# martinruenz/co-fusion

Measured on AMD Instinct MI355X. Metric: frames/sec at 640x480 (N active models) + ICP-reduce achieved HBM GB/s vs peak, higher is better.
Workload: dtype f32

## Files before the change

### co_fusion_amd/csrc/cabi.hip

```cpp
#include <stdlib.h>
#include <string.h>

#include <string>

#include "cf_host.h"

using namespace cf;

void cf_ctx::set_error(const std::string& m)
{
    std::lock_guard<std::mutex> lk(error_mutex);
    last_error = m;
}

static int lane_ready(cf_ctx* ctx, int lane)
{
    if (!ctx->lanes[lane]) {
        HIPCHK(ctx, hipStreamCreateWithFlags(&ctx->lanes[lane], hipStreamNonBlocking));
        HIPCHK(ctx, hipEventCreateWithFlags(&ctx->lane_done[lane], hipEventDisableTiming));
    }
    return CF_OK;
}
static void leave_lane(cf_ctx* ctx)
{
    if (ctx->forked) { ctx->stream = ctx->forked_from; ctx->forked = false; }
}
static int join_lane(cf_ctx* ctx, int lane)
{
    HIPCHK(ctx, hipEventRecord(ctx->lane_done[lane], ctx->lanes[lane]));
    HIPCHK(ctx, hipStreamWaitEvent(ctx->stream, ctx->lane_done[lane], 0));
    return CF_OK;
}

extern "C" {

int cf_create(const cf_config* cfg, cf_ctx** out)
{
    if (!cfg || !out || cfg->width <= 0 || cfg->height <= 0 || (cfg->width % 16) || (cfg->height % 4)) return CF_EINVAL;
    int ndev = 0;
    if (hipGetDeviceCount(&ndev) != hipSuccess || ndev <= 0) return CF_EHIP;
    cf_ctx* ctx = new cf_ctx();
    ctx->cfg = *cfg;
    if (ctx->cfg.max_models <= 0) ctx->cfg.max_models = 1;
    *out = ctx;
    HIPCHK(ctx, hipSetDevice(cfg->device));
    HIPCHK(ctx, hipStreamCreateWithFlags(&ctx->own_stream, hipStreamNonBlocking));
    ctx->stream = ctx->own_stream;
    ctx->icp_launch = IcpLaunch{256, 0, 0};
    if (int r = dmalloc(ctx, &ctx->d_acc_a, (size_t)kGroups * 32)) return r;
    if (int r = dmalloc(ctx, &ctx->d_acc_b, (size_t)kGroups * 32)) return r;
    if (int r = dmalloc(ctx, &ctx->d_out, 64)) return r;
    if (int r = dmalloc(ctx, &ctx->d_scratch_state, 1)) return r;
    if (int r = dmalloc(ctx, &ctx->d_state_pool, (size_t)cf_ctx::kStateSlots)) return r;
    HIPCHK(ctx, hipHostMalloc(reinterpret_cast<void**>(&ctx->h_state_pool), sizeof(OdomDev) * cf_ctx::kStateSlots, hipHostMallocCoherent));
    memset(ctx->h_state_pool, 0, sizeof(OdomDev) * cf_ctx::kStateSlots);
    if (int r = dmalloc(ctx, &ctx->d_so3_sync, (size_t)ctx->cfg.max_models + 1)) return r;
    if (const char* e = getenv("CF_ICP_ARITH")) {
        if (cf_set_icp_arith(ctx, (!strcmp(e, "gram") || !strcmp(e, "1")) ? CF_ICP_ARITH_GRAM : (!strcmp(e, "reference") || !strcmp(e, "2")) ? CF_ICP_ARITH_REFERENCE
                                  : (!strcmp(e, "product") || !strcmp(e, "0")) ? CF_ICP_ARITH_PRODUCT : -1) != CF_OK) {
            ctx->set_error("CF_ICP_ARITH: product | gram | reference"); return CF_EINVAL;
        }
    }
    if (int r = dmalloc(ctx, &ctx->d_cand_scratch, (size_t)cfg->width * cfg->height)) return r;
    HIPCHK(ctx, hipHostMalloc(reinterpret_cast<void**>(&ctx->h_scratch_state), sizeof(OdomDev)));
    HIPCHK(ctx, hipHostMalloc(reinterpret_cast<void**>(&ctx->h_out), sizeof(unsigned long long) * 64));
    ctx->prof.capacity = 8192;
    ctx->prof.events = new hipEvent_t[ctx->prof.capacity];
    for (int i = 0; i < ctx->prof.capacity; i++) HIPCHK(ctx, hipEventCreate(&ctx->prof.events[i]));
    ctx->prof.used = 0; ctx->prof.enabled = 0; ctx->prof.bytes = 0; ctx->prof.launches = 0;
    HIPCHK(ctx, hipStreamSynchronize(ctx->stream));
    return CF_OK;
}

void cf_destroy(cf_ctx* ctx)
{
    if (ctx && ctx->batch_event) (void)hipEventDestroy(ctx->batch_event);
    if (ctx) for (int i = 0; i < cf_ctx::kSurfEvents; i++) if (ctx->surf_events[i]) (void)hipEventDestroy(ctx->surf_events[i]);
    if (!ctx) return;
    (void)hipStreamSynchronize(ctx->stream);
    (void)cf_rccl_destroy(ctx);
    (void)hipFree(ctx->d_acc_a); (void)hipFree(ctx->d_acc_b); (void)hipFree(ctx->d_out);
    (void)hipFree(ctx->d_scratch_state); (void)hipFree(ctx->d_so3_sync); (void)hipFree(ctx->d_cand_scratch);
    (void)hipFree(ctx->d_state_pool); (void)hipHostFree(ctx->h_state_pool);
    (void)hipHostFree(ctx->h_scratch_state); (void)hipHostFree(ctx->h_out);
    if (ctx->d_ref) (void)hipFree(ctx->d_ref);
    if (ctx->h_ref) (void)hipHostFree(ctx->h_ref);
    if (ctx->d_redetect_bits) (void)hipFree(ctx->d_redetect_bits);
    if (ctx->d_redetect_counts) (void)hipFree(ctx->d_redetect_counts);
    if (ctx->h_redetect_counts) (void)hipHostFree(ctx->h_redetect_counts);
    if (ctx->d_search) (void)hipFree(ctx->d_search);
    if (ctx->h_search) (void)hipHostFree(ctx->h_search);
    for (hipEvent_t e : ctx->redetect_ev) if (e) (void)hipEventDestroy(e);
    if (ctx->prof.events) {
        for (int i = 0; i < ctx->prof.capacity; i++) (void)hipEventDestroy(ctx->prof.events[i]);
        delete[] ctx->prof.events;
    }
    for (int i = 0; i < cf_ctx::kLanes; i++) {
        if (ctx->lanes[i]) (void)hipStreamDestroy(ctx->lanes[i]);
        if (ctx->lane_done[i]) (void)hipEventDestroy(ctx->lane_done[i]);
    }
    if (ctx->fork_point) (void)hipEventDestroy(ctx->fork_point);
    for (int i = 0; i < cf_ctx::kMarks; i++) if (ctx->marks[i]) (void)hipEventDestroy(ctx->marks[i]);
    if (ctx->own_stream) (void)hipStreamDestroy(ctx->own_stream);
    delete ctx;
}

const char* cf_last_error(const cf_ctx* ctx)
{
    if (!ctx) return "null ctx";
    static thread_local std::string copy;
    {
        std::lock_guard<std::mutex> lk(const_cast<cf_ctx*>(ctx)->error_mutex);
        copy = ctx->last_error;
    }
    return copy.c_str();
}
int cf_set_stream(cf_ctx* ctx, void* s)
{
    if (!ctx || ctx->forked) return CF_EINVAL;
    if (ctx->stream != (hipStream_t)s) HIPCHK(ctx, hipStreamSynchronize(ctx->stream));
    ctx->stream = (hipStream_t)s;
    return CF_OK;
}
int cf_use_own_stream(cf_ctx* ctx)
{
    if (!ctx || ctx->forked) return CF_EINVAL;
    if (ctx->stream != ctx->own_stream) HIPCHK(ctx, hipStreamSynchronize(ctx->stream));
    ctx->stream = ctx->own_stream;
    return CF_OK;
}

extern "C++" { thread_local cf_thread_binding cf_tls_binding; }

int cf_fork(cf_ctx* ctx, int lane)
{
    if (!ctx || lane < 0) return CF_EINVAL;
    lane %= cf_ctx::kLanes;
    if (int r = lane_ready(ctx, lane)) return r;
    if (!ctx->fork_point) HIPCHK(ctx, hipEventCreateWithFlags(&ctx->fork_point, hipEventDisableTiming));
    if (!ctx->forked) {
        ctx->forked_from = ctx->stream;
        HIPCHK(ctx, hipEventRecord(ctx->fork_point, ctx->forked_from));
        ctx->forked = true;
    }
    HIPCHK(ctx, hipStreamWaitEvent(ctx->lanes[lane], ctx->fork_point, 0));
    ctx->lanes_used |= 1u << lane;
    ctx->stream = ctx->lanes[lane];
    return CF_OK;
}
int cf_mark(cf_ctx* ctx, int slot)
{
    if (!ctx || slot < 0 || slot >= cf_ctx::kMarks) return CF_EINVAL;
    if (!ctx->marks[slot]) HIPCHK(ctx, hipEventCreateWithFlags(&ctx->marks[slot], hipEventDisableTiming));
    HIPCHK(ctx, hipEventRecord(ctx->marks[slot], ctx->stream));
    ctx->mark_set[slot] = true;
    return CF_OK;
}
int cf_event_wait_host(cf_ctx* ctx, int slot)
{
    if (!ctx || slot < 0 || slot >= cf_ctx::kMarks) return CF_EINVAL;
    if (ctx->mark_set[slot]) HIPCHK(ctx, hipEventSynchronize(ctx->marks[slot]));
    return CF_OK;
}
int cf_fork_after(cf_ctx* ctx, int lane, int slot)
{
    if (!ctx || lane < 0 || slot >= cf_ctx::kMarks || ctx->forked) return CF_EINVAL;
    lane %= cf_ctx::kLanes;
    if (int r = lane_ready(ctx, lane)) return r;
    if (slot >= 0 && ctx->mark_set[slot]) HIPCHK(ctx, hipStreamWaitEvent(ctx->lanes[lane], ctx->marks[slot], 0));
    ctx->forked_from = ctx->stream;
    ctx->forked = true;
    ctx->lanes_used |= 1u << lane;
    ctx->stream = ctx->lanes[lane];
    return CF_OK;
}
int cf_main(cf_ctx* ctx)
{
    if (!ctx) return CF_EINVAL;
    leave_lane(ctx);
    return CF_OK;
}
int cf_join(cf_ctx* ctx)
{
    if (!ctx) return CF_EINVAL;
    leave_lane(ctx);
    for (int lane = 0; lane < cf_ctx::kLanes; lane++)
        if (ctx->lanes_used & (1u << lane))
            if (int r = join_lane(ctx, lane)) return r;
    ctx->lanes_used = 0;
    return CF_OK;
}
int cf_join_lane(cf_ctx* ctx, int lane)
{
    if (!ctx || lane < 0) return CF_EINVAL;
    lane %= cf_ctx::kLanes;
    leave_lane(ctx);
    if (ctx->lanes_used & (1u << lane)) {
        if (int r = join_lane(ctx, lane)) return r;
        ctx->lanes_used &= ~(1u << lane);
    }
    return CF_OK;
}
int cf_thread_lane(cf_ctx* ctx, int lane)
{
    if (!ctx) return CF_EINVAL;
    if (lane < 0) { cf_tls_binding = cf_thread_binding{}; return CF_OK; }
    lane %= cf_ctx::kLanes;
    if (!ctx->lanes[lane] || !(ctx->lanes_used & (1u << lane))) { ctx->set_error("cf_thread_lane: lane was not forked"); return CF_ESTATE; }
    HIPCHK(ctx, hipSetDevice(ctx->cfg.device));
    cf_tls_binding.ctx = ctx;
    cf_tls_binding.stream = ctx->lanes[lane];
    return CF_OK;
}
void* cf_get_stream(cf_ctx* ctx) { return ctx ? (void*)ctx->stream : nullptr; }
int cf_synchronize(cf_ctx* ctx) { if (!ctx) return CF_EINVAL; HIPCHK(ctx, hipStreamSynchronize(ctx->stream)); return CF_OK; }
int cf_malloc(cf_ctx* ctx, uint64_t bytes, void** dptr)
{
    if (!ctx || !dptr) return CF_EINVAL;
    HIPCHK(ctx, hipMalloc(dptr, bytes));
    HIPCHK(ctx, hipMemsetAsync(*dptr, 0, bytes, ctx->stream));
    return CF_OK;
}
int cf_free(cf_ctx* ctx, void* dptr) { if (!ctx) return CF_EINVAL; HIPCHK(ctx, hipStreamSynchronize(ctx->stream)); HIPCHK(ctx, hipFree(dptr)); return CF_OK; }
int cf_memcpy_h2d(cf_ctx* ctx, void* dst, const void* src, uint64_t bytes)
{
    if (!ctx) return CF_EINVAL;
    HIPCHK(ctx, hipMemcpyAsync(dst, src, bytes, hipMemcpyHostToDevice, ctx->stream));
    HIPCHK(ctx, hipStreamSynchronize(ctx->stream));
    return CF_OK;
}
int cf_memcpy_d2h(cf_ctx* ctx, void* dst, const void* src, uint64_t bytes)
{
    if (!ctx) return CF_EINVAL;
    HIPCHK(ctx, hipMemcpyAsync(dst, src, bytes, hipMemcpyDeviceToHost, ctx->stream));
    HIPCHK(ctx, hipStreamSynchronize(ctx->stream));
    return CF_OK;
}

int cf_malloc_host(cf_ctx* ctx, uint64_t bytes, void** hptr)
{
    if (!ctx || !hptr) return CF_EINVAL;
    HIPCHK(ctx, hipHostMalloc(hptr, bytes));
    return CF_OK;
}
int cf_free_host(cf_ctx* ctx, void* hptr) { if (!ctx) return CF_EINVAL; HIPCHK(ctx, hipHostFree(hptr)); return CF_OK; }
int cf_memcpy_h2d_async(cf_ctx* ctx, void* dst, const void* src_pinned, uint64_t bytes)
{
    if (!ctx) return CF_EINVAL;
    HIPCHK(ctx, hipMemcpyAsync(dst, src_pinned, bytes, hipMemcpyHostToDevice, ctx->stream));
    return CF_OK;
}
int cf_memcpy_d2h_async(cf_ctx* ctx, void* dst_pinned, const void* src, uint64_t bytes)
{
    if (!ctx) return CF_EINVAL;
    HIPCHK(ctx, hipMemcpyAsync(dst_pinned, src, bytes, hipMemcpyDeviceToHost, ctx->stream));
    return CF_OK;
}
int cf_memcpy_d2d_async(cf_ctx* ctx, void* dst, const void* src, uint64_t bytes)
{
    if (!ctx) return CF_EINVAL;
    HIPCHK(ctx, hipMemcpyAsync(dst, src, bytes, hipMemcpyDeviceToDevice, ctx->stream));
    return CF_OK;
}
int cf_rgb_to_rgba(cf_ctx* ctx, const uint8_t* rgb_dev, int cols, int rows, uint8_t* rgba_dev)
{
    if (!ctx || !rgb_dev || !rgba_dev || cols <= 0 || rows <= 0) return CF_EINVAL;
    launch_rgb_expand(ctx->stream, rgb_dev, cols * rows, rgba_dev);
    LAUNCHCHK(ctx);
    return CF_OK;
}

int cf_set_icp_launch(cf_ctx* ctx, int threads, int ppt)
{
    if (!ctx || (threads != 64 && threads != 128 && threads != 256 && threads != 512 && threads != 1024) ||
        (ppt != 0 && ppt != 1 && ppt != 2 && ppt != 4))
        return CF_EINVAL;
    ctx->icp_launch = IcpLaunch{threads, ppt, ctx->icp_launch.gram};
    return CF_OK;
}

int cf_set_icp_arith(cf_ctx* ctx, int mode)
{
    if (!ctx || (mode != CF_ICP_ARITH_PRODUCT && mode != CF_ICP_ARITH_GRAM && mode != CF_ICP_ARITH_REFERENCE)) return CF_EINVAL;
    ctx->icp_arith = mode;
    ctx->icp_launch.gram = mode == CF_ICP_ARITH_GRAM ? 1 : 0;
    return CF_OK;
}
int cf_get_icp_arith(cf_ctx* ctx) { return ctx ? ctx->icp_arith : CF_EINVAL; }

int cf_profile_enable(cf_ctx* ctx, int on) { if (!ctx || on < 0) return CF_EINVAL; ctx->prof.enabled = on; ctx->prof_calls = 0; return CF_OK; }
int cf_profile_read(cf_ctx* ctx, cf_profile* out, int reset)
{
    if (!ctx || !out) return CF_EINVAL;
    HIPCHK(ctx, hipStreamSynchronize(ctx->stream));
    double ms = ctx->prof_ms_accum;
    for (int i = 0; i + 1 < ctx->prof.used; i += 2) {
        float t = 0;
        HIPCHK(ctx, hipEventElapsedTime(&t, ctx->prof.events[i], ctx->prof.events[i + 1]));
        ms += t;
    }
    ctx->prof_ms_accum = ms;
    ctx->prof.used = 0;
    out->icp_ms_total = ms; out->icp_launches = ctx->prof.launches; out->icp_bytes = ctx->prof.bytes;
    for (int i = 0; i + 1 < ctx->surf_used; i += 2) {
        float t = 0;
        HIPCHK(ctx, hipEventElapsedTime(&t, ctx->surf_events[i], ctx->surf_events[i + 1]));
        ctx->surf_ms_accum += t;
    }
    ctx->surf_used = 0;
    out->surfel_ms_total = ctx->surf_ms_accum; out->surfel_calls = ctx->surf_calls; out->surfel_bytes = ctx->surf_bytes;
    if (reset) { ctx->prof_ms_accum = 0; ctx->prof.launches = 0; ctx->prof.bytes = 0; ctx->surf_ms_accum = 0; ctx->surf_calls = 0; ctx->surf_bytes = 0; }
    return CF_OK;
}

}
```

### co_fusion_amd/csrc/cabi_model.hip

```cpp
#include <math.h>
#include <string.h>

#include <string>
#include <vector>

#include "cf_host.h"

using namespace cf;

struct cf_model {
    cf_ctx* ctx = nullptr;
    uint32_t max_surfels = 0;
    uint32_t count_host = 0;
    bool count_pending = false;
    hipEvent_t count_event = nullptr;
    hipEvent_t count_wait = nullptr;
    bool ratio_valid = false;
    hipEvent_t ratio_event = nullptr;
    float* buf[2] = {nullptr, nullptr};
    int target = 0;
    float* staged = nullptr;
    unsigned* flags = nullptr;
    unsigned* block_sums = nullptr;
    unsigned* d_count = nullptr;
// ... 240 lines not shown
}

int cf_model_initialise(cf_model* m, const uint8_t* rgba, const float* depth_raw, const float* depth_filt, int time, float maxDepth)
{
    if (!m || !rgba || !depth_raw || !depth_filt) return CF_EINVAL;
    m->drop_preindex();
    m->extents_unknown();
    cf_ctx* ctx = m->ctx; hipStream_t s = ctx->cur();
    const int W = ctx->cfg.width, H = ctx->cfg.height; const long long N = (long long)W * H;
    if ((uint32_t)N > m->max_surfels) return CF_ENOMEM;
    const cf_cam cam = ctx_cam(ctx);
    launch_feedback(s, rgba, depth_raw, W, H, cam, m->inv_fx, m->inv_fy, m->tcx, m->tcy, time, maxDepth, m->fb_rec, m->new_flags);
    HIPCHK(ctx, hipMemsetAsync(m->fb_raw, 0, sizeof(float) * 12 * N, s));
    const ScanPassArgs raw{m->fb_rec, m->new_flags, N, m->block_sums, m->d_count, 0, m->fb_raw, nullptr};
    launch_scan_scatter_batch(s, &raw, 1);
    launch_feedback(s, rgba, depth_filt, W, H, cam, m->inv_fx, m->inv_fy, m->tcx, m->tcy, time, maxDepth, m->fb_rec, m->new_flags);
    HIPCHK(ctx, hipMemsetAsync(m->fb_filt, 0, sizeof(float) * 12 * N, s));
    const ScanPassArgs filt{m->fb_rec, m->new_flags, N, m->block_sums, m->d_tmp2, 0, m->fb_filt, nullptr};
    launch_scan_scatter_batch(s, &filt, 1);
    m->new_flags_clean = false;
    launch_init(s, m->fb_raw, m->fb_filt, m->d_count, N, m->buf[m->target]);
    LAUNCHCHK(ctx);
    return sync_count(m);
}

int cf_model_count(cf_model* m, uint32_t* count) { if (!m || !count) return CF_EINVAL; return exact_count(m, count); }

int cf_model_predict_indices(cf_model* m, const float pose[16], int time, float maxDepth, int timeDelta)
{
    if (!m || !pose) return CF_EINVAL;
    m->drop_preindex();
    m->extents_unknown();
    cf_ctx* ctx = m->ctx;
    uint32_t nb = 0;
    if (int r = count_bound(m, &nb)) return r;
    const IndexPassArgs a = index_pass_args(m, pose, nullptr, nb, maxDepth, time, timeDelta);
    launch_index_keys_batch(ctx->cur(), &a, 1, ctx_cam(ctx), ctx->cfg.width, ctx->cfg.height);
    launch_index_resolve_batch(ctx->cur(), &a, 1, ctx_cam(ctx), ctx->cfg.width, ctx->cfg.height);
    LAUNCHCHK(ctx);
    return CF_OK;
}

int cf_model_index_keys(cf_model* m, const float pose[16], int time, float maxDepth, int timeDelta, uint32_t surfel_begin, uint32_t surfel_end,
                        uint64_t* keys_dev)
{
    if (!m || !pose || !keys_dev || surfel_begin > surfel_end) return CF_EINVAL;
    m->drop_preindex();
    m->extents_unknown();
    cf_ctx* ctx = m->ctx;
    const int W = ctx->cfg.width, H = ctx->cfg.height;
    uint32_t nb = 0;
    if (int r = count_bound(m, &nb)) return r;
    HIPCHK(ctx, hipMemsetAsync(keys_dev, 0xFF, sizeof(uint64_t) * (size_t)W * H, ctx->cur()));
    IndexPassArgs a = index_pass_args(m, pose, nullptr, surfel_end < nb ? surfel_end : nb, maxDepth, time, timeDelta);
    a.id_begin = surfel_begin; a.keys = reinterpret_cast<unsigned long long*>(keys_dev);
    launch_index_keys_batch(ctx->cur(), &a, 1, ctx_cam(ctx), W, H);
    LAUNCHCHK(ctx);
    return CF_OK;
}
int cf_model_index_resolve(cf_model* m, const float pose[16], uint64_t* keys_dev)
{
    if (!m || !pose || !keys_dev) return CF_EINVAL;
    m->drop_preindex();
    m->extents_unknown();
    cf_ctx* ctx = m->ctx;
    IndexPassArgs a = index_pass_args(m, pose, nullptr, 0, 0.f, 0, 0);
    a.keys = reinterpret_cast<unsigned long long*>(keys_dev);
    launch_index_resolve_batch(ctx->cur(), &a, 1, ctx_cam(ctx), ctx->cfg.width, ctx->cfg.height);
    LAUNCHCHK(ctx);
    return CF_OK;
}

int cf_model_predict_indices_sharded(cf_model* m, const float pose[16], int time, float maxDepth, int timeDelta, int shard, int nshards)
{
    if (!m || !pose || nshards < 1 || shard < 0 || shard >= nshards) return CF_EINVAL;
    m->drop_preindex();
    cf_ctx* ctx = m->ctx;
    if (!ctx->collective) { ctx->set_error("cf_model_predict_indices_sharded: no collective registered (cf_set_collective)"); return CF_ESTATE; }
    uint32_t n = 0;
    if (int r = exact_count(m, &n)) return r;
    const uint32_t b = (uint32_t)(((uint64_t)n * (uint64_t)shard) / (uint64_t)nshards), e = (uint32_t)(((uint64_t)n * (uint64_t)(shard + 1)) / (uint64_t)nshards);
    if (int r = cf_model_index_keys(m, pose, time, maxDepth, timeDelta, b, e, reinterpret_cast<uint64_t*>(m->keys))) return r;
    if (ctx->collective(ctx->collective_user, 1, m->keys, (uint64_t)ctx->cfg.width * ctx->cfg.height, (void*)ctx->cur()) != 0) {
        ctx->set_error("cf_model_predict_indices_sharded: the collective failed");
        return CF_ESTATE;
    }
    return cf_model_index_resolve(m, pose, reinterpret_cast<uint64_t*>(m->keys));
}

int cf_model_combined_predict(cf_model* m, const float pose[16], float maxDepth, float confThreshold, int time, int maxTime, int timeDelta)
{
    if (!m || !pose) return CF_EINVAL;
    cf_ctx* ctx = m->ctx;
    uint32_t nb = 0;
    if (int r = count_bound(m, &nb)) return r;
    const SplatPassArgs a = splat_args(m, pose, nb, maxDepth, confThreshold, time, maxTime, timeDelta);
    launch_combined_predict_batch(ctx->cur(), &a, 1, ctx_cam(ctx), ctx->cfg.width, ctx->cfg.height);
    LAUNCHCHK(ctx);
    m->ratio_valid = false;
    return CF_OK;
}

int cf_model_predict_inactive(cf_model* m, const float pose[16], float maxDepth, float confThreshold, int maxTime, int timeDelta)
{
    if (!m || !pose) return CF_EINVAL;
    cf_ctx* ctx = m->ctx;
    const size_t N = (size_t)ctx->cfg.width * ctx->cfg.height;
    if (!m->old_covered) {
        if (!m->old_image) if (int r = dmalloc(ctx, &m->old_image, N * 4)) return r;
        if (!m->old_vertex) if (int r = dmalloc(ctx, &m->old_vertex, N * 4)) return r;
        if (!m->old_normal) if (int r = dmalloc(ctx, &m->old_normal, N * 4)) return r;
        if (!m->old_time) if (int r = dmalloc(ctx, &m->old_time, N)) return r;
        if (int r = dmalloc(ctx, &m->old_covered, 1)) return r;
    }
    uint32_t nb = 0;
    if (int r = count_bound(m, &nb)) return r;
    SplatPassArgs a = splat_args(m, pose, nb, maxDepth, confThreshold, 0, maxTime, timeDelta);
    a.image = m->old_image; a.vertexConf = m->old_vertex; a.normalRad = m->old_normal; a.time16 = m->old_time;
    a.fill.out2 = m->old_covered;
    HIPCHK(ctx, hipMemsetAsync(m->old_covered, 0, sizeof(unsigned), ctx->cur()));
    launch_combined_predict_batch(ctx->cur(), &a, 1, ctx_cam(ctx), ctx->cfg.width, ctx->cfg.height, kSplatCount);
    LAUNCHCHK(ctx);
    return CF_OK;
}

int cf_model_synthesize_depth(cf_model* m, const float pose[16], float maxDepth, float confThreshold, int time, int maxTime, int timeDelta,
                              float* depth_out_dev)
{
    if (!m || !pose || !depth_out_dev) return CF_EINVAL;
    cf_ctx* ctx = m->ctx;
    uint32_t nb = 0;
    if (int r = count_bound(m, &nb)) return r;
    SplatPassArgs a = splat_args(m, pose, nb, maxDepth, confThreshold, time, maxTime, timeDelta);
    a.image = nullptr; a.vertexConf = depth_out_dev; a.normalRad = nullptr; a.time16 = nullptr;
    launch_combined_predict_batch(ctx->cur(), &a, 1, ctx_cam(ctx), ctx->cfg.width, ctx->cfg.height, kSplatDepth);
    LAUNCHCHK(ctx);
    return CF_OK;
}

int cf_model_prefetch_fill_ratio(cf_model* m)
{
    if (!m) return CF_EINVAL;
    cf_ctx* ctx = m->ctx;
    launch_fill_ratio(ctx->cur(), m->splat_image, ctx->cfg.width, ctx->cfg.height, m->d_tmp2 + 2, m->h_counts + 2);
    LAUNCHCHK(ctx);
    HIPCHK(ctx, hipEventRecord(m->ratio_event, ctx->cur()));
    m->ratio_valid = true;
    return CF_OK;
}

int cf_model_perform_fill_in(cf_model* m, const uint8_t* rgba, const float* depth_filt, int passthrough_geom, int passthrough_rgb)
{
    if (!m || !rgba || !depth_filt) return CF_EINVAL;
    cf_ctx* ctx = m->ctx;
    launch_fill_in(ctx->cur(), m->splat_vertex, m->splat_normal, m->splat_image, depth_filt, rgba, ctx->cfg.width, ctx->cfg.height, ctx_cam(ctx),
                   m->inv_fx, m->inv_fy, passthrough_geom, passthrough_rgb, m->fill_vertex, m->fill_normal, m->fill_image);
    LAUNCHCHK(ctx);
    return CF_OK;
}

int cf_model_requires_fill_in(cf_model* m, float ratio, int* out)
{
    if (!m || !out) return CF_EINVAL;
    cf_ctx* ctx = m->ctx;
    if (m->ratio_valid) {
        HIPCHK(ctx, hipEventSynchronize(m->ratio_event));
    } else {
        launch_fill_ratio(ctx->cur(), m->splat_image, ctx->cfg.width, ctx->cfg.height, m->d_tmp2 + 2, m->h_counts + 2);
        LAUNCHCHK(ctx);
        HIPCHK(ctx, hipStreamSynchronize(ctx->cur()));
    }
    *out = ((float)m->h_counts[2] / (float)m->h_counts[3] < ratio) ? 1 : 0;
    return CF_OK;
}

int cf_model_fill_ratio_device(cf_model* m, const uint32_t** counts_dev)
{
    if (!m || !counts_dev) return CF_EINVAL;
    *counts_dev = m->ratio_valid ? m->d_tmp2 + 2 : nullptr;
    return CF_OK;
}

int cf_model_fuse(cf_model* m, const float pose[16], int time, const uint8_t* rgba, const uint8_t* mask, const float* depth_raw,
                  const float* depth_filt, float maxDepth, float weighting, int maskID)
{
    if (!m || !pose || !rgba || !mask || !depth_raw || !depth_filt) return CF_EINVAL;
    m->drop_preindex();
    m->extents_unknown();
    cf_ctx* ctx = m->ctx; hipStream_t s = ctx->cur();
    cf_model_pass it{};
    it.model = m; it.pose = pose; it.rgba = rgba; it.mask = mask; it.depth_raw = depth_raw; it.depth_filtered = depth_filt; it.time = time;
    it.fuse_max_depth = maxDepth; it.weighting = weighting; it.mask_id = maskID;
    const SurfelFuseArgs a = fuse_args(it);
    launch_associate_batch(s, &a, 1);
    const ScanPassArgs sp = fresh_compaction_args(m);
    launch_scan_scatter_batch(s, &sp, 1);
    m->new_flags_clean = true;
    uint32_t nb = 0;
    if (int r = count_bound(m, &nb)) return r;
    const UpdatePassArgs ua = update_pass_args(m, nb, time);
    launch_update_batch(s, &ua, 1);
    m->target = 1 - m->target;
    LAUNCHCHK(ctx);
    return CF_OK;
}

int cf_model_clean(cf_model* m, const float pose[16], int time, float confThreshold, float outlierCoeff, int timeDelta, const float* depth_filt,
                   const uint8_t* mask, int maskID, uint32_t* count_out)
{
    if (!m || !pose || !depth_filt || !mask) return CF_EINVAL;
    m->drop_preindex();
    m->extents_unknown();
    cf_ctx* ctx = m->ctx; hipStream_t s = ctx->cur();
    uint32_t nb = 0;
    if (int r = count_bound(m, &nb)) return r;
    unsigned bound = 0;
    if (int r = clean_staging_bound(m, nb, "cf_model_clean", &bound)) return r;
    cf_model_pass it{};
    it.model = m; it.pose = pose; it.mask = mask; it.depth_filtered = depth_filt; it.time = time; it.mask_id = maskID; it.conf_threshold = confThreshold;
    const CleanPassArgs a = clean_pass_args(it, outlierCoeff, timeDelta, bound, false);
    launch_clean_batch(s, &a, 1);
    const ScanPassArgs sp = kept_compaction_args(m, bound);
    launch_scan_scatter_batch(s, &sp, 1);
    m->target = 1 - m->target;
    LAUNCHCHK(ctx);
    const uint32_t upper = bound < m->max_surfels ? bound : m->max_surfels;
    if (int r = post_count(m, upper)) return r;
    if (count_out) return exact_count(m, count_out);
    return CF_OK;
}

int cf_models_preindex(cf_ctx* ctx, const cf_model_preindex* items, int n, float depth_cutoff, int time_delta)
{
    if (!ctx || !items || n <= 0) return CF_EINVAL;
    hipStream_t s = ctx->cur();
    const int W = ctx->cfg.width, H = ctx->cfg.height;
    std::vector<IndexPassArgs> a((size_t)n);
    for (int k = 0; k < n; k++)
        if (!items[k].model || !items[k].odom || items[k].model->ctx != ctx || items[k].odom->ctx != ctx) return CF_EINVAL;
    ExtentGuard guard;
    for (int k = 0; k < n; k++) guard.models.push_back(items[k].model);
    const bool cull = extent_culling_on(ctx);
    for (int k = 0; k < n; k++) {
        cf_model* m = items[k].model; const cf_odom* od = items[k].odom;
        uint32_t nb = 0;
        if (int r = count_bound(m, &nb)) return r;
        const float* pinv = reinterpret_cast<const float*>(reinterpret_cast<const char*>(od->d_state) + offsetof(cf::OdomDev, pose_inv));
        a[k] = index_pass_args(m, nullptr, pinv, nb, depth_cutoff, items[k].time, time_delta);
        if (int r = next_extent(m, cull, nb, s, &a[k].ext, &a[k].ext_slot)) return r;
    }
    launch_index_keys_batch(s, a.data(), n, ctx_cam(ctx), W, H);
    launch_index_resolve_batch(s, a.data(), n, ctx_cam(ctx), W, H);
    LAUNCHCHK(ctx);
    for (int k = 0; k < n; k++) {
        cf_model* m = items[k].model;
        m->preindex_od = items[k].odom; m->preindex_time = items[k].time; m->preindex_cutoff = depth_cutoff; m->preindex_delta = time_delta; m->preindex_nb = a[k].id_end;
    }
    guard.done = true;
    return CF_OK;
}
static bool preindexed_with(const cf_model* m, const float pose[16], int time, float depth_cutoff, int time_delta, uint32_t nb)
{
    if (!m->preindex_od || m->preindex_time != time) return false;
    if (m->preindex_cutoff != depth_cutoff || m->preindex_delta != time_delta || m->preindex_nb != nb) return false;
    const cf::OdomDev* h = m->preindex_od->h_state;
    for (int r = 0; r < 3; r++) {
        if (memcmp(&pose[r * 4], &h->Rcurr[r * 3], 12) != 0 || memcmp(&pose[r * 4 + 3], &h->tcurr[r], 4) != 0) return false;
    }
    return pose[12] == 0 && pose[13] == 0 && pose[14] == 0 && pose[15] == 1;
}

int cf_models_frame_passes(cf_ctx* ctx, const cf_model_pass* items, int n, float depth_cutoff, float outlier_coeff, int time_delta)
{
    if (!ctx || !items || n <= 0) return CF_EINVAL;
    hipStream_t s = ctx->cur();
    const int W = ctx->cfg.width, H = ctx->cfg.height;
    const cf_cam cam = ctx_cam(ctx);
    std::vector<int> fusing;
    for (int k = 0; k < n; k++) {
        const cf_model_pass& it = items[k];
        if (!it.model || it.model->ctx != ctx || !it.pose || !it.rgba || !it.depth_filtered) return CF_EINVAL;
        if (it.do_fuse) { if (!it.mask || !it.depth_raw) return CF_EINVAL; fusing.push_back(k); }
    }
    for (int k : fusing) {
        cf_model* m = items[k].model;
        uint32_t nb = 0; unsigned bound = 0;
        if (int r = count_bound(m, &nb)) return r;
        if (int r = clean_staging_bound(m, nb, "cf_models_frame_passes", &bound)) return r;
    }
    for (int k = 0; k < n; k++) { uint32_t nb = 0; if (int r = count_bound(items[k].model, &nb)) return r; }
    ExtentGuard guard;
    for (int k = 0; k < n; k++) guard.models.push_back(items[k].model);
    const bool cull = extent_culling_on(ctx);
    int surf_ev = -1;
    if (ctx->prof.enabled > 0 && (ctx->surf_calls_seen++ % (unsigned)ctx->prof.enabled) == 0 && ctx->surf_used + 2 <= cf_ctx::kSurfEvents) {
        for (int e = ctx->surf_used; e < ctx->surf_used + 2; e++)
            if (!ctx->surf_events[e]) HIPCHK(ctx, hipEventCreate(&ctx->surf_events[e]));
        surf_ev = ctx->surf_used; ctx->surf_used += 2;
        HIPCHK(ctx, hipEventRecord(ctx->surf_events[surf_ev], s));
        for (int k = 0; k < n; k++) ctx->surf_bytes += (uint64_t)items[k].model->count_host * 48u * (items[k].do_fuse ? 8u : 2u);
        ctx->surf_calls++;
    }
    static const bool clean_rec_on = getenv("CF_NO_CLEAN_REC") == nullptr;
    auto index_args_of = [&](const std::vector<int>& which, bool feeds_clean, std::vector<IndexPassArgs>& a) -> int {
        a.assign(which.size(), IndexPassArgs{});
        for (size_t q = 0; q < which.size(); q++) {
            const cf_model_pass& it = items[which[q]]; cf_model* m = it.model;
            uint32_t nb = 0;
            if (int r = count_bound(m, &nb)) return r;
            a[q] = index_pass_args(m, it.pose, nullptr, nb, depth_cutoff, it.time, time_delta, feeds_clean && clean_rec_on ? it.depth_filtered : nullptr);
            if (int r = next_extent(m, cull, nb, s, &a[q].ext, &a[q].ext_slot)) return r;
        }
        return CF_OK;
    };
    if (!fusing.empty()) {
        const int nf = (int)fusing.size();
        {
            std::vector<int> todo;
            for (int k : fusing) {
                uint32_t nb = 0;
                if (int r = count_bound(items[k].model, &nb)) return r;
                if (!preindexed_with(items[k].model, items[k].pose, items[k].time, depth_cutoff, time_delta, nb)) todo.push_back(k);
            }
            std::vector<IndexPassArgs> a;
            if (int r = index_args_of(todo, false, a)) return r;
            launch_index_keys_batch(s, a.data(), (int)a.size(), cam, W, H);
            launch_index_resolve_batch(s, a.data(), (int)a.size(), cam, W, H);
        }
        std::vector<SurfelFuseArgs> fa(nf);
        std::vector<ScanPassArgs> sa(nf);
        std::vector<UpdatePassArgs> ua(nf);
        for (int q = 0; q < nf; q++) {
            const cf_model_pass& it = items[fusing[q]]; cf_model* m = it.model;
            fa[q] = fuse_args(it);
            sa[q] = fresh_compaction_args(m);
            m->new_flags_clean = true;
            uint32_t nb = 0;
            if (int r = count_bound(m, &nb)) return r;
            ua[q] = update_pass_args(m, nb, it.time);
        }
        launch_associate_batch(s, fa.data(), nf);
        for (int q = 0; q < nf; q++) items[fusing[q]].model->target = 1 - items[fusing[q]].model->target;
        {
            std::vector<IndexPassArgs> ia;
            if (int r = index_args_of(fusing, true, ia)) return r;
            static const bool side_by_side = getenv("CF_NO_SIDE_BY_SIDE") == nullptr;
            if (!(side_by_side && launch_update_compaction_index_keys(s, ua.data(), sa.data(), ia.data(), nf, cam, W, H))) {
                launch_scan_scatter_batch(s, sa.data(), nf);
                launch_update_batch(s, ua.data(), nf);
                launch_index_keys_batch(s, ia.data(), nf, cam, W, H);
            }
            launch_index_resolve_batch(s, ia.data(), nf, cam, W, H);
        }
        std::vector<CleanPassArgs> ca(nf);
        for (int q = 0; q < nf; q++) {
            const cf_model_pass& it = items[fusing[q]]; cf_model* m = it.model;
            uint32_t nb = 0; unsigned bound = 0;
            if (int r = count_bound(m, &nb)) return r;
            if (int r = clean_staging_bound(m, nb, "cf_models_frame_passes", &bound)) return r;
            ca[q] = clean_pass_args(it, outlier_coeff, time_delta, bound, clean_rec_on);
            sa[q] = kept_compaction_args(m, bound);
        }
        launch_clean_batch(s, ca.data(), nf);
        launch_scan_scatter_batch(s, sa.data(), nf);
        if (!ctx->batch_event) HIPCHK(ctx, hipEventCreateWithFlags(&ctx->batch_event, hipEventDisableTiming));
        for (int q = 0; q < nf; q++) {
            cf_model* m = items[fusing[q]].model;
            m->target = 1 - m->target;
            m->count_host = ca[q].total_bound < m->max_surfels ? ca[q].total_bound : m->max_surfels; m->count_pending = true; m->count_wait = nullptr;
        }
    }
    std::vector<SplatPassArgs> pa(n);
    for (int k = 0; k < n; k++) {
        const cf_model_pass& it = items[k]; cf_model* m = it.model;
        uint32_t nb = m->count_host;
        if (!(m->count_pending && !m->count_wait)) { if (int r = count_bound(m, &nb)) return r; }
        SplatPassArgs& p = pa[k];
        p = splat_args(m, it.pose, nb, depth_cutoff, it.conf_threshold, it.time, it.time, time_delta);
        m->ratio_valid = false;
        if (it.fill_in)
            p.fill = SplatFillArgs{it.depth_filtered, it.rgba, m->inv_fx, m->inv_fy, it.passthrough_geom ? 1 : 0, it.passthrough_rgb ? 1 : 0,
                                   m->fill_vertex, m->fill_normal, m->fill_image, reinterpret_cast<unsigned long long*>(m->d_tmp2 + 4),
                                   m->d_tmp2 + 2, m->h_counts + 2, m->ratio_blocks};
    }
    launch_combined_predict_batch(s, pa.data(), n, cam, W, H);
    LAUNCHCHK(ctx);
    for (int k = 0; k < n; k++)
        if (items[k].fill_in) {
            HIPCHK(ctx, hipEventRecord(items[k].model->ratio_event, s));
            items[k].model->ratio_valid = true;
        }
    if (surf_ev >= 0) HIPCHK(ctx, hipEventRecord(ctx->surf_events[surf_ev + 1], s));
    if (!fusing.empty()) {
        HIPCHK(ctx, hipEventRecord(ctx->batch_event, s));
        for (int k : fusing) items[k].model->count_wait = ctx->batch_event;
    }
    for (int k = 0; k < n; k++) items[k].model->drop_preindex();
    guard.done = true;
    return CF_OK;
}

int cf_model_download_map(cf_model* m, float* host_surfels, uint32_t capacity, uint32_t* count)
{
    if (!m || !count) return CF_EINVAL;
    cf_ctx* ctx = m->ctx;
    if (int r = exact_count(m, count)) return r;
    if (host_surfels) {
        const uint32_t n = m->count_host < capacity ? m->count_host : capacity;
        HIPCHK(ctx, hipMemcpyAsync(host_surfels, m->buf[m->target], (size_t)n * 48, hipMemcpyDeviceToHost, ctx->cur()));
        HIPCHK(ctx, hipStreamSynchronize(ctx->cur()));
    }
    return CF_OK;
}

int cf_model_upload_map(cf_model* m, const float* host_surfels, uint32_t count)
{
    if (!m || (!host_surfels && count) || count > m->max_surfels) return CF_EINVAL;
    m->drop_preindex();
    m->extents_unknown();
    cf_ctx* ctx = m->ctx;
    if (count) HIPCHK(ctx, hipMemcpyAsync(m->buf[m->target], host_surfels, (size_t)count * 48, hipMemcpyHostToDevice, ctx->cur()));
    launch_set_count(ctx->cur(), m->d_count, count);
    HIPCHK(ctx, hipStreamSynchronize(ctx->cur()));
    m->count_host = count; m->count_pending = false;
    return CF_OK;
}

int cf_model_buffer(cf_model* m, int which, void** dptr, uint64_t* bytes)
{
    if (!m || !dptr) return CF_EINVAL;
    const size_t N = (size_t)m->ctx->cfg.width * m->ctx->cfg.height;
    void* p = nullptr; size_t b = 0;
    switch (which) {
        case 0: p = m->index; b = N * 4; break;
        case 1: p = m->vertConf; b = N * 16; break;
        case 2: p = m->colorTime; b = N * 16; break;
        case 3: p = m->normRad; b = N * 16; break;
        case 4: p = m->splat_image; b = N * 4; break;
        case 5: p = m->splat_vertex; b = N * 16; break;
        case 6: p = m->splat_normal; b = N * 16; break;
        case 7: p = m->splat_time; b = N * 2; break;
        case 8: p = m->fill_vertex; b = N * 16; break;
        case 9: p = m->fill_normal; b = N * 16; break;
        case 10: p = m->fill_image; b = N * 4; break;
        case 11: { uint32_t c = 0; if (int r = exact_count(m, &c)) return r; p = m->buf[m->target]; b = (size_t)c * 48; break; }
        case 12: {
            unsigned nf = 0;
            HIPCHK(m->ctx, hipMemcpyAsync(&nf, m->d_nfresh, sizeof(unsigned), hipMemcpyDeviceToHost, m->ctx->cur()));
            HIPCHK(m->ctx, hipStreamSynchronize(m->ctx->cur()));
            if (nf > N / 4 + 64) { m->ctx->set_error("cf_model_buffer: the new-surfel count exceeds its buffer"); return CF_ESTATE; }
            p = m->fresh; b = (size_t)nf * 48; break;
        }
        case 13: p = m->clean_rec; b = N * 32; break;
        case 14: p = m->keys; b = N * 8; break;
        case 15: case 16: case 17: case 18: case 19:
            if (!m->old_covered) { m->ctx->set_error("cf_model_buffer: no inactive prediction yet (cf_model_predict_inactive)"); return CF_ESTATE; }
            if (which == 15) { p = m->old_image; b = N * 4; }
            else if (which == 16) { p = m->old_vertex; b = N * 16; }
            else if (which == 17) { p = m->old_normal; b = N * 16; }
            else if (which == 18) { p = m->old_time; b = N * 2; }
            else { p = m->old_covered; b = 4; }
            break;
        default: return CF_EINVAL;
    }
    *dptr = p; if (bytes) *bytes = b;
    return CF_OK;
}

int cf_set_extent_culling(cf_ctx* ctx, int on)
{
    if (!ctx) return CF_EINVAL;
    ctx->extent_cull = on != 0;
    return CF_OK;
}
int cf_model_extents_unknown(cf_model* m)
{
    if (!m) return CF_EINVAL;
    m->extents_unknown();
    return CF_OK;
}

int cf_redetect_score(cf_ctx* ctx, const cf_redetect_candidate* cands, int n, const cf_redetect_frame* f, cf_redetect_counts* counts, uint32_t* label_pixels)
{
    if (!ctx || !cands || !f || !counts || n <= 0 || n > kRedetectBatch) return CF_EINVAL;
    if (!f->depth || !f->label || f->cols <= 0 || f->rows <= 0 || (long long)f->cols * f->rows > 0x7fffffffLL) return CF_EINVAL;
    hipStream_t s = ctx->cur();
    const unsigned words = (unsigned)(((long long)f->cols * f->rows + 31) / 32);
    const size_t n_counts = (size_t)kRedetectBatch * kRedetectWords + 1;
    if (!ctx->d_redetect_counts) {
        if (int r = dmalloc(ctx, &ctx->d_redetect_counts, n_counts)) return r;
        HIPCHK(ctx, hipHostMalloc(reinterpret_cast<void**>(&ctx->h_redetect_counts), n_counts * sizeof(unsigned)));
    }
    if (words > ctx->redetect_words) {
        HIPCHK(ctx, hipStreamSynchronize(s));
        if (ctx->d_redetect_bits) (void)hipFree(ctx->d_redetect_bits);
        ctx->d_redetect_bits = nullptr; ctx->redetect_words = 0;
        if (int r = dmalloc(ctx, &ctx->d_redetect_bits, (size_t)kRedetectBatch * words)) return r;
        ctx->redetect_words = words;
    }
    RedetectCand rc[kRedetectBatch];
    for (int k = 0; k < n; k++) {
        cf_model* m = cands[k].model;
        if (!m || m->ctx != ctx) return CF_EINVAL;
        uint32_t nb = 0;
        if (int r = count_bound(m, &nb)) return r;
        rc[k].surfels = m->buf[m->target]; rc[k].count = m->d_count; rc[k].count_bound = nb; rc[k].theta = cands[k].conf_threshold;
        inv44f(cands[k].pose, rc[k].t_inv);
    }
    RedetectFrame rf{f->depth, f->label, f->cols, f->rows, f->cam, f->new_label, f->depth_cutoff, f->depth_tol};
    if (ctx->redetect_timing) HIPCHK(ctx, hipEventRecord(ctx->redetect_ev[0], s));
    HIPCHK(ctx, hipMemsetAsync(ctx->d_redetect_counts, 0, n_counts * sizeof(unsigned), s));
    launch_redetect_score(s, rc, n, rf, ctx->d_redetect_bits, words, ctx->d_redetect_counts);
    LAUNCHCHK(ctx);
    if (ctx->redetect_timing) HIPCHK(ctx, hipEventRecord(ctx->redetect_ev[1], s));
    HIPCHK(ctx, hipMemcpyAsync(ctx->h_redetect_counts, ctx->d_redetect_counts, n_counts * sizeof(unsigned), hipMemcpyDeviceToHost, s));
    HIPCHK(ctx, hipStreamSynchronize(s));
    if (ctx->redetect_timing) HIPCHK(ctx, hipEventElapsedTime(&ctx->redetect_last_ms, ctx->redetect_ev[0], ctx->redetect_ev[1]));
    for (int k = 0; k < n; k++) {
        const unsigned* w = ctx->h_redetect_counts + (size_t)k * kRedetectWords;
        counts[k] = cf_redetect_counts{w[0], w[1], w[2], w[3], w[4], w[5]};
    }
    if (label_pixels) *label_pixels = ctx->h_redetect_counts[(size_t)kRedetectBatch * kRedetectWords];
    return CF_OK;
}

int cf_redetect_timing(cf_ctx* ctx, int on, float* last_ms)
{
    if (!ctx) return CF_EINVAL;
    if (on) for (hipEvent_t& e : ctx->redetect_ev) if (!e) HIPCHK(ctx, hipEventCreate(&e));
    ctx->redetect_timing = on != 0;
    if (last_ms) *last_ms = ctx->redetect_last_ms;
    return CF_OK;
}

int cf_relabel(cf_ctx* ctx, uint8_t* label_dev, uint64_t n, int from, int to)
{
    if (!ctx || !label_dev || from < 0 || from > 255 || to < 0 || to > 255 || (reinterpret_cast<uintptr_t>(label_dev) & 15u)) return CF_EINVAL;
    if (from == to || n == 0) return CF_OK;
    launch_relabel(ctx->cur(), label_dev, n, (unsigned)from, (unsigned)to);
    LAUNCHCHK(ctx);
    return CF_OK;
}

static int search_buffers(cf_ctx* ctx)
{
    if (ctx->d_search) return CF_OK;
    HIPCHK(ctx, hipMalloc(reinterpret_cast<void**>(&ctx->d_search), cf_ctx::kSearchBytes));
    HIPCHK(ctx, hipHostMalloc(reinterpret_cast<void**>(&ctx->h_search), cf_ctx::kSearchBytes));
    return CF_OK;
}
static bool search_frame_ok(const cf_redetect_frame* f)
{
    return f && f->depth && f->label && f->cols > 0 && f->rows > 0 && (long long)f->cols * f->rows <= 0x7fffffffLL;
}
static int search_fetch(cf_ctx* ctx, hipStream_t s, size_t offset, size_t bytes)
{
    LAUNCHCHK(ctx);
    if (ctx->redetect_timing) HIPCHK(ctx, hipEventRecord(ctx->redetect_ev[1], s));
    HIPCHK(ctx, hipMemcpyAsync(reinterpret_cast<char*>(ctx->h_search) + offset, reinterpret_cast<char*>(ctx->d_search) + offset, bytes, hipMemcpyDeviceToHost, s));
    HIPCHK(ctx, hipStreamSynchronize(s));
    if (ctx->redetect_timing) HIPCHK(ctx, hipEventElapsedTime(&ctx->redetect_last_ms, ctx->redetect_ev[0], ctx->redetect_ev[1]));
    return CF_OK;
}
static unsigned* search_hist(unsigned long long* base) { return reinterpret_cast<unsigned*>(base + cf_ctx::kSearchWords); }
static constexpr size_t kSearchStepWord = (size_t)kRedetectBatch * kMomentWords;

int cf_redetect_frame_moments(cf_ctx* ctx, const cf_redetect_frame* f, const uint8_t* rgba_dev, int64_t moments[4], uint32_t hist[CF_REDETECT_BINS])
{
    if (!ctx || !search_frame_ok(f) || !rgba_dev || !moments || !hist) return CF_EINVAL;
    if (int r = search_buffers(ctx)) return r;
    hipStream_t s = ctx->cur();
    RedetectFrame rf{f->depth, f->label, f->cols, f->rows, f->cam, f->new_label, f->depth_cutoff, f->depth_tol};
    if (ctx->redetect_timing) HIPCHK(ctx, hipEventRecord(ctx->redetect_ev[0], s));
    HIPCHK(ctx, hipMemsetAsync(ctx->d_search, 0, kMomentWords * 8, s));
    HIPCHK(ctx, hipMemsetAsync(search_hist(ctx->d_search), 0, kRedetectBins * 4, s));
    launch_redetect_frame_moments(s, rf, rgba_dev, ctx->d_search, search_hist(ctx->d_search));
    if (int r = search_fetch(ctx, s, 0, cf_ctx::kSearchWords * 8 + kRedetectBins * 4)) return r;
    for (int k = 0; k < kMomentWords; k++) moments[k] = (int64_t)ctx->h_search[k];
    memcpy(hist, search_hist(ctx->h_search), kRedetectBins * 4);
    return CF_OK;
}

static int search_cand(cf_ctx* ctx, cf_model* m, float theta, RedetectCand* rc)
{
    if (!m || m->ctx != ctx) return CF_EINVAL;
    uint32_t nb = 0;
    if (int r = count_bound(m, &nb)) return r;
    rc->surfels = m->buf[m->target]; rc->count = m->d_count; rc->count_bound = nb; rc->theta = theta;
    return CF_OK;
}

int cf_redetect_model_moments(cf_ctx* ctx, const cf_redetect_candidate* cands, int n, const float dhat[3], int64_t* moments, uint32_t* hist)
{
    if (!ctx || !cands || !dhat || !moments || !hist || n <= 0 || n > kRedetectBatch) return CF_EINVAL;
    if (int r = search_buffers(ctx)) return r;
    RedetectCand rc[kRedetectBatch];
    for (int k = 0; k < n; k++) {
        if (int r = search_cand(ctx, cands[k].model, cands[k].conf_threshold, &rc[k])) return r;
        inv44f(cands[k].pose, rc[k].t_inv);
    }
    hipStream_t s = ctx->cur();
    if (ctx->redetect_timing) HIPCHK(ctx, hipEventRecord(ctx->redetect_ev[0], s));
    HIPCHK(ctx, hipMemsetAsync(ctx->d_search, 0, (size_t)n * kMomentWords * 8, s));
    HIPCHK(ctx, hipMemsetAsync(search_hist(ctx->d_search), 0, (size_t)n * kRedetectBins * 4, s));
    launch_redetect_model_moments(s, rc, n, dhat, ctx->d_search, search_hist(ctx->d_search));
    if (int r = search_fetch(ctx, s, 0, cf_ctx::kSearchWords * 8 + (size_t)n * kRedetectBins * 4)) return r;
    for (int k = 0; k < n * kMomentWords; k++) moments[k] = (int64_t)ctx->h_search[k];
    memcpy(hist, search_hist(ctx->h_search), (size_t)n * kRedetectBins * 4);
    return CF_OK;
}

static int register_step(cf_ctx* ctx, RedetectCand& rc, const float T[16], const RedetectFrame& rf, const float centre[3])
{
    hipStream_t s = ctx->cur();
    memcpy(rc.t_inv, T, sizeof(rc.t_inv));
    if (ctx->redetect_timing) HIPCHK(ctx, hipEventRecord(ctx->redetect_ev[0], s));
    HIPCHK(ctx, hipMemsetAsync(ctx->d_search + kSearchStepWord, 0, 32 * 8, s));
    launch_redetect_register_step(s, rc, rf, centre, ctx->d_search + kSearchStepWord);
    return search_fetch(ctx, s, kSearchStepWord * 8, 32 * 8);
}

int cf_redetect_register_step(cf_ctx* ctx, cf_model* model, float conf_threshold, const float cam_from_model[16], const cf_redetect_frame* f,
                              const float centre[3], int64_t sums[32])
{
    if (!ctx || !cam_from_model || !search_frame_ok(f) || !centre || !sums) return CF_EINVAL;
    if (int r = search_buffers(ctx)) return r;
    RedetectCand rc{};
    if (int r = search_cand(ctx, model, conf_threshold, &rc)) return r;
    RedetectFrame rf{f->depth, f->label, f->cols, f->rows, f->cam, f->new_label, f->depth_cutoff, f->depth_tol};
    if (int r = register_step(ctx, rc, cam_from_model, rf, centre)) return r;
    for (int k = 0; k < 32; k++) sums[k] = (int64_t)ctx->h_search[kSearchStepWord + k];
    return CF_OK;
}

int cf_redetect_register(cf_ctx* ctx, cf_model* model, float conf_threshold, const float seed[16], const cf_redetect_frame* f, const float centre[3],
                         int max_iterations, cf_redetect_registration* out)
{
    if (!ctx || !seed || !search_frame_ok(f) || !centre || !out || max_iterations < 1) return CF_EINVAL;
    if (int r = search_buffers(ctx)) return r;
    RedetectCand rc{};
    if (int r = search_cand(ctx, model, conf_threshold, &rc)) return r;
    RedetectFrame rf{f->depth, f->label, f->cols, f->rows, f->cam, f->new_label, f->depth_cutoff, f->depth_tol};
    double R[9], t[3];
    for (int i = 0; i < 3; i++) { R[3 * i] = seed[4 * i]; R[3 * i + 1] = seed[4 * i + 1]; R[3 * i + 2] = seed[4 * i + 2]; t[i] = seed[4 * i + 3]; }
    const double c[3] = {centre[0], centre[1], centre[2]};
    cf_redetect_registration res{};
    res.ok = 1;
    for (int it = 0; it < max_iterations; it++) {
        float T[16] = {(float)R[0], (float)R[1], (float)R[2], (float)t[0], (float)R[3], (float)R[4], (float)R[5], (float)t[1],
                       (float)R[6], (float)R[7], (float)R[8], (float)t[2], 0.f, 0.f, 0.f, 1.f};
        if (int r = register_step(ctx, rc, T, rf, centre)) return r;
        const long long* sums = reinterpret_cast<const long long*>(ctx->h_search + kSearchStepWord);
        const long long n = sums[28];
        if (it == 0) res.first_inliers = (uint32_t)n;
        res.last_inliers = (uint32_t)n;
        res.rms = n > 0 ? (float)sqrt(ldexp((double)sums[27], -32) / (double)n) : 0.f;
        if (n < 6 || 2 * n < (long long)res.first_inliers) { res.ok = 0; break; }
        double tn, on;
        if (!redetect_register_solve(sums, 1e-3, c, R, t, &tn, &on)) { res.ok = 0; break; }
        res.iterations = it + 1;
        if (tn < 1e-5 && on < 1e-5) break;
    }
    const float T[16] = {(float)R[0], (float)R[1], (float)R[2], (float)t[0], (float)R[3], (float)R[4], (float)R[5], (float)t[1],
                         (float)R[6], (float)R[7], (float)R[8], (float)t[2], 0.f, 0.f, 0.f, 1.f};
    memcpy(res.cam_from_model, T, sizeof(T));
    *out = res;
    return CF_OK;
}

float cf_fusion_weight(const float pose[16], const float lastPose[16], float weightMultiplier)
{
    float pinv[16], diff[16];
    inv44f(pose, pinv);
    for (int i = 0; i < 4; i++)
        for (int j = 0; j < 4; j++) {
            float s = 0;
            for (int k = 0; k < 4; k++) s += pinv[i * 4 + k] * lastPose[k * 4 + j];
            diff[i * 4 + j] = s;
        }
    const float tn = sqrtf(diff[3] * diff[3] + diff[7] * diff[7] + diff[11] * diff[11]);
    const float* R = diff;
    double rx = R[2 * 4 + 1] - R[1 * 4 + 2], ry = R[0 * 4 + 2] - R[2 * 4 + 0], rz = R[1 * 4 + 0] - R[0 * 4 + 1];
    const double s = sqrt((rx * rx + ry * ry + rz * rz) * 0.25);
    double c = (double)((R[0] + R[5] + R[10]) - 1.0f) * 0.5;
    c = c > 1. ? 1. : c < -1. ? -1. : c;
    double theta = acos(c);
    if (s < 1e-5) {
        double t;
        if (c > 0) rx = ry = rz = 0;
        else {
            t = (R[0] + 1) * 0.5; rx = sqrt(t > 0.0 ? t : 0.0);
            t = (R[5] + 1) * 0.5; ry = sqrt(t > 0.0 ? t : 0.0) * (R[0 * 4 + 1] < 0 ? -1.0 : 1.0);
            t = (R[10] + 1) * 0.5; rz = sqrt(t > 0.0 ? t : 0.0) * (R[0 * 4 + 2] < 0 ? -1.0 : 1.0);
            if (fabs(rx) < fabs(ry) && fabs(rx) < fabs(rz) && (R[1 * 4 + 2] > 0) != (ry * rz > 0)) rz = -rz;
            theta /= sqrt(rx * rx + ry * ry + rz * rz);
            rx *= theta; ry *= theta; rz *= theta;
        }
    } else {
        double vth = 1 / (2 * s);
        vth *= theta;
        rx *= vth; ry *= vth; rz *= vth;
    }
    const float rv[3] = {(float)rx, (float)ry, (float)rz};
    const float rn = sqrtf(rv[0] * rv[0] + rv[1] * rv[1] + rv[2] * rv[2]);
    float weighting = tn > rn ? tn : rn;
    const float largest = 0.01f, minWeight = 0.5f;
    if (weighting > largest) weighting = largest;
    const float w = 1.0f - (weighting / largest);
    weighting = (w > minWeight ? w : minWeight) * weightMultiplier;
    return weighting;
}

}
```

### co_fusion_amd/csrc/cf_host.h

```cpp
#pragma once

#include <string.h>

#include <mutex>
#include <string>

#include "cf_kernels.h"

struct cf_ctx;
struct cf_thread_binding { const cf_ctx* ctx = nullptr; hipStream_t stream = nullptr; };
extern thread_local cf_thread_binding cf_tls_binding;

struct cf_ctx {
    cf_config cfg{};
    hipStream_t stream = nullptr;
    hipStream_t cur() const { return cf_tls_binding.ctx == this ? cf_tls_binding.stream : stream; }
    hipStream_t own_stream = nullptr;
    std::string last_error;
    std::mutex error_mutex;
    cf::IcpLaunch icp_launch{256, 0};
    int icp_arith = 0;
    float* d_ref = nullptr;
    float* h_ref = nullptr;
    unsigned long long* d_acc_a = nullptr;
    unsigned long long* d_acc_b = nullptr;
    unsigned long long* d_out = nullptr;
    unsigned long long* h_out = nullptr;
    cf::OdomDev* d_scratch_state = nullptr;
    cf::OdomDev* h_scratch_state = nullptr;
    uint8_t* d_cand_scratch = nullptr;
    cf::So3Sync* d_so3_sync = nullptr;
    unsigned gn_mode_epoch = 0;
    int xcd_round_robin = -1;
    int gn_mode = 1;
    static constexpr int kStateSlots = 256;
    cf::OdomDev* d_state_pool = nullptr;
    cf::OdomDev* h_state_pool = nullptr;
    bool slot_used[kStateSlots]{};
    hipEvent_t batch_event = nullptr;
    bool extent_cull = true;
    static constexpr int kLanes = 8;
    hipStream_t lanes[kLanes]{};
    hipEvent_t lane_done[kLanes]{};
    hipEvent_t fork_point = nullptr;
    static constexpr int kMarks = 64;
    hipEvent_t marks[kMarks]{};
    bool mark_set[kMarks]{};
    hipStream_t forked_from = nullptr;
    bool forked = false;
    unsigned lanes_used = 0;
    int (*collective)(void* user, int op, void* dev_buf, uint64_t words, void* stream) = nullptr;
    void* collective_user = nullptr;
    void* rccl = nullptr;
    unsigned prof_calls = 0;
    cf::ProfSink prof{};
    double prof_ms_accum = 0;
    static constexpr int kSurfEvents = 64;
    hipEvent_t surf_events[kSurfEvents]{};
    int surf_used = 0; unsigned surf_calls_seen = 0;
    double surf_ms_accum = 0; uint64_t surf_calls = 0, surf_bytes = 0;
    unsigned* d_redetect_bits = nullptr; unsigned redetect_words = 0;
    unsigned* d_redetect_counts = nullptr; unsigned* h_redetect_counts = nullptr;
    bool redetect_timing = false; hipEvent_t redetect_ev[2]{}; float redetect_last_ms = 0.f;
    static constexpr size_t kSearchWords = (size_t)cf::kRedetectBatch * cf::kMomentWords + 32;
    static constexpr size_t kSearchBytes = kSearchWords * 8 + (size_t)cf::kRedetectBatch * cf::kRedetectBins * 4;
    unsigned long long* d_search = nullptr; unsigned long long* h_search = nullptr;
    void set_error(const std::string& m);
};
inline cf_cam ctx_cam(const cf_ctx* ctx) { return cf_cam{ctx->cfg.fx, ctx->cfg.fy, ctx->cfg.cx, ctx->cfg.cy}; }
extern "C" int cf_wait_stream(cf_ctx* ctx);
#define HIPCHK(ctx, call)                                                                      \
    do {                                                                                       \
        hipError_t e_ = (call);                                                                \
        if (e_ != hipSuccess) {                                                                \
            (ctx)->set_error(std::string(#call) + ": " + hipGetErrorString(e_));               \
            return CF_EHIP;                                                                    \
        }                                                                                      \
    } while (0)
#define LAUNCHCHK(ctx) HIPCHK(ctx, hipGetLastError())
template <typename T>
inline int dmalloc(cf_ctx* ctx, T** p, size_t count)
{
    HIPCHK(ctx, hipMalloc(reinterpret_cast<void**>(p), count * sizeof(T)));
    HIPCHK(ctx, hipMemsetAsync(*p, 0, count * sizeof(T), ctx->cur()));
    return CF_OK;
}
inline int clear_acc(cf_ctx* ctx, unsigned long long* acc)
{
    HIPCHK(ctx, hipMemsetAsync(acc, 0, sizeof(unsigned long long) * cf::kGroups * 32, ctx->stream));
    return CF_OK;
}
struct cf_odom;
namespace cf {
int ref_track(cf_ctx* ctx, cf_odom* od, const float pose[16], const cf_track_opts* opts, float* err_surface);
int ref_icp_step(cf_ctx* ctx, const float Rcurr[9], const float tcurr[3], const float* vc, const float* nc, const float Rprev_inv[9], const float tprev[3],
                 cf_cam intr, const float* vp, const float* np, float dist_thres, float angle_thres, int cols, int rows, float* err, float out29[29]);
int ref_rgb_step(cf_ctx* ctx, const cf_dataterm* corres, float sigma, const float* cloud3, float fx, float fy, const int16_t* dIdx, const int16_t* dIdy,
                 float sobel_scale, int cols, int rows, float out29[29]);
int ref_so3_step(cf_ctx* ctx, const uint8_t* last_image, const uint8_t* next_image, const float basis[9], const float kinv[9], const float krlr[9],
                 int cols, int rows, float out11[11]);
inline void pose_split(const float pose[16], float R[9], float t[3])
{
    for (int i = 0; i < 3; i++) { R[3 * i] = pose[4 * i]; R[3 * i + 1] = pose[4 * i + 1]; R[3 * i + 2] = pose[4 * i + 2]; t[i] = pose[4 * i + 3]; }
}
struct TrackTerms { bool icp, rgb; };
inline TrackTerms track_terms(const cf_track_opts* o) { return TrackTerms{!o->rgb_only && o->icp_weight > 0, o->rgb_only || o->icp_weight < 100}; }
}

struct cf_odom {
    cf_ctx* ctx = nullptr;
    float* vmaps_tmp = nullptr;
    float* nmaps_tmp = nullptr;
    float* vmap_g_prev[3]{};
    float* nmap_g_prev[3]{};
    float* vmap_curr[3]{};
    float* nmap_curr[3]{};
    const float* ext_vmap_curr[3]{};
    const float* ext_nmap_curr[3]{};
    float2* zrange[3]{};
    bool zrange_valid = false;
    const float2* ext_zrange[3]{};
    const float* cur_vmap(int l) const { return ext_vmap_curr[l] ? ext_vmap_curr[l] : vmap_curr[l]; }
    const float* cur_nmap(int l) const { return ext_nmap_curr[l] ? ext_nmap_curr[l] : nmap_curr[l]; }
    const float2* cur_zrange(int l) const { return ext_vmap_curr[l] ? ext_zrange[l] : (zrange_valid ? zrange[l] : nullptr); }
    float* lastDepth[3]{};
    float* nextDepth[3]{};
    bool next_depth_is_last = false;
    float* next_depth(int i) const { return next_depth_is_last ? lastDepth[i] : nextDepth[i]; }
    uint8_t* lastImage[3]{};
    uint8_t* nextImage[3]{};
    uint8_t* lastNextImage[3]{};
    int16_t* dIdx[3]{};
    int16_t* dIdy[3]{};
    float* cloud[3]{};
    cf_dataterm* corres[3]{};
    uint8_t* cand[3]{};
    unsigned char* occ = nullptr;
    bool occ_valid = false;
    bool use_occ = false;
    unsigned* aabb = nullptr;
    float map_pose[12]{};
    int box_hint[4] = {0x7fffffff, 0, 0, 0};
    unsigned* res_range = nullptr;
    int res_hint[3] = {-1, -1, -1};
    bool box_valid = false;
    int band_begin = 0, band_end = 0;
    bool band_counts = true;
    unsigned long long* icp_acc = nullptr;
    unsigned long long* rgb_acc = nullptr;
    cf::OdomDev* d_state = nullptr;
    cf::OdomDev* h_state = nullptr;
    int slot = -1;
    float distThres = 0, angleThres = 0, sobelScale = 0, maxDepthDeltaRGB = 0, maxDepthRGB = 0;
    float angleSqLt = 0, distSqLe = 0;
    float minGrad[3]{};
    bool pending_so3_swap = false;
    size_t rgb_acc_words = 0;
    unsigned gn_epoch_seen = 0;
    bool result_pending = false;
    int expected_solves = -1;
    cf::LaunchShape launch_shape{};
};
```

### co_fusion_amd/csrc/cf_kernels.h

```cpp
#pragma once

#include <hip/hip_runtime.h>
#include <hip/hip_ext.h>
#include <stdint.h>

#include "../../include/cofusion_hip.h"

namespace cf {

__host__ __device__ __forceinline__ cf_cam cam_level(cf_cam c, int level)
{
    const int div = 1 << level;
    return cf_cam{c.fx / div, c.fy / div, c.cx / div, c.cy / div};
}

constexpr int kGroups = 64;

struct alignas(64) GnHot {
    int icp, level_done; float cull_z[2];
    float Rcurr[9], tcurr[3];
    float Rprev_inv[9], tprev[3];
    int cull_box[4];
    int rgb, rgbOnly, level_done2, pad;
    float krkInv[9], kt[3];
// ... 1 lines not shown
static_assert(sizeof(GnHot) == 192, "three 64-byte lines");

struct OdomDev;
struct OdomDev {
    const float* vmap_curr[3];
    const float* nmap_curr[3];
    const float* vmap_g_prev[3];
    const float* nmap_g_prev[3];
    const float* lastDepth[3];
    const float* nextDepth[3];
    const uint8_t* lastImage[3];
    const uint8_t* nextImage[3];
    const uint8_t* lastNextImage[3];
    const int16_t* dIdx[3];
    const int16_t* dIdy[3];
    const float* cloud[3];
    cf_dataterm* corres[3];
    const uint8_t* cand[3];
    unsigned long long* icp_acc;
    unsigned long long* rgb_acc;
    float* err_surface;
    cf_cam intr;
    int width, height;
    float distThres, angleThres, sobelScale, maxDepthDeltaRGB;
    float minGrad[3];
    float icpWeight;
    int icp, rgb, rgbOnly;
    unsigned* aabb_acc;
    int cull;
    float box_R[9], box_t[3];
    unsigned* res_range;
    OdomDev* host_twin;
    float Rprev[9], tprev[3], Rprev_inv[9], Rcurr[9], tcurr[3];
    double resultRt[16];
    float krkInv[9], kt[3];
    float lastRGBError;
    int level_done;
    int solves;
    float residual[2];
    float box_lo[3], box_hi[3];
    int res_seen[3];
    float cull_z[2];
    float pose_inv[16];
    cf_track_stats stats;
    GnHot hot;
};
__host__ __device__ inline void refresh_hot(OdomDev* od)
{
    GnHot& h = od->hot;
    h.icp = od->icp; h.level_done = od->level_done; h.cull_z[0] = od->cull_z[0]; h.cull_z[1] = od->cull_z[1];
    for (int k = 0; k < 9; k++) { h.Rcurr[k] = od->Rcurr[k]; h.Rprev_inv[k] = od->Rprev_inv[k]; h.krkInv[k] = od->krkInv[k]; }
    for (int k = 0; k < 3; k++) { h.tcurr[k] = od->tcurr[k]; h.tprev[k] = od->tprev[k]; h.kt[k] = od->kt[k]; }
    for (int k = 0; k < 4; k++) h.cull_box[k] = od->stats.cull_box[k];
    h.rgb = od->rgb; h.rgbOnly = od->rgbOnly; h.level_done2 = od->level_done; h.pad = 0;
}

void launch_vmap(hipStream_t s, const float* depth, int cols, int rows, cf_cam intr, float cutoff, float* vmap);
void launch_nmap(hipStream_t s, const float* vmap, int cols, int rows, float* nmap);
void launch_copy_maps(hipStream_t s, const float* v4, const float* n4, int cols, int rows, float* vmap, float* nmap);
void launch_resize_map(hipStream_t s, const float* in, int in_cols, int in_rows, float* out, bool normalize);
void launch_transform_maps(hipStream_t s, float* vmap, float* nmap, int cols, int rows, const float R[9], const float t[3]);
void launch_vertices_to_depth(hipStream_t s, const float* v4, int cols, int rows, float cutoff, float* depth);
void launch_pyrdown_f32(hipStream_t s, const float* src, int scols, int srows, float* dst);
void launch_pyrdown_u8(hipStream_t s, const uint8_t* src, int scols, int srows, uint8_t* dst);
void launch_intensity(hipStream_t s, const uint8_t* rgba, int cols, int rows, uint8_t* dst);
void launch_rgb_expand(hipStream_t s, const uint8_t* rgb, int n, uint8_t* rgba);
void launch_sobel(hipStream_t s, const uint8_t* src, int cols, int rows, int16_t* dx, int16_t* dy);
void launch_cloud(hipStream_t s, const float* depth, int cols, int rows, cf_cam il, float* cloud3);

struct Level3 { int cols[3], rows[3], blk_end[3]; };
struct FrameMapsArgs {
    Level3 L;
    const float* depth[3]; float* vmap[3]; float* nmap[3];
    float fx_inv[3], fy_inv[3], cx[3], cy[3];
    float cutoff;
    float2* zrange[3];
};
struct RgbPrepArgs {
    Level3 L;
    const uint8_t* nextImage[3]; const float* nextDepth[3]; const float* lastDepth[3];
    int16_t* dIdx[3]; int16_t* dIdy[3]; uint8_t* cand[3]; float* cloud[3];
    float minScale[3], fx_inv[3], fy_inv[3], cx[3], cy[3];
    unsigned* res_range;
};
struct ModelMapsArgs {
    const float* pred_v4; const float* pred_n4;
    const float* alt_v4; const float* alt_n4;
    const unsigned* sel; float sel_ratio;
    float* snapshot;
    float* vmap[3]; float* nmap[3];
    int cols, rows;
    float R[9], t[3];
    unsigned char* occ;
    unsigned* aabb;
};
constexpr int kPrepBatch = 8;
struct ModelMapsBatch { ModelMapsArgs m[kPrepBatch]; };
struct RgbPrepBatch { RgbPrepArgs m[kPrepBatch]; };
struct RgbdChain {
    const float* v4; const uint8_t* rgba; float* depth[3]; uint8_t* image[3];
    const float* alt_v4; const uint8_t* alt_rgba; const unsigned* sel; float sel_ratio;
};
struct RgbdBatch {
    RgbdChain c[2 * kPrepBatch];
    uint8_t* fan_image[3][kPrepBatch];
    signed char fan_owner[kPrepBatch];
};
void launch_model_maps(hipStream_t s, const ModelMapsBatch& b, int n);
void launch_frame_maps(hipStream_t s, FrameMapsArgs a, int W, int H);
void launch_rgbd_pyramids(hipStream_t s, const RgbdBatch& b, int n_chains, int W, int H, float cutoff);
void launch_model_maps_and_pyramids(hipStream_t s, const ModelMapsBatch& mb, int n, const RgbdBatch& rb, int n_chains, int W, int H, float cutoff);
void launch_rgb_prep(hipStream_t s, RgbPrepBatch b, int n, int W, int H);

struct IDiv { unsigned M, s; };
inline IDiv make_idiv(int d)
{
    if (d < 2) return IDiv{0x80000000u, 0u};
    unsigned l = 0;
    while ((1u << l) < (unsigned)d) l++;
    return IDiv{(unsigned)((((unsigned long long)1 << (31 + l)) + (unsigned)d - 1) / (unsigned)d), l - 1};
}
constexpr int kGramBits[8] = {20, 20, 20, 17, 17, 17, 22, 0};
struct LaunchShape { int icp[3]; int res[3]; int icp_err; };
struct IcpLaunch { int threads; int ppt; int gram;
                   LaunchShape* const* shape = nullptr; };

constexpr int kMaxBatch = 16;
struct IcpModelArgs {
    const float* vc; const float* nc;
    const float* vp; const float* np;
    const OdomDev* st;
    unsigned long long* acc;
    float* err;
    const unsigned char* occ;
    int row_begin, row_end;
    int cull;
    const float2* zr;
    int box_blocks;
};
constexpr int kNoBoxHint = 0x7fffffff;
struct CullRuns { int x0, y0, nrx, total; };
__host__ __device__ inline CullRuns cull_runs(const int box[4], int L, int cols, int rows)
{
    int bx0 = (box[0] >> L) - 1, by0 = (box[1] >> L) - 1, bx1 = (box[2] >> L) + 1, by1 = (box[3] >> L) + 1;
    bx0 = bx0 < 0 ? 0 : bx0; by0 = by0 < 0 ? 0 : by0; bx1 = bx1 > cols - 1 ? cols - 1 : bx1; by1 = by1 > rows - 1 ? rows - 1 : by1;
    if (bx0 > bx1 || by0 > by1) return CullRuns{0, 0, 0, 0};
    if ((cols & 63) == 0) { const int nrx = (bx1 >> 6) - (bx0 >> 6) + 1; return CullRuns{bx0 >> 6, by0, nrx, nrx * (by1 - by0 + 1)}; }
    const int q0 = (by0 * cols) >> 6, q1 = ((by1 + 1) * cols - 1) >> 6;
    return CullRuns{0, q0, 0, q1 - q0 + 1};
}
inline int box_blocks_for(const int box_hint[4], int L, int cols, int rows, int threads)
{
    if (box_hint[0] == kNoBoxHint) return 0;
    const CullRuns cr = cull_runs(box_hint, L, cols, rows);
    const int wpb = threads / 64;
    const int runs = cr.total + cr.total / 4 + 2 * (cr.nrx > 0 ? cr.nrx : (cols + 63) / 64);
    int want = (((runs + 2 * wpb - 1) / (2 * wpb) + 7) / 8) * 8;
    return want < 8 ? 8 : want;
}
inline int residual_blocks_for(int seen) { return seen < 0 ? 0 : seen + seen / 4 + 2; }
struct GnArgs {
    OdomDev* od[kMaxBatch];
    unsigned long long* icp_acc[kMaxBatch];
    unsigned long long* rgb_acc[kMaxBatch];
    OdomDev* od_host[kMaxBatch];
    int slot_px;
    int icp_gram;
};
struct RgbModelArgs {
    OdomDev* st;
    const uint8_t* cand; const float* nextDepth; const float* lastDepth;
    const uint8_t* lastImage; const uint8_t* nextImage;
    cf_dataterm* corres; const float* cloud; const int16_t* dIdx; const int16_t* dIdy;
    unsigned long long* icp_acc; unsigned long long* rgb_acc;
    int no_counts;
    uint2* recs;
    unsigned* slot_counts;
    const unsigned* res_range;
    int res_blocks;
};
struct RgbArgs {
    RgbModelArgs m[kMaxBatch];
    int cols, rows;
    cf_cam il;
    float sobelScale, maxDepthDelta;
    int compact;
    int slot_px;
    IDiv cdiv;
};
inline RgbModelArgs rgb_model_args(const OdomDev* h , OdomDev* d_state, int level)
{
    return RgbModelArgs{d_state, h->cand[level], h->nextDepth[level], h->lastDepth[level], h->lastImage[level], h->nextImage[level],
                        h->corres[level], h->cloud[level], h->dIdx[level], h->dIdy[level], h->icp_acc, h->rgb_acc, 0,
                        reinterpret_cast<uint2*>(h->corres[level]),
                        reinterpret_cast<unsigned*>(reinterpret_cast<uint2*>(h->corres[level]) + (size_t)(h->width >> level) * (h->height >> level)),
                        h->res_range ? h->res_range + 2 * level : nullptr, 0};
}
constexpr int kMaxSlots = 2 * kMaxBatch;
struct IcpArgs {
    IcpModelArgs m[kMaxBatch];
    int cols, rows;
    cf_cam intr;
    float distThres, angleThres;
    float angleSqLt, distSqLe;
    int occ_w, occ_shift;
    int flags;
    int row_begin, row_end;
    IDiv cdiv;
    int slot_end[kMaxSlots];
    unsigned char slot_desc[kMaxSlots];
    int slots_used;
};
constexpr unsigned char kResidualSlot = 0x80;
void launch_icp_level(hipStream_t s, IcpLaunch cfg, const IcpArgs& args, int n, int level, hipEvent_t ev0 = nullptr, hipEvent_t ev1 = nullptr);
void launch_rgb_residual(hipStream_t s, const RgbArgs& ra, int n);
void launch_rgb_step(hipStream_t s, const RgbArgs& ra, int n);
constexpr uint64_t kRgbResidualBytes = 27;
constexpr uint64_t kRgbResidualBytesCompact = 11;
void launch_acc_total(hipStream_t s, const unsigned long long* acc, unsigned long long* out);
void launch_rgb_cand(hipStream_t s, const int16_t* dIdx, const int16_t* dIdy, const float* next_depth,
                     const uint8_t* next_image, float min_scale, int cols, int rows, uint8_t* cand);
void launch_so3_step(hipStream_t s, const uint8_t* last_image, const uint8_t* next_image, const float basis[9],
                     const float kinv[9], const float krlr[9], int cols, int rows, unsigned long long* out16);
void launch_gn_solve(hipStream_t s, const GnArgs& gn, int n, int next_level, int last_of_level);

struct ProfSink {
    hipEvent_t* events; int capacity; int used; uint64_t bytes; uint64_t launches; int enabled;
};

constexpr int kSo3Blocks = 16;
constexpr int kStepSubs = 16;
struct So3Sync { unsigned long long acc[10][16]; unsigned arrive, depart;
                 unsigned step_top, pad;
                 unsigned step_sub[kStepSubs][32]; };
struct GnHook { int (*fn)(void* user, int op, void* dev_buf, uint64_t words, void* stream); void* user; int split[kMaxBatch]; };
struct TrackerStates { OdomDev* dev[kMaxBatch]; const OdomDev* host[kMaxBatch]; };
bool launch_gn_track(hipStream_t s, IcpLaunch cfg, const TrackerStates& states, So3Sync* so3_syncs ,
                     const GnHook* hook, const IcpArgs icp_args[3], const RgbArgs rgb_args[3], int n, int width, int height, bool so3,
                     bool pyramid, bool fast_odom, bool rgb, bool icp, int mode, ProfSink* prof,
                     OdomDev* const* h_states = nullptr ,
                     const RgbPrepBatch* prep = nullptr );
void launch_rgb_slot_step(hipStream_t s, const RgbArgs& ra, So3Sync* so3_syncs , int n, int mode, int icp_fix, int next_level, int last_of_level);
void launch_rgb_records_residual(hipStream_t s, IcpLaunch cfg, const RgbArgs& ra, int n, int level);
inline size_t rgb_acc_rows(size_t n0)
{
    const size_t slots0 = (n0 + 255) / 256, quads0 = (slots0 + 1) / 2;
    return quads0 > (size_t)kGroups ? quads0 : (size_t)kGroups;
}
void launch_so3_prealign(hipStream_t s, const TrackerStates& states, So3Sync* so3_syncs , int n, bool so3, int first_level,
                         const RgbPrepBatch* prep );
void rgb_prep_levels(RgbPrepBatch& b, int n, int W, int H);
float replay_icp_level0(hipStream_t s, IcpLaunch cfg, const IcpArgs& a0, const RgbArgs& r0, int n, int slots, int ablate, int reps, hipEvent_t e0, hipEvent_t e1);
#ifdef CF_ABLATE
void trace_so3_dump(hipStream_t s);
void trace_solve_begin();
void trace_solve_end(hipStream_t s, const char* path);
void trace_step_solve(hipStream_t s, IcpLaunch cfg, const IcpArgs& a0, const RgbArgs& r0, So3Sync* syncs, int n, const char* path);
void trace_icp_level0(hipStream_t s, IcpLaunch cfg, const IcpArgs& a0, const RgbArgs& r0, int n, int slots, const char* path);
#endif
bool probe_xcd_round_robin(hipStream_t s);
float sqrt_gate_lt(float T);
float sqrt_gate_le(float T);

constexpr int kSurfBatch = 16;
struct IndexPassArgs {
    const float* surfels; const unsigned* count; unsigned id_begin, id_end; float t_inv[16]; float maxDepth; int time, timeDelta;
    unsigned long long* keys; unsigned* index; float* vertConf; float* colorTime; float* normRad;
    const float* t_inv_dev;
    float* clean_rec;
    const float* clean_depth;
    unsigned* ext;
    int ext_slot;
};
__host__ __device__ inline void inv44f(const float a[16], float o[16])
{
    const float c00 = a[5] * a[10] - a[6] * a[9];
    const float c01 = a[6] * a[8] - a[4] * a[10];
    const float c02 = a[4] * a[9] - a[5] * a[8];
    const float det = a[0] * c00 + a[1] * c01 + a[2] * c02;
    const float id = 1.0f / det;
    float Li[9];
    Li[0] = c00 * id; Li[1] = (a[2] * a[9] - a[1] * a[10]) * id; Li[2] = (a[1] * a[6] - a[2] * a[5]) * id;
    Li[3] = c01 * id; Li[4] = (a[0] * a[10] - a[2] * a[8]) * id; Li[5] = (a[2] * a[4] - a[0] * a[6]) * id;
    Li[6] = c02 * id; Li[7] = (a[1] * a[8] - a[0] * a[9]) * id; Li[8] = (a[0] * a[5] - a[1] * a[4]) * id;
    for (int i = 0; i < 3; i++) {
        o[i * 4 + 0] = Li[i * 3 + 0]; o[i * 4 + 1] = Li[i * 3 + 1]; o[i * 4 + 2] = Li[i * 3 + 2];
        o[i * 4 + 3] = -(Li[i * 3 + 0] * a[3] + Li[i * 3 + 1] * a[7] + Li[i * 3 + 2] * a[11]);
    }
    o[12] = 0; o[13] = 0; o[14] = 0; o[15] = 1;
}
struct SplatFillArgs {
    const float* depth_filt; const uint8_t* rgba;
    float inv_fx, inv_fy; int pass_geom, pass_rgb;
    float* fill_vertex; float* fill_normal; uint8_t* fill_image;
    unsigned long long* acc;
    unsigned* out2; unsigned* out2_host;
    int sample_blocks;
};
int fill_ratio_sample_blocks(int cols, int rows);
struct SplatPassArgs {
    const float* surfels; const unsigned* count; unsigned count_bound; float t_inv[16]; float maxDepth, confThreshold; int time, maxTime, timeDelta;
    const float* rays; unsigned long long* keys; uint8_t* image; float* vertexConf; float* normalRad; uint16_t* time16;
    SplatFillArgs fill;
};
struct UpdatePassArgs { const float* in; const unsigned* count; unsigned count_bound; unsigned* owner; const float* records; int time; float* out; };
struct SurfelFuseArgs {
    const unsigned* index; const float* vertConf; const float* normRad;
    const uint8_t* rgba; const float* depth_raw; const float* depth_filt; const uint8_t* mask;
    const float* tcx; const float* tcy;
    float pose[16]; cf_cam cam; float inv_fx, inv_fy;
    int cols, rows, time; float weighting; int maskID; float maxDepth;
    float* records; unsigned* new_flags; unsigned* owner;
    int flags_clean = 0;
};
struct CleanPassArgs {
    const unsigned* index; const float* vertConf; const float* colorTime;
    const float* depth_filt; const uint8_t* mask;
    const float* rec;
    float t_inv[16]; cf_cam cam; int cols, rows, time; float confThreshold, outlierCoeff; int timeDelta, maskID;
    const float* surfels; const unsigned* count; const float* fresh; const unsigned* n_fresh; unsigned total_bound; float* staged; unsigned* flags;
};
struct ScanPassArgs {
    const float* rec; const unsigned* flags; long long n; unsigned* block_sums; unsigned* total; unsigned add_to_total; float* out; unsigned* total_host;
    int zero_flags = 0;
};
void launch_index_keys_batch(hipStream_t s, const IndexPassArgs* items, int n, cf_cam cam, int cols, int rows);
bool launch_update_compaction_index_keys(hipStream_t s, const UpdatePassArgs* up, const ScanPassArgs* sc, const IndexPassArgs* ix, int n, cf_cam cam, int cols,
                                         int rows);
void launch_index_resolve_batch(hipStream_t s, const IndexPassArgs* items, int n, cf_cam cam, int cols, int rows);
enum { kSplatFull = 0, kSplatCount = 1, kSplatDepth = 2 };
void launch_combined_predict_batch(hipStream_t s, const SplatPassArgs* items, int n, cf_cam cam, int cols, int rows, int mode = kSplatFull);
void launch_associate_batch(hipStream_t s, const SurfelFuseArgs* items, int n);
void launch_update_batch(hipStream_t s, const UpdatePassArgs* items, int n);
void launch_clean_batch(hipStream_t s, const CleanPassArgs* items, int n);
void launch_scan_scatter_batch(hipStream_t s, const ScanPassArgs* items, int n);
void launch_bilateral(hipStream_t s, const float* depth, int cols, int rows, float maxD, float* out);
void launch_feedback(hipStream_t s, const uint8_t* rgba, const float* depth, int cols, int rows, cf_cam cam, float inv_fx, float inv_fy,
                     const float* tcx, const float* tcy, int time, float maxDepth, float* rec, unsigned* flags);
void launch_init(hipStream_t s, const float* raw, const float* filt, const unsigned* raw_count, long long max_n, float* out);
void launch_splat_rays(hipStream_t s, cf_cam cam, int cols, int rows, float* rays );
void launch_fill_in(hipStream_t s, const float* pv, const float* pn, const uint8_t* pimg, const float* depth, const uint8_t* rgba, int cols,
                    int rows, cf_cam cam, float inv_fx, float inv_fy, int pass_geom, int pass_rgb, float* ov, float* on, uint8_t* oi);
void launch_fill_ratio(hipStream_t s, const uint8_t* pimg, int cols, int rows, unsigned* out2, unsigned* out2_host = nullptr );
void launch_set_count(hipStream_t s, unsigned* out, unsigned v);

constexpr int kRedetectBatch = 16;
constexpr int kRedetectWords = 8;
struct RedetectCand {
    const float* surfels; const unsigned* count; unsigned count_bound;
    float theta;
    float t_inv[16];
};
struct RedetectFrame {
    const float* depth; const uint8_t* label; int cols, rows; cf_cam cam; int new_label; float cutoff, tol;
};
void launch_redetect_score(hipStream_t s, const RedetectCand* cands, int n, const RedetectFrame& f, unsigned* bits, unsigned words, unsigned* counts);
void launch_relabel(hipStream_t s, uint8_t* label , unsigned long long n, unsigned from, unsigned to);

constexpr int kRedetectBins = 512;
constexpr int kMomentWords = 4;
void launch_redetect_frame_moments(hipStream_t s, const RedetectFrame& f, const uint8_t* rgba, unsigned long long* moments, unsigned* hist);
void launch_redetect_model_moments(hipStream_t s, const RedetectCand* cands, int n, const float dhat[3], unsigned long long* moments, unsigned* hist);
void launch_redetect_register_step(hipStream_t s, const RedetectCand& c, const RedetectFrame& f, const float centre[3], unsigned long long* out);
bool redetect_register_solve(const long long sums[32], double lambda, const double centre[3], double R[9], double t[3], double* tau_norm, double* omega_norm);

}
```

### co_fusion_amd/csrc/surf_batch_dev.h

```cpp
#pragma once

#include "cf_surfel_device.h"
#include "cf_kernels.h"

namespace cf {

static constexpr int kB = 256;
static inline int gridFor(long long n, int wg = kB) { return (int)((n + wg - 1) / wg); }
static inline int gridXcd(long long n, int chunk = 1, int wg = kB) { const int q = 8 * (chunk > 1 ? chunk : 1); return (gridFor(n, wg) + q - 1) / q * q; }
#ifdef CF_ABLATE
static int xcd_env(const char* name, int dflt) { const char* e = getenv(name); return e ? atoi(e) : dflt; }
#else
static constexpr int xcd_env(const char*, int dflt) { return dflt; }
#endif
struct BatchHdr { int n; int blk_end[kSurfBatch]; };
template <class A> struct Batch { BatchHdr h; A m[kSurfBatch]; };
struct VBlock { int model, bid, nblk; };
__device__ __forceinline__ VBlock batch_decode_at(const BatchHdr& h, int b)
{
    int slot = 0;
#pragma unroll
    for (int k = 0; k < kSurfBatch - 1; k++) slot += (b >= h.blk_end[k]) ? 1 : 0;
    const int start = slot ? h.blk_end[slot - 1] : 0;
    return VBlock{slot, b - start, h.blk_end[slot] - start};
}
__device__ __forceinline__ VBlock batch_decode(const BatchHdr& h) { return batch_decode_at(h, (int)blockIdx.x); }
template <class A>
static int batch_layout(Batch<A>& B, const int* blocks, int n)
{
    int total = 0;
    B.h.n = n;
    for (int k = 0; k < kSurfBatch; k++) {
        if (k < n) total += (blocks[k] + 7) / 8 * 8;
        B.h.blk_end[k] = k < n ? total : 0x7fffffff;
    }
    return total;
}
template <class A, class H, class Item, class Launch>
static void for_each_batch(const H* items, int n_items, Item item, Launch launch)
{
    for (int base = 0; base < n_items; base += kSurfBatch) {
        const int nb = n_items - base < kSurfBatch ? n_items - base : kSurfBatch;
        Batch<A> B;
        int blocks[kSurfBatch];
        for (int k = 0; k < nb; k++) blocks[k] = item(items[base + k], B.m[k]);
        launch(B, blocks, nb, items + base);
    }
}

__device__ __forceinline__ int xcd_block(int chunk, int b, int nblk)
{
    if (chunk == 0) return b;
    const int per = nblk >> 3, x = b & 7, r = b >> 3;
    if (chunk < 0) return x * per + r;
    const int lb = ((r / chunk) * 8 + x) * chunk + (r % chunk);
    return lb;
}

__device__ __forceinline__ unsigned sortable_bits(float z)
{
    const unsigned b = __float_as_uint(z);
    return (b & 0x80000000u) ? ~b : (b | 0x80000000u);
}
__device__ __forceinline__ unsigned long long zkey(float z, unsigned id) { return ((unsigned long long)sortable_bits(z) << 32) | id; }
constexpr unsigned long long kEmptyKey = ~0ull;

static Mat4 mat4_from(const float m[16]) { Mat4 r; for (int i = 0; i < 16; i++) r.m[i] = m[i]; return r; }

}
```

### co_fusion_amd/csrc/surf_scan_dev.h

```cpp
#pragma once
#include "surf_batch_dev.h"

namespace cf {

static constexpr int kScanItems = 2048;
struct ScanArgs {
    const float4* rec; const unsigned* flags; long long n; unsigned* block_sums; unsigned* total; unsigned add_to_total; int zero_flags;
    float4* out; unsigned* total_host;
};
__device__ __forceinline__ void scan_load_flags(const unsigned* __restrict__ flags, long long i0, long long n, unsigned (&f)[8])
{
    if (i0 + 8 <= n) {
        const uint4 a = *reinterpret_cast<const uint4*>(flags + i0), c = *reinterpret_cast<const uint4*>(flags + i0 + 4);
        f[0] = a.x; f[1] = a.y; f[2] = a.z; f[3] = a.w; f[4] = c.x; f[5] = c.y; f[6] = c.z; f[7] = c.w;
    } else {
        unsigned t[8];
#pragma unroll
        for (int e = 0; e < 8; e++) t[e] = flags[i0 + e < n ? i0 + e : n - 1];
#pragma unroll
        for (int e = 0; e < 8; e++) f[e] = (i0 + e < n) ? t[e] : 0u;
    }
}
__device__ __forceinline__ void scan_block_sums_body(const Batch<ScanArgs>& B, int blk)
{
    const VBlock vb = batch_decode_at(B.h, blk);
    const ScanArgs& a = B.m[vb.model];
    const unsigned* __restrict__ flags = a.flags; const long long n = a.n; unsigned* __restrict__ block_sums = a.block_sums;
    if ((long long)vb.bid * kScanItems >= n) return;
    unsigned f[8];
    scan_load_flags(flags, (long long)vb.bid * kScanItems + (long long)threadIdx.x * 8, n, f);
    unsigned s = 0;
#pragma unroll
    for (int e = 0; e < 8; e++) s += f[e];
    for (int o = 32; o > 0; o >>= 1) s += __shfl_xor((int)s, o, 64);
    __shared__ unsigned w[4];
    if ((threadIdx.x & 63) == 0) w[threadIdx.x >> 6] = s;
    __syncthreads();
    if (threadIdx.x == 0) block_sums[vb.bid] = w[0] + w[1] + w[2] + w[3];
}
__global__ void __launch_bounds__(256) scan_block_sums_kernel(const Batch<ScanArgs> B) { scan_block_sums_body(B, (int)blockIdx.x); }
__device__ __forceinline__ void scan_scatter_body(const Batch<ScanArgs>& B, int blk)
{
    const VBlock vb = batch_decode_at(B.h, blk);
    const ScanArgs& a = B.m[vb.model];
    const float4* __restrict__ rec = a.rec; const unsigned* __restrict__ flags = a.flags; const long long n = a.n;
    const unsigned* __restrict__ block_sums = a.block_sums; unsigned* __restrict__ total = a.total; const unsigned add_to_total = a.add_to_total;
    float4* __restrict__ out = a.out; unsigned* __restrict__ total_host = a.total_host;
    const int nb = (int)((n + kScanItems - 1) / kScanItems);
    if (vb.bid >= nb) return;
    __shared__ unsigned wsum[4], s_base;
    __shared__ unsigned short s_src[kScanItems];
    const int tid = threadIdx.x, lane = tid & 63, wave = tid >> 6;
    const long long i0 = (long long)vb.bid * kScanItems + (long long)tid * 8;
    unsigned f[8];
    scan_load_flags(flags, i0, n, f);
    if (a.zero_flags) {
        unsigned* fz = const_cast<unsigned*>(flags);
        if (i0 + 8 <= n) { *reinterpret_cast<uint4*>(fz + i0) = make_uint4(0, 0, 0, 0); *reinterpret_cast<uint4*>(fz + i0 + 4) = make_uint4(0, 0, 0, 0); }
        else
            for (int e = 0; e < 8; e++) if (i0 + e < n) fz[i0 + e] = 0;
    }
    unsigned b = 0;
    for (int k = tid; k < vb.bid; k += 256) b += block_sums[k];
    for (int o = 32; o > 0; o >>= 1) b += __shfl_xor((int)b, o, 64);
    if (lane == 0) wsum[wave] = b;
    __syncthreads();
    if (tid == 0) s_base = wsum[0] + wsum[1] + wsum[2] + wsum[3];
    unsigned mine = 0;
#pragma unroll
    for (int e = 0; e < 8; e++) mine += f[e];
    unsigned incl = mine;
    for (int o = 1; o < 64; o <<= 1) { const unsigned t = __shfl_up((int)incl, o, 64); if (lane >= o) incl += t; }
    __syncthreads();
    if (lane == 63) wsum[wave] = incl;
    __syncthreads();
    unsigned rel = incl - mine;
    for (int w = 0; w < wave; w++) rel += wsum[w];
#pragma unroll
    for (int e = 0; e < 8; e++)
        if (f[e]) s_src[rel++] = (unsigned short)(tid * 8 + e);
    const unsigned count = wsum[0] + wsum[1] + wsum[2] + wsum[3];
    const unsigned base = s_base;
    __syncthreads();
    const float4* __restrict__ in0 = rec + (size_t)vb.bid * kScanItems * 3;
    float4* __restrict__ out0 = out + (size_t)base * 3;
    const unsigned words = count * 3;
#ifndef CF_SCAN_FLY
#define CF_SCAN_FLY 4
#endif
    constexpr int kFly = CF_SCAN_FLY;
    for (unsigned m0 = tid; m0 < words; m0 += kFly * 256) {
        float4 v[kFly];
#pragma unroll
        for (int u = 0; u < kFly; u++) {
            const unsigned m = m0 + u * 256;
            const unsigned mc = m < words ? m : words - 1;
            const unsigned j = mc / 3u;
            v[u] = in0[(size_t)s_src[j] * 3 + (mc - 3u * j)];
        }
#pragma unroll
        for (int u = 0; u < kFly; u++) { const unsigned m = m0 + u * 256; if (m < words) out0[m] = v[u]; }
    }
    if (vb.bid == nb - 1 && tid == 255) {
        *total = base + count + add_to_total;
        if (total_host) *total_host = base + count + add_to_total;
    }
}
__global__ void __launch_bounds__(256) scan_scatter_kernel(const Batch<ScanArgs> B) { scan_scatter_body(B, (int)blockIdx.x); }

struct FillArgs { uint4* p; long long n16; };
__global__ void __launch_bounds__(kB) fill_zero_kernel(const Batch<FillArgs> B)
{
    const VBlock vb = batch_decode(B.h);
    const FillArgs& a = B.m[vb.model];
    const long long i = (long long)vb.bid * kB + threadIdx.x;
    if (i < a.n16) a.p[i] = make_uint4(0, 0, 0, 0);
}
__global__ void set_count_kernel(unsigned* out, unsigned v) { *out = v; }
__global__ void set_count2_kernel(unsigned* out, unsigned* out_host, unsigned v) { *out = v; if (out_host) *out_host = v; }

static ScanArgs scan_args(const ScanPassArgs& h)
{
    return ScanArgs{reinterpret_cast<const float4*>(h.rec), h.flags, h.n, h.block_sums, h.total, h.add_to_total, h.zero_flags, reinterpret_cast<float4*>(h.out), h.total_host};
}
static int scan_blocks(const ScanPassArgs& h) { return (int)((h.n + kScanItems - 1) / kScanItems); }
void launch_scan_scatter_batch(hipStream_t s, const ScanPassArgs* items, int n_items)
{
    for_each_batch<ScanArgs>(items, n_items, [](const ScanPassArgs& h, ScanArgs& a) { a = scan_args(h); return scan_blocks(h); },
        [s](Batch<ScanArgs>& B, const int* blocks, int nb, const ScanPassArgs*) {
            for (int k = 0; k < nb; k++)
                if (blocks[k] == 0) set_count2_kernel<<<1, 1, 0, s>>>(B.m[k].total, B.m[k].total_host, B.m[k].add_to_total);
            const int grid = batch_layout(B, blocks, nb);
            if (!grid) return;
            scan_block_sums_kernel<<<grid, 256, 0, s>>>(B);
            scan_scatter_kernel<<<grid, 256, 0, s>>>(B);
        });
}
void launch_set_count(hipStream_t s, unsigned* out, unsigned v) { set_count_kernel<<<1, 1, 0, s>>>(out, v); }

}
```

### co_fusion_amd/csrc/surf_splat_dev.h

```cpp
#pragma once
#include "surf_index_dev.h"

namespace cf {

struct SplatSetup { f3 ph, n; float rad, pn; int x_lo, x_hi, y_lo, y_hi; };

__device__ __forceinline__ bool splat_setup(const float4 pc, const float4 ct, const float4 nr, const Mat4& t_inv, cf_cam cam, int cols,
                                            int rows, float maxDepth, float confThreshold, int time, int maxTime, int timeDelta,
                                            SplatSetup& s)
{
    s.ph = xform_point(t_inv, f3{pc.x, pc.y, pc.z});
    if (s.ph.z > maxDepth || s.ph.z < 0 || pc.w < confThreshold || (float)time - ct.w > (float)timeDelta || ct.w > (float)maxTime) return false;
    s.n = normalized(xform_dir(t_inv, f3{nr.x, nr.y, nr.z}));
    s.rad = nr.w;
    const f3 x1n = normalized(f3{s.n.y - s.n.z, -s.n.x, s.n.x});
    const f3 x1 = {x1n.x * s.rad * 1.41421356f, x1n.y * s.rad * 1.41421356f, x1n.z * s.rad * 1.41421356f};
    const f3 y1 = cross(s.n, x1);
    const f3 c[4] = {s.ph + x1, s.ph + y1, s.ph - y1, s.ph - x1};
    float px_[4], py_[4];
#pragma unroll
    for (int k = 0; k < 4; k++) { px_[k] = ((cam.fx * c[k].x) / c[k].z) + cam.cx; py_[k] = ((cam.fy * c[k].y) / c[k].z) + cam.cy; }
    const float xmin = fminf(px_[0], fminf(px_[1], fminf(px_[2], px_[3]))), xmax = fmaxf(px_[0], fmaxf(px_[1], fmaxf(px_[2], px_[3])));
    const float ymin = fminf(py_[0], fminf(py_[1], fminf(py_[2], py_[3]))), ymax = fmaxf(py_[0], fmaxf(py_[1], fmaxf(py_[2], py_[3])));
    const float size = fmaxf(0.0f, fmaxf(fabsf(xmax - xmin), fabsf(ymax - ymin)));
    if (!(size > 0.0f) || !(size <= 4096.0f)) return false;
    const float u = ((cam.fx * s.ph.x) / s.ph.z) + cam.cx, v = ((cam.fy * s.ph.y) / s.ph.z) + cam.cy;
    if (!(u >= 0.0f && v >= 0.0f && u <= (float)cols && v <= (float)rows)) return false;
    const float half = size * 0.5f;
    s.x_lo = max((int)ceilf(u - half - 0.5f), 0); s.x_hi = min((int)ceilf(u + half - 0.5f) - 1, cols - 1);
    s.y_lo = max((int)ceilf(v - half - 0.5f), 0); s.y_hi = min((int)ceilf(v + half - 0.5f) - 1, rows - 1);
    s.pn = dot(s.ph, s.n);
    return true;
}

__device__ __forceinline__ bool splat_fragment(const SplatSetup& s, const float4* __restrict__ rays, int cols, int px, int py, float maxDepth,
                                               float& z)
{
    const float4 lr = rays[py * cols + px];
    const f3 l = {lr.x, lr.y, lr.z};
    const float k = s.pn / dot(l, s.n);
    const f3 cp = {k * l.x, k * l.y, k * l.z};
    const f3 diff = cp - s.ph;
    if (!(dot(diff, diff) <= s.rad * s.rad)) return false;
    if (!(cp.z < maxDepth)) return false;
    z = cp.z;
    return true;
}

__global__ void __launch_bounds__(kB) splat_rays_kernel(cf_cam cam, int cols, int rows, float4* __restrict__ rays)
{
    const int q = blockIdx.x * kB + threadIdx.x;
    if (q >= cols * rows) return;
    const int py = q / cols, px = q - py * cols;
    const float fx_ = (float)px + 0.5f, fy_ = (float)py + 0.5f;
    const f3 l = normalized(f3{(fx_ - cam.cx) / cam.fx, (fy_ - cam.cy) / cam.fy, 1.0f});
    rays[q] = make_float4(l.x, l.y, l.z, 0.f);
}

struct SplatArgs {
    const float4* surfels; const unsigned* count; Mat4 t_inv; float maxDepth, confThreshold; int time, maxTime, timeDelta;
    const float4* rays; unsigned long long* keys; uchar4* image; float4* vertexConf; float4* normalRad; unsigned short* time16;
    SplatFillArgs fill;
};

__global__ void __launch_bounds__(kB) splat_raster_kernel(const Batch<SplatArgs> B, const FrameGeom g)
{
    const VBlock vb = batch_decode(B.h);
    const SplatArgs& a = B.m[vb.model];
    const float4* __restrict__ surfels = a.surfels; const float4* __restrict__ rays = a.rays; unsigned long long* __restrict__ keys = a.keys;
    const int cols = g.cols, rows = g.rows;
    const unsigned gt = vb.bid * kB + threadIdx.x;
    const unsigned id = gt >> 2;
    const int sub = (int)(gt & 3u);
    if (id >= *a.count) return;
    SplatSetup s;
    if (!splat_setup(surfels[id * 3], surfels[id * 3 + 1], surfels[id * 3 + 2], a.t_inv, g.cam, cols, rows, a.maxDepth, a.confThreshold, a.time,
                     a.maxTime, a.timeDelta, s))
        return;
    const int w = s.x_hi - s.x_lo + 1, h = s.y_hi - s.y_lo + 1;
    if (w <= 0 || h <= 0) return;
    int fx = sub, fy = 0;
    while (fx >= w) { fx -= w; fy++; }
    while (fy < h) {
        const int px = s.x_lo + fx, py = s.y_lo + fy;
        float z;
        if (splat_fragment(s, rays, cols, px, py, a.maxDepth, z)) {
            atomicMin(&keys[py * cols + px], zkey(z, id));
        }
        fx += 4;
        while (fx >= w) { fx -= w; fy++; }
    }
}

__device__ __forceinline__ void fill_in_px(float4 v, float4 n, uchar4 e, const float* __restrict__ depth, const uchar4* __restrict__ rgba, int cols,
                                           int rows, int x, int y, int q, float cx, float cy, float inv_fx, float inv_fy, int pass_geom, int pass_rgb,
                                           float4* __restrict__ ov, float4* __restrict__ on, uchar4* __restrict__ oi)
{
    const float z = depth[q];
    const f3 p = {((float)x - cx) * z * inv_fx, ((float)y - cy) * z * inv_fy, z};
    ov[q] = (v.z == 0 || pass_geom) ? make_float4(p.x, p.y, p.z, 1.f) : v;
    if (n.z == 0 || pass_geom) {
        const float zx = depth[y * cols + min(x + 1, cols - 1)], zy = depth[min(y + 1, rows - 1) * cols + x];
        const f3 vx = {((float)(x + 1) - cx) * zx * inv_fx, ((float)y - cy) * zx * inv_fy, zx};
        const f3 vy = {((float)x - cx) * zy * inv_fx, ((float)(y + 1) - cy) * zy * inv_fy, zy};
        const f3 nn = normalized(cross(vx - p, vy - p));
        on[q] = make_float4(nn.x, nn.y, nn.z, 1.f);
    } else
        on[q] = n;
    oi[q] = (((int)e.x + (int)e.y + (int)e.z) == 0 || pass_rgb) ? rgba[q] : e;
}
__global__ void __launch_bounds__(kB) fill_in_kernel(const float4* __restrict__ pv, const float4* __restrict__ pn, const uchar4* __restrict__ pimg,
                                                     const float* __restrict__ depth, const uchar4* __restrict__ rgba, int cols, int rows,
                                                     float cx, float cy, float inv_fx, float inv_fy, int pass_geom, int pass_rgb,
                                                     float4* __restrict__ ov, float4* __restrict__ on, uchar4* __restrict__ oi)
{
    const int q = blockIdx.x * kB + threadIdx.x;
    if (q >= cols * rows) return;
    const int y = q / cols, x = q - y * cols;
    fill_in_px(pv[q], pn[q], pimg[q], depth, rgba, cols, rows, x, y, q, cx, cy, inv_fx, inv_fy, pass_geom, pass_rgb, ov, on, oi);
}
__device__ __forceinline__ bool fill_ratio_sample(int p, int dn, int size)
{
    const int i0 = p * dn / size;
    bool hit = false;
    for (int i = max(i0 - 1, 0); i <= min(i0 + 1, dn - 1); i++) hit = hit || nearest_texel(((float)i + 0.5f) / (float)dn, size) == p;
    return hit;
}

int fill_ratio_sample_blocks(int cols, int rows)
{
    const int dw = cols / 20, dh = rows / 20;
    int blocks = 0, last = -1;
    for (int j = 0; j < dh; j++)
        for (int i = 0; i < dw; i++) {
            const auto texel = [](float u, int size) { const int t = (int)floorf(u * (float)size); return t < 0 ? 0 : (t > size - 1 ? size - 1 : t); };
            const int b = (texel(((float)j + 0.5f) / (float)dh, rows) * cols + texel(((float)i + 0.5f) / (float)dw, cols)) / kB;
            if (b != last) { blocks++; last = b; }
        }
    return blocks;
}

template <int kMode>
__global__ void __launch_bounds__(kB) splat_resolve_kernel(const Batch<SplatArgs> B, const FrameGeom g)
{
    const VBlock vb = batch_decode(B.h);
    const SplatArgs& a = B.m[vb.model];
    const float4* __restrict__ surfels = a.surfels; const float4* __restrict__ rays = a.rays; unsigned long long* __restrict__ keys = a.keys;
    uchar4* __restrict__ image = a.image; float4* __restrict__ vertexConf = a.vertexConf; float4* __restrict__ normalRad = a.normalRad;
    unsigned short* __restrict__ time16 = a.time16;
    const int cols = g.cols, rows = g.rows;
    const cf_cam cam = g.cam;
    const int q = vb.bid * kB + threadIdx.x;
    const bool fill = a.fill.depth_filt != nullptr;
    bool covered = false, sample = false, timed = false;
    if (q < cols * rows) {
        const int py = q / cols, px = q - py * cols;
        const unsigned long long k = keys[q];
        keys[q] = kEmptyKey;
        uchar4 img = make_uchar4(0, 0, 0, 0);
        float4 vc = make_float4(0, 0, 0, 0), nrad = make_float4(0, 0, 0, 0);
        unsigned short t16 = 0;
        if (k != kEmptyKey) {
            const unsigned id = (unsigned)k;
            const float4 pc = surfels[id * 3], ct = surfels[id * 3 + 1], nr = surfels[id * 3 + 2];
            SplatSetup s;
            splat_setup(pc, ct, nr, a.t_inv, cam, cols, rows, a.maxDepth, a.confThreshold, a.time, a.maxTime, a.timeDelta, s);
            float z;
            splat_fragment(s, rays, cols, px, py, a.maxDepth, z);
            const f3 col = decode_color(ct.x);
            img = make_uchar4((unsigned char)glsl_round(col.x * 255.0f), (unsigned char)glsl_round(col.y * 255.0f),
                              (unsigned char)glsl_round(col.z * 255.0f), 255);
            const float fx_ = (float)px + 0.5f, fy_ = (float)py + 0.5f;
            vc = make_float4((fx_ - cam.cx) * z * (1.f / cam.fx), (fy_ - cam.cy) * z * (1.f / cam.fy), z, pc.w);
            nrad = make_float4(s.n.x, s.n.y, s.n.z, s.rad);
            t16 = (unsigned short)(unsigned)ct.z;
        }
        if constexpr (kMode == kSplatDepth) {
            reinterpret_cast<float*>(vertexConf)[q] = vc.z;
        } else {
            image[q] = img; vertexConf[q] = vc; normalRad[q] = nrad; time16[q] = t16;
        }
        timed = t16 > 0;
        if (fill) {
            fill_in_px(vc, nrad, img, a.fill.depth_filt, reinterpret_cast<const uchar4*>(a.fill.rgba), cols, rows, px, py, q, cam.cx, cam.cy,
                       a.fill.inv_fx, a.fill.inv_fy, a.fill.pass_geom, a.fill.pass_rgb, reinterpret_cast<float4*>(a.fill.fill_vertex),
                       reinterpret_cast<float4*>(a.fill.fill_normal), reinterpret_cast<uchar4*>(a.fill.fill_image));
            const int dw = cols / 20, dh = rows / 20;
            sample = dw > 0 && dh > 0 && fill_ratio_sample(py, dh, rows) && fill_ratio_sample(px, dw, cols);
            covered = sample && img.x > 0 && img.y > 0 && img.z > 0;
        }
    }
    if constexpr (kMode == kSplatCount) {
        const int n_timed = __syncthreads_count(timed ? 1 : 0);
        if (threadIdx.x == 0 && n_timed > 0) atomicAdd(a.fill.out2, (unsigned)n_timed);
        return;
    }
    if (!fill) return;
    const unsigned samples = (unsigned)((cols / 20) * (rows / 20));
    unsigned total = 0;
    if (a.fill.sample_blocks > 0) {
        const int n_covered = __syncthreads_count(covered ? 1 : 0);
        if (!__syncthreads_or(sample ? 1 : 0) || threadIdx.x != 0) return;
        const unsigned long long old = atomicAdd(a.fill.acc, ((unsigned long long)(unsigned)n_covered << 32) | 1ull);
        if ((unsigned)old != (unsigned)a.fill.sample_blocks - 1u) return;
        total = (unsigned)(old >> 32) + (unsigned)n_covered;
        __hip_atomic_store(a.fill.acc, 0ull, __ATOMIC_RELAXED, __HIP_MEMORY_SCOPE_AGENT);
    } else if (vb.bid != 0 || threadIdx.x != 0)
        return;
    a.fill.out2[0] = total; a.fill.out2[1] = samples;
    if (a.fill.out2_host) { a.fill.out2_host[0] = total; a.fill.out2_host[1] = samples; }
}

__global__ void __launch_bounds__(1024) fill_ratio_kernel(const uchar4* __restrict__ pimg, int cols, int rows, unsigned* __restrict__ out2,
                                                          unsigned* __restrict__ out2_host)
{
    const int dw = cols / 20, dh = rows / 20;
    unsigned s = 0;
    for (int k = threadIdx.x; k < dw * dh; k += 1024) {
        const int j = k / dw, i = k - j * dw;
        const int sx = nearest_texel(((float)i + 0.5f) / (float)dw, cols), sy = nearest_texel(((float)j + 0.5f) / (float)dh, rows);
        const uchar4 p = pimg[sy * cols + sx];
        s += (p.x > 0 && p.y > 0 && p.z > 0) ? 1u : 0u;
    }
    for (int o = 32; o > 0; o >>= 1) s += __shfl_xor((int)s, o, 64);
    __shared__ unsigned w[16];
    if ((threadIdx.x & 63) == 0) w[threadIdx.x >> 6] = s;
    __syncthreads();
    if (threadIdx.x == 0) {
        unsigned t = 0;
        for (int k = 0; k < 16; k++) t += w[k];
        out2[0] = t; out2[1] = (unsigned)(dw * dh);
        if (out2_host) { out2_host[0] = t; out2_host[1] = (unsigned)(dw * dh); }
    }
}

void launch_combined_predict_batch(hipStream_t s, const SplatPassArgs* items, int n_items, cf_cam cam, int cols, int rows, int mode)
{
    const FrameGeom g{cam, cols, rows};
    for_each_batch<SplatArgs>(items, n_items,
        [](const SplatPassArgs& h, SplatArgs& a) {
            a = SplatArgs{reinterpret_cast<const float4*>(h.surfels), h.count, mat4_from(h.t_inv), h.maxDepth, h.confThreshold, h.time, h.maxTime,
                          h.timeDelta, reinterpret_cast<const float4*>(h.rays), h.keys, reinterpret_cast<uchar4*>(h.image),
                          reinterpret_cast<float4*>(h.vertexConf), reinterpret_cast<float4*>(h.normalRad), h.time16, h.fill};
            return gridFor(4ll * h.count_bound);
        },
        [&](Batch<SplatArgs>& B, int* blocks, int nb, const SplatPassArgs*) {
            if (const int grid = batch_layout(B, blocks, nb)) splat_raster_kernel<<<grid, kB, 0, s>>>(B, g);
            for (int k = 0; k < nb; k++) blocks[k] = gridFor((long long)cols * rows);
            const int grid = batch_layout(B, blocks, nb);
            if (mode == kSplatCount) splat_resolve_kernel<kSplatCount><<<grid, kB, 0, s>>>(B, g);
            else if (mode == kSplatDepth) splat_resolve_kernel<kSplatDepth><<<grid, kB, 0, s>>>(B, g);
            else splat_resolve_kernel<kSplatFull><<<grid, kB, 0, s>>>(B, g);
        });
}
void launch_splat_rays(hipStream_t s, cf_cam cam, int cols, int rows, float* rays)
{
    splat_rays_kernel<<<gridFor((long long)cols * rows), kB, 0, s>>>(cam, cols, rows, reinterpret_cast<float4*>(rays));
}
void launch_fill_in(hipStream_t s, const float* pv, const float* pn, const uint8_t* pimg, const float* depth, const uint8_t* rgba, int cols,
                    int rows, cf_cam cam, float inv_fx, float inv_fy, int pass_geom, int pass_rgb, float* ov, float* on, uint8_t* oi)
{
    fill_in_kernel<<<gridFor((long long)cols * rows), kB, 0, s>>>(
        reinterpret_cast<const float4*>(pv), reinterpret_cast<const float4*>(pn), reinterpret_cast<const uchar4*>(pimg), depth,
        reinterpret_cast<const uchar4*>(rgba), cols, rows, cam.cx, cam.cy, inv_fx, inv_fy, pass_geom, pass_rgb, reinterpret_cast<float4*>(ov),
        reinterpret_cast<float4*>(on), reinterpret_cast<uchar4*>(oi));
}
void launch_fill_ratio(hipStream_t s, const uint8_t* pimg, int cols, int rows, unsigned* out2, unsigned* out2_host)
{
    fill_ratio_kernel<<<1, 1024, 0, s>>>(reinterpret_cast<const uchar4*>(pimg), cols, rows, out2, out2_host);
}

}
```

### co_fusion_amd/csrc/surfel.hip

```cpp
#include "surf_batch_dev.h"
#include "surf_scan_dev.h"
#include "surf_boot_dev.h"
#include "surf_index_dev.h"
#include "surf_splat_dev.h"
#include "surf_fuse_dev.h"
#include "surf_clean_dev.h"

namespace cf {

static_assert(sizeof(Batch<FuseArgs>) + 16 <= 4096 && sizeof(Batch<CleanArgs>) + 16 <= 4096 && sizeof(Batch<IndexArgs>) + sizeof(FrameGeom) <= 4096 &&
              sizeof(Batch<SplatArgs>) + sizeof(FrameGeom) <= 4096 && sizeof(Batch<ScanArgs>) <= 4096, "lower kSurfBatch");
static_assert(sizeof(Batch<IndexArgs>) + sizeof(FrameGeom) + sizeof(Batch<ScanArgs>) + 16 <= 4096 && sizeof(Batch<UpdateArgs>) + sizeof(Batch<ScanArgs>) + 16 <= 4096,
              "the side-by-side launches carry two batches' arguments in one 4 KB kernel-argument segment");

__global__ void __launch_bounds__(kB) update_blocksums_kernel(const Batch<UpdateArgs> U, const Batch<ScanArgs> S, int u_blocks)
{
    const int b = (int)blockIdx.x;
    if (b < u_blocks) update_body(U, b);
    else scan_block_sums_body(S, b - u_blocks);
}
__global__ void __launch_bounds__(kB) indexsplat_scatter_kernel(const Batch<IndexArgs> I, const FrameGeom g, const Batch<ScanArgs> S, int i_blocks)
{
    const int b = (int)blockIdx.x;
    if (b < i_blocks) index_splat_body(I, g, b);
    else scan_scatter_body(S, b - i_blocks);
}

bool launch_update_compaction_index_keys(hipStream_t s, const UpdatePassArgs* up, const ScanPassArgs* sc, const IndexPassArgs* ix, int n, cf_cam cam, int cols,
                                         int rows)
{
    if (n <= 0 || n > kSurfBatch) return false;
    Batch<UpdateArgs> U; Batch<ScanArgs> S; Batch<IndexArgs> I;
    int ub[kSurfBatch], sb[kSurfBatch], ib[kSurfBatch];
    for (int k = 0; k < n; k++) {
        U.m[k] = update_args(up[k]); ub[k] = update_blocks(up[k]);
        S.m[k] = scan_args(sc[k]); sb[k] = scan_blocks(sc[k]);
        if (sb[k] == 0) return false;
        I.m[k] = index_args(ix[k]); ib[k] = index_blocks(ix[k]);
    }
    const int ug = batch_layout(U, ub, n), sg = batch_layout(S, sb, n), ig = batch_layout(I, ib, n);
    const FrameGeom g{cam, cols, rows};
    update_blocksums_kernel<<<ug + sg, kB, 0, s>>>(U, S, ug);
    indexsplat_scatter_kernel<<<ig + sg, kB, 0, s>>>(I, g, S, ig);
    return true;
}

}
```

### co_fusion_amd/facade.py

```python
from __future__ import annotations

import ctypes as C
import os

import numpy as np
import torch

from . import lib as _libmod
from .api import Profile


class Config(C.Structure):
    _fields_ = [("width", C.c_int), ("height", C.c_int), ("fx", C.c_float), ("fy", C.c_float), ("cx", C.c_float), ("cy", C.c_float),
                ("device", C.c_int), ("max_surfels", C.c_int), ("max_models", C.c_int), ("conf_global_init", C.c_float),
                ("conf_object_init", C.c_float), ("depth_cutoff", C.c_float), ("icp_weight", C.c_float),
                ("outlier_coefficient", C.c_float), ("fast_odom", C.c_int), ("so3", C.c_int), ("frame_to_frame_rgb", C.c_int),
                ("pyramid", C.c_int), ("rgb_only", C.c_int), ("model_spawn_offset", C.c_uint), ("enable_multiple_models", C.c_int),
                ("enable_pose_logging", C.c_int), ("rank", C.c_int), ("world", C.c_int), ("device_frames_complete", C.c_int),
                ("mid_frame_predict", C.c_int), ("shard_background", C.c_int), ("enqueue_threads", C.c_int),
                ("colocate_background", C.c_int), ("reloc", C.c_int), ("early_index_maps", C.c_int), ("time_delta", C.c_int)]


class RedetectCandidate(C.Structure):
    _fields_ = [("id", C.c_uint), ("projected", C.c_uint32), ("occluded", C.c_uint32), ("seen_through", C.c_uint32), ("agree", C.c_uint32),
# ... 192 lines not shown
        self.lib.cofusion_set_mesh_max_voxels.argtypes = [C.c_void_p, C.c_uint64]
        self._check(self.lib.cofusion_set_mesh_max_voxels(self.h, int(max_voxels)))

    def set_export_segmentation(self, prefix):
        self._check(self.lib.cofusion_set_export_segmentation(self.h, str(prefix or "").encode()))

    def render(self, pose=None, intrinsics=None, size=None, near=0.0, far=0.0, background_mode=2, object_mode=4, flags=0,
               depth=False, labels=False, as_torch=False):
        from .render import make_view
        view = None
        if pose is not None or intrinsics is not None or size is not None or near or far:
            cur = self.model_info(0)["pose"] if pose is None else pose
            fx, fy, cx, cy = intrinsics if intrinsics is not None else (self.cfg.fx, self.cfg.fy, self.cfg.cx, self.cfg.cy)
            w, h = size if size is not None else (self.width, self.height)
            view = make_view(cur, fx, fy, cx, cy, w, h, near, far)
        w, h = (view.width, view.height) if view is not None else (self.width, self.height)
        vref = C.byref(view) if view is not None else None
        if as_torch:
            r = C.c_void_p(); d = C.c_void_p(); lb = C.c_void_p()
            self._check(self.lib.cofusion_render_device(self.h, vref, int(background_mode), int(object_mode), int(flags), C.byref(r),
                                                        C.byref(d), C.byref(lb)))
            out = [(r, torch.empty((h, w, 4), dtype=torch.uint8, device=self.device))]
            if depth:
                out.append((d, torch.empty((h, w), dtype=torch.float32, device=self.device)))
            if labels:
                out.append((lb, torch.empty((h, w), dtype=torch.uint8, device=self.device)))
            ctx = self._ctx()
            for src, t in out:
                assert self.abi.cf_memcpy_d2d_async(ctx, C.c_void_p(t.data_ptr()), src, C.c_uint64(t.numel() * t.element_size())) == 0
            assert self.abi.cf_synchronize(ctx) == 0
            res = [t for _, t in out]
        else:
            rgba = np.empty((h, w, 4), np.uint8)
            dep = np.empty((h, w), np.float32) if depth else None
            lab = np.empty((h, w), np.uint8) if labels else None
            ptr = lambda a: a.ctypes.data_as(C.c_void_p) if a is not None else None
            self._check(self.lib.cofusion_render(self.h, vref, int(background_mode), int(object_mode), int(flags), ptr(rgba), ptr(dep),
                                                 ptr(lab)))
            res = [a for a in (rgba, dep, lab) if a is not None]
        return res[0] if len(res) == 1 else tuple(res)

    def set_export_views(self, prefix, labels=False, normals=False, viewport=False):
        which = (1 if labels else 0) | (2 if normals else 0) | (4 if viewport else 0)
        self._check(self.lib.cofusion_set_export_views(self.h, str(prefix or "").encode(), which))

    def set_export_async(self, on=True, workers=2, slots=8):
        self._check(self.lib.cofusion_set_export_async(self.h, int(bool(on)), int(workers), int(slots)))

    def export_flush(self):
        self._check(self.lib.cofusion_export_flush(self.h))

    def export_stats(self, timing=False):
        im, by, stl, n = C.c_uint64(), C.c_uint64(), C.c_uint64(), C.c_uint64()
        ms = C.c_double()
        self._check(self.lib.cofusion_export_stats(self.h, C.byref(im), C.byref(by), C.byref(stl), C.byref(ms), C.byref(n), int(bool(timing))))
        return dict(images=im.value, bytes=by.value, stalls=stl.value, device_ms=ms.value, device_images=n.value)

    def export_poses(self, prefix):
        n = self.lib.cofusion_export_poses(self.h, str(prefix).encode())
        if n < 0:
            raise CoFusionError(self.lib.cofusion_last_error().decode())
        return n

    def close(self):
        if getattr(self, "h", None):
            if getattr(self, "_owned", True):
                self.lib.cofusion_destroy(self.h)
            self.h = None

    def __del__(self):
        try:
            self.close()
        except Exception:
            pass

    def set_crf(self, unary_weight_error=75.0, unary_k_error=0.0375, threshold_new=5.5, weight_appearance=7.0, weight_smoothness=2.0,
                sigma_rgb=10.0, sigma_depth=0.9, sigma_pos=1.8, min_rel_size_new=0.015, max_rel_size_new=0.4, iterations=10):
        f = C.c_float
        self._check(self.lib.cofusion_set_crf(self.h, f(unary_weight_error), f(unary_k_error), f(threshold_new), f(weight_appearance),
                                              f(weight_smoothness), f(sigma_rgb), f(sigma_depth), f(sigma_pos), f(min_rel_size_new),
                                              f(max_rel_size_new), C.c_uint(iterations)))

    def set_seg_early(self, on=True):
        self._check(self.lib.cofusion_set_seg_early(self.h, 1 if on else 0))

    def process_frame(self, depth, rgb, mask=None, in_pose=None, timestamp=0):
        d = np.ascontiguousarray(depth, np.float32); c = np.ascontiguousarray(rgb, np.uint8)
        m = None if mask is None else np.ascontiguousarray(mask, np.uint8)
        p = None if in_pose is None else np.ascontiguousarray(in_pose, np.float32).reshape(16)
        self._check(self.lib.cofusion_process_frame(self.h, C.c_int64(timestamp), c.ctypes.data_as(C.c_void_p), d.ctypes.data_as(C.c_void_p),
                                                    None if m is None else m.ctypes.data_as(C.c_void_p),
                                                    None if p is None else p.ctypes.data_as(C.c_void_p)))

    def process_frame_device(self, depth_t, rgba_t, in_pose=None, timestamp=0, mask=None):
        p = None if in_pose is None else np.ascontiguousarray(in_pose, np.float32).reshape(16)
        if mask is not None:
            _check_mask_tensor(mask, depth_t)
            self._check(self.lib.cofusion_process_frame_device_masked(self.h, C.c_int64(timestamp), C.c_void_p(depth_t.data_ptr()),
                                                                      C.c_void_p(rgba_t.data_ptr()), C.c_void_p(mask.data_ptr()),
                                                                      None if p is None else p.ctypes.data_as(C.c_void_p)))
            return
        self._check(self.lib.cofusion_process_frame_device(self.h, C.c_int64(timestamp), C.c_void_p(depth_t.data_ptr()),
                                                           C.c_void_p(rgba_t.data_ptr()),
                                                           None if p is None else p.ctypes.data_as(C.c_void_p)))

    def process_frame_device_ptr(self, depth_ptr, rgba_ptr, mask_ptr=None, in_pose=None, timestamp=0):
        p = None if in_pose is None else np.ascontiguousarray(in_pose, np.float32).reshape(16)
        self._check(self.lib.cofusion_process_frame_device_masked(self.h, C.c_int64(timestamp), C.c_void_p(depth_ptr), C.c_void_p(rgba_ptr),
                                                                  C.c_void_p(mask_ptr) if mask_ptr else None,
                                                                  None if p is None else p.ctypes.data_as(C.c_void_p)))

    @property
    def num_models(self):
        return self.lib.cofusion_num_models(self.h)

    @property
    def tick(self):
        return self.lib.cofusion_tick(self.h)

    @property
    def lost(self):
        return bool(self.lib.cofusion_is_lost(self.h))

    def set_relocalisation(self, on=True, n_ferns=500, fern_threshold=0.3095, photo_threshold=115.0, min_age=300, seed=0, capacity=1024):
        self._check(self.lib.cofusion_set_relocalisation(self.h, int(bool(on)), int(n_ferns), C.c_float(fern_threshold), C.c_float(photo_threshold),
                                                         int(min_age), C.c_uint64(seed), int(capacity)))

    def reloc_stats(self):
        k = C.c_int(); c = C.c_int(); r = C.c_int(); f = C.c_int()
        self._check(self.lib.cofusion_reloc_stats(self.h, C.byref(k), C.byref(c), C.byref(r), C.byref(f)))
        return dict(keyframes=k.value, last_closest=c.value, recoveries=r.value, database_full=bool(f.value))

    def deform_background(self, src, dst, src_time, dst_time=None, pin=False, sample_rate=25000):
        from . import deform as _deform
        s = np.ascontiguousarray(src, np.float32).reshape(-1, 3); d = np.ascontiguousarray(dst, np.float32).reshape(-1, 3)
        ts = np.ascontiguousarray(src_time, np.float32).reshape(-1)
        td = None if dst_time is None else np.ascontiguousarray(dst_time, np.float32).reshape(-1)
        assert len(s) == len(d) == len(ts) and (td is None or len(td) == len(s))
        res = _deform.Result(); nodes = C.c_int()
        vp = lambda a: None if a is None else a.ctypes.data_as(C.c_void_p)
        self._check(self.lib.cofusion_deform_background(self.h, vp(s), vp(d), vp(ts), vp(td), len(s), int(bool(pin)), int(sample_rate), C.byref(res),
                                                        C.byref(nodes)))
        out = {k: getattr(res, k) for k in _deform.RESULT_FIELDS}
        for k in ("optimised", "accepted", "failed"):
            out[k] = bool(out[k])
        out["nodes"] = nodes.value
        return out

    def set_loop_closure(self, on=True, sample_rate=25000):
        self._check(self.lib.cofusion_set_loop_closure(self.h, int(bool(on)), int(sample_rate)))

    def loop_stats(self):
        from . import deform as _deform

        class _Stats(C.Structure):
            _fields_ = [(k, C.c_int32) for k in ("gated", "candidates", "fern_accepts", "optimised", "accepted", "failed", "last_keyframe",
                                                "last_keyframe_time", "last_nodes", "last_tick")] + [("last", _deform.Result)]
        s = _Stats()
        self._check(self.lib.cofusion_loop_stats(self.h, C.byref(s)))
        out = {k: getattr(s, k) for k, _ in _Stats._fields_[:-1]}
        last = {k: getattr(s.last, k) for k in _deform.RESULT_FIELDS}
        for k in ("optimised", "accepted", "failed"):
            last[k] = bool(last[k])
        out["last"] = last
        return out

    def set_local_loop_closure(self, on=True, sample_rate=5000, icp_count_thresh=40000, icp_err_thresh=5e-5, cov_thresh=1e-5,
                               min_inactive_pixels=None):
        f = C.c_float
        self._check(self.lib.cofusion_set_local_loop_closure(self.h, int(bool(on)), int(sample_rate), int(icp_count_thresh), f(icp_err_thresh),
                                                             f(cov_thresh), -1 if min_inactive_pixels is None else int(min_inactive_pixels)))

    def local_loop_stats(self):
        from . import deform as _deform
        ints = ("examined", "skipped_by_gate", "tracker_accepts", "optimised", "accepted", "failed", "last_nodes", "last_constraints",
                "last_pinned", "last_tick", "deforms", "last_deform_time")

        class _Stats(C.Structure):
            _fields_ = ([(k, C.c_int32) for k in ints] + [("last_covered", C.c_uint32), ("last_tracker_accepted", C.c_int32),
                        ("last_icp_error", C.c_float), ("last_icp_count", C.c_float), ("last_max_covariance", C.c_double),
                        ("last_est_pose", C.c_float * 16), ("last", _deform.Result)])
        assert C.sizeof(_Stats) == 168
        s = _Stats()
        self._check(self.lib.cofusion_local_loop_stats(self.h, C.byref(s)))
        out = {k: getattr(s, k) for k in ints + ("last_covered", "last_icp_error", "last_icp_count", "last_max_covariance")}
        out["last_pinned"] = bool(out["last_pinned"]); out["last_tracker_accepted"] = bool(s.last_tracker_accepted)
        out["last_est_pose"] = np.array(list(s.last_est_pose), np.float32).reshape(4, 4)
        last = {k: getattr(s.last, k) for k in _deform.RESULT_FIELDS}
        for k in ("optimised", "accepted", "failed"):
            last[k] = bool(last[k])
        out["last"] = last
        return out

    def set_relative_constraints(self, on=True):
        self._check(self.lib.cofusion_set_relative_constraints(self.h, int(bool(on))))

    def add_relative_constraints(self, src, dst, src_time, dst_time):
        src = np.ascontiguousarray(src, np.float32).reshape(-1, 3); dst = np.ascontiguousarray(dst, np.float32).reshape(-1, 3)
        ts = np.ascontiguousarray(src_time, np.float32).reshape(-1); td = np.ascontiguousarray(dst_time, np.float32).reshape(-1)
        assert len(src) == len(dst) == len(ts) == len(td)
        vp = lambda a: a.ctypes.data_as(C.c_void_p)
        self._check(self.lib.cofusion_add_relative_constraints(self.h, vp(src), vp(dst), vp(ts), vp(td), len(src)))

    def relative_constraints(self):
        n = C.c_int()
        out = np.zeros((128, 8), np.float32)
        self._check(self.lib.cofusion_relative_constraints(self.h, out.ctypes.data_as(C.c_void_p), 128, C.byref(n)))
        return out[:n.value].copy()

    def local_closure(self):
        found, rows, pinned, ldt, n = C.c_int(), C.c_int(), C.c_int(), C.c_int(), C.c_int()
        src = np.zeros((1536, 3), np.float32); dst = np.zeros((1536, 3), np.float32); tm = np.zeros(1536, np.float32); tt = np.zeros(1536, np.float32)
        nodes = np.zeros((1024, 4), np.float32); params = np.zeros((1024, 12), np.float32)
        vp = lambda a: a.ctypes.data_as(C.c_void_p)
        self._check(self.lib.cofusion_local_closure_download(self.h, C.byref(found), C.byref(rows), C.byref(pinned), C.byref(ldt), vp(src), vp(dst), vp(tm),
                                                             vp(tt), 1536, C.byref(n), vp(nodes), vp(params), 1024))
        if not found.value:
            return None
        r, c = rows.value, rows.value // (2 if pinned.value else 1)
        return dict(pinned=bool(pinned.value), last_deform_time=ldt.value, src=src[:r].copy(), dst=dst[:r].copy(), time=tm[:r].copy(),
                    target_time=tt[:c].copy(), nodes=nodes[:n.value].copy(), params=params[:n.value].copy())

    def relative_stats(self):
        class _Stats(C.Structure):
            _fields_ = [("appended", C.c_int64), ("overwritten", C.c_int64), ("stored", C.c_int32), ("used_by_last_closure", C.c_int32),
                        ("last_picked", C.c_int32), ("pad", C.c_int32)]
        assert C.sizeof(_Stats) == 32
        s = _Stats()
        self._check(self.lib.cofusion_relative_stats(self.h, C.byref(s)))
        return {k: getattr(s, k) for k, _ in _Stats._fields_[:-1]}

    def set_redetection(self, on=True, min_fit=0.5, min_cover=0.044, depth_tol=0.10, max_candidates=8, keep_min_surfels=4000,
                        keep_conf_threshold=0.3):
        f = C.c_float
        self._check(self.lib.cofusion_set_redetection(self.h, int(bool(on)), f(min_fit), f(min_cover), f(depth_tol), int(max_candidates),
                                                      int(keep_min_surfels), f(keep_conf_threshold)))

    def redetect_stats(self):
        a = C.c_int(); r = C.c_int(); i = C.c_int()
        self._check(self.lib.cofusion_redetect_stats(self.h, C.byref(a), C.byref(r), C.byref(i)))
        return dict(attempts=a.value, reactivations=r.value, last_id=i.value)

    def redetect_last(self):
        cap = 16
        out = (RedetectCandidate * cap)()
        n = C.c_int(); px = C.c_uint32(); w = C.c_int()
        self._check(self.lib.cofusion_redetect_last(self.h, out, cap, C.byref(n), C.byref(px), C.byref(w)))
        cands = [{k: getattr(out[q], k) for k, _ in RedetectCandidate._fields_} for q in range(min(n.value, cap))]
        for c in cands:
            c["eligible"] = bool(c["eligible"])
        return dict(label_pixels=px.value, winner=w.value, candidates=cands)

    def set_redetection_search(self, on=True, iterations=10, min_colour=-1.0, max_registered=2):
        self._check(self.lib.cofusion_set_redetection_search(self.h, int(bool(on)), int(iterations), C.c_float(min_colour), int(max_registered)))

    def redetect_search_last(self):
        cap = 16
        out = (RedetectSearchCandidate * cap)()
        n = C.c_int(); w = C.c_int(); a = C.c_int()
        self._check(self.lib.cofusion_redetect_search_last(self.h, out, cap, C.byref(n), C.byref(w), C.byref(a)))
        cands = [{k: getattr(out[q], k) for k, _ in RedetectSearchCandidate._fields_} for q in range(min(n.value, cap))]
        for c in cands:
            for k in ("registered", "converged", "eligible"):
                c[k] = bool(c[k])
        return dict(winner=w.value, attempts=a.value, candidates=cands)

    @property
    def num_inactive_models(self):
        return self.lib.cofusion_num_inactive_models(self.h)

    def model_info(self, index):
        mid = C.c_uint(); cnt = C.c_uint(); conf = C.c_float(); pose = (C.c_float * 16)()
        self._check(self.lib.cofusion_model_info(self.h, index, C.byref(mid), C.byref(cnt), pose, C.byref(conf)))
        return dict(id=mid.value, count=cnt.value, pose=np.array(pose, np.float32).reshape(4, 4), conf_threshold=conf.value)

    def model_cull_box(self, index):
        b = (C.c_int * 4)()
        self._check(self.lib.cofusion_model_cull_box(self.h, index, b))
        return list(b)

    def model_level0_visited(self, index):
        a = C.c_uint64(); b = C.c_uint64()
        self._check(self.lib.cofusion_model_level0_visited(self.h, index, C.byref(a), C.byref(b)))
        return int(a.value), int(b.value)

    def model_icp_stats(self, index):
        e = C.c_float(); c = C.c_float()
        self._check(self.lib.cofusion_model_icp_stats(self.h, index, C.byref(e), C.byref(c)))
        return e.value, c.value

    def model_tracking_inputs(self, index):
        H, W = self.height, self.width
        v = np.empty((H, W, 4), np.float32); n = np.empty((H, W, 4), np.float32); img = np.empty((H, W, 4), np.uint8)
        self._check(self.lib.cofusion_model_tracking_inputs(self.h, index, v.ctypes.data_as(C.c_void_p), n.ctypes.data_as(C.c_void_p),
                                                            img.ctypes.data_as(C.c_void_p)))
        return v, n, img

    def set_gn_mode(self, mode):
        assert self.abi.cf_set_gn_mode(self._ctx(), int(mode)) == 0

    def set_extent_culling(self, on=True):
        assert self.abi.cf_set_extent_culling(self._ctx(), int(bool(on))) == 0

    def model_download(self, index):
        n = self.model_info(index)["count"]
        out = np.zeros((max(n, 1), 12), np.float32)
        c = C.c_uint32()
        self._check(self.lib.cofusion_model_download(self.h, index, out.ctypes.data_as(C.c_void_p), n, C.byref(c)))
        return out[:n]

    def mask(self):
        ptr = self.lib.cofusion_mask_device(self.h)
        host = np.empty(self.width * self.height, np.uint8)
        ctx = C.c_void_p(self.lib.cofusion_context(self.h))
        rc = self.abi.cf_memcpy_d2h(ctx, host.ctypes.data_as(C.c_void_p), C.c_void_p(ptr), C.c_uint64(host.size))
        if rc != 0:
            raise CoFusionError("mask readback failed")
        return host.reshape(self.height, self.width)

    def _ctx(self):
        return C.c_void_p(self.lib.cofusion_context(self.h))

    def set_icp_launch(self, threads, ppt):
        assert self.abi.cf_set_icp_launch(self._ctx(), threads, ppt) == 0

    def set_icp_arith(self, mode):
        assert self.abi.cf_set_icp_arith(self._ctx(), {"product": 0, "gram": 1, "reference": 2}.get(mode, mode)) == 0

    def profile_enable(self, on=True):
        assert self.abi.cf_profile_enable(self._ctx(), int(on)) == 0

    def profile_read(self, reset=True):
        p = Profile()
        assert self.abi.cf_profile_read(self._ctx(), C.byref(p), int(reset)) == 0
        return p


class CoFusionGroup:

    def __init__(self, n_sequences, width=640, height=480, fx=528.0, fy=528.0, cx=320.0, cy=240.0, device=0, **kw):
        if not torch.cuda.is_available():
            raise CoFusionError("no GPU visible: the Co-Fusion hot path has no CPU fallback")
        self.lib = _libmod.load_host()
        cfg = _make_config(self.lib, width, height, fx, fy, cx, cy, device, kw)
        self.device = torch.device("cuda", device)
        torch.cuda.set_device(self.device)
        self.n = int(n_sequences)
        self.g = C.c_void_p()
        if self.lib.cofusion_group_create(C.byref(cfg), self.n, C.byref(self.g)) != 0:
            raise CoFusionError(f"cofusion_group_create: {self.lib.cofusion_last_error().decode()}")
        self._check(self.lib.cofusion_group_set_stream(self.g, C.c_void_p(torch.cuda.current_stream(self.device).cuda_stream)))
        self.sequences = [CoFusion(width, height, fx, fy, cx, cy, device, _borrowed=self.lib.cofusion_group_sequence(self.g, s), **kw)
                          for s in range(self.n)]

    def _check(self, rc):
        if rc != 0:
            raise CoFusionError(f"cofusion error {rc}: {self.lib.cofusion_last_error().decode()}")

    def set_stream(self, stream):
        ptr = stream.cuda_stream if hasattr(stream, "cuda_stream") else int(stream)
        self._check(self.lib.cofusion_group_set_stream(self.g, C.c_void_p(ptr)))

    def process_frames(self, depths, rgbs, masks=None, timestamp=0):
        keep = [np.ascontiguousarray(d, np.float32) for d in depths] + [np.ascontiguousarray(r, np.uint8) for r in rgbs]
        mk = [None if (masks is None or m is None) else np.ascontiguousarray(m, np.uint8) for m in (masks or [None] * self.n)]
        P = C.c_void_p * self.n
        ts = (C.c_int64 * self.n)(*([timestamp] * self.n))
        self._check(self.lib.cofusion_group_process_frames(
            self.g, ts, P(*[r.ctypes.data for r in keep[self.n:]]), P(*[d.ctypes.data for d in keep[:self.n]]),
            P(*[None if m is None else m.ctypes.data for m in mk]) if masks is not None else None))

    def process_frames_device(self, depth_ts, rgba_ts, timestamp=0, masks=None):
        P = C.c_void_p * self.n
        ts = (C.c_int64 * self.n)(*([timestamp] * self.n))
        if masks is not None:
            for m, d in zip(masks, depth_ts):
                if m is not None:
                    _check_mask_tensor(m, d)
            self._check(self.lib.cofusion_group_process_frames_device_masked(
                self.g, ts, P(*[t.data_ptr() for t in depth_ts]), P(*[t.data_ptr() for t in rgba_ts]),
                P(*[None if m is None else m.data_ptr() for m in masks])))
            return
        self._check(self.lib.cofusion_group_process_frames_device(self.g, ts, P(*[t.data_ptr() for t in depth_ts]),
                                                                  P(*[t.data_ptr() for t in rgba_ts])))

    def close(self):
        if getattr(self, "g", None):
            for s in self.sequences:
                s.h = None
            self.lib.cofusion_group_destroy(self.g)
            self.g = None

    def __del__(self):
        try:
            self.close()
        except Exception:
            pass
```

### co_fusion_amd/lib.py

```python
from __future__ import annotations

import ctypes as C
import os
import subprocess

_HERE = os.path.dirname(os.path.abspath(__file__))
_LIB_DIR = os.environ.get("CF_LIB_DIR") or os.path.join(_HERE, "lib")
LIB_PATH = os.environ.get("CF_HIP_LIB") or os.path.join(_LIB_DIR, "libcofusion_hip.so")

SYMBOLS = [
    "cf_create", "cf_destroy", "cf_last_error", "cf_set_stream", "cf_use_own_stream", "cf_get_stream", "cf_synchronize", "cf_fork", "cf_main", "cf_join", "cf_join_lane", "cf_thread_lane", "cf_mark", "cf_event_wait_host", "cf_fork_after", "cf_malloc",
    "cf_free", "cf_memcpy_h2d", "cf_memcpy_d2h", "cf_malloc_host", "cf_free_host", "cf_memcpy_h2d_async", "cf_memcpy_d2h_async", "cf_memcpy_d2d_async", "cf_rgb_to_rgba", "cf_create_vmap", "cf_create_nmap", "cf_copy_maps", "cf_resize_map",
    "cf_transform_maps", "cf_vertices_to_depth", "cf_pyrdown_gauss_f32", "cf_pyrdown_gauss_u8",
    "cf_rgba_to_intensity", "cf_sobel", "cf_project_cloud", "cf_icp_step", "cf_icp_step_band", "cf_rgb_residual", "cf_rgb_step",
    "cf_so3_step", "cf_gn_solve_step", "cf_so3_prealign_step", "cf_rgb_records_step","cf_odom_create", "cf_odom_destroy", "cf_odom_init_icp_model", "cf_odom_init_rgb_model",
    "cf_odom_init_rgb", "cf_odom_init_models_batch", "cf_odom_init_models_batch_frames", "cf_odom_init_models_batch_select", "cf_model_fill_ratio_device", "cf_odom_init_first_rgb", "cf_odom_init_icp", "cf_odom_init_icp_maps", "cf_odom_get_incremental_transformation",
    "cf_odom_track_batch_async", "cf_odom_fetch_result", "cf_odom_get_covariance", "cf_odom_bind_frame_maps", "cf_odom_share_frame_maps", "cf_odom_set_culling", "cf_odom_set_band", "cf_set_collective", "cf_model_predict_indices_sharded", "cf_odom_buffer",
    "cf_bilateral", "cf_model_create", "cf_model_destroy", "cf_model_initialise", "cf_model_count",
    "cf_model_predict_indices", "cf_model_index_keys", "cf_model_index_resolve", "cf_model_combined_predict", "cf_model_predict_inactive", "cf_model_synthesize_depth", "cf_model_prefetch_fill_ratio", "cf_model_perform_fill_in", "cf_model_requires_fill_in",
    "cf_model_fuse", "cf_model_clean", "cf_models_frame_passes", "cf_models_preindex", "cf_model_download_map", "cf_model_upload_map", "cf_model_buffer",
    "cf_set_extent_culling", "cf_model_extents_unknown",
    "cf_redetect_score", "cf_redetect_timing", "cf_relabel",
    "cf_redetect_frame_moments", "cf_redetect_model_moments", "cf_redetect_register_step", "cf_redetect_register",
    "cf_fusion_weight", "cf_seg_create", "cf_seg_destroy", "cf_seg_slic", "cf_seg_crf", "cf_seg_sums", "cf_seg_infer", "cf_seg_early", "cf_seg_run_batch", "cf_seg_fetch", "cf_seg_publish_poses", "cf_seg_fetch_poses",
    "cf_seg_labels", "cf_seg_buffer", "cf_seg_create_masks", "cf_seg_masks", "cf_seg_masks_batch", "cf_seg_new_mask_value",
    "cf_depth_pyramid", "cf_set_icp_launch", "cf_set_icp_arith", "cf_get_icp_arith", "cf_set_gn_mode", "cf_profile_enable", "cf_profile_read", "cf_odom_bench_icp", "cf_odom_level0_visited", "cf_odom_last_launch_shape",
    "cf_rccl_unique_id", "cf_rccl_init", "cf_rccl_allreduce", "cf_rccl_broadcast", "cf_rccl_info", "cf_rccl_destroy",
    "cf_render_create", "cf_render_destroy", "cf_render", "cf_render_palette",
    "cf_ferns_table", "cf_ferns_create", "cf_ferns_destroy", "cf_ferns_get_table", "cf_ferns_encode", "cf_ferns_search", "cf_ferns_append", "cf_ferns_add_async",
    "cf_ferns_relocalise", "cf_ferns_count", "cf_ferns_download", "cf_ferns_last_search",
    "cf_frame_decoder_create", "cf_frame_decoder_destroy", "cf_frame_decoder_slot", "cf_frame_decoder_submit", "cf_frame_decoder_acquire", "cf_frame_decoder_timing",
    "cf_frame_decoder_enable_images", "cf_frame_decoder_image_slot", "cf_frame_decoder_submit_images", "cf_frame_decoder_acquire_mask", "cf_frame_decoder_image_timing",
    "cf_png_encoder_create", "cf_png_encoder_destroy", "cf_png_encoder_submit", "cf_png_encoder_acquire", "cf_png_encoder_timing",
    "cf_deform_create", "cf_deform_destroy", "cf_deform_default_thresholds", "cf_deform_sample", "cf_deform_set_nodes", "cf_deform_weights", "cf_deform_assemble",
    "cf_deform_iterate", "cf_deform_optimise", "cf_deform_apply", "cf_deform_apply_poses", "cf_deform_download", "cf_deform_weights_device",
    "cf_deform_create_sized", "cf_deform_assemble_local", "cf_deform_iterate_local", "cf_deform_optimise_local",
    "cf_deform_enable_relative", "cf_deform_set_relative", "cf_deform_set_relative_device", "cf_deform_pick_relative", "cf_deform_download_relative",
    "cf_deform_download_out", "cf_deform_bench_relative_y",
    "cf_ferns_gate_async", "cf_ferns_gate_wait", "cf_ferns_constraints", "cf_ferns_find_frame", "cf_ferns_constraint_buffers", "cf_ferns_keyframe_buffers",
    "cf_local_loop_create", "cf_local_loop_destroy", "cf_local_loop_constraints_async", "cf_local_loop_wait", "cf_local_loop_constraint_buffers",
    "cf_local_loop_target_times",
    "cf_mesh_create", "cf_mesh_destroy", "cf_mesh_default_grid", "cf_mesh_accumulate", "cf_mesh_extract", "cf_mesh_download", "cf_mesh_grid_download",
    "cf_mesh_extract_grid", "cf_mesh_timing",
]


def build(verbose: bool = False) -> str:
    cmd = ["make", "-C", os.path.join(_HERE, "csrc"), "-j8"]
    if not verbose:
        cmd.insert(1, "-s")
    subprocess.check_call(cmd)
    cmd = ["make", "-C", os.path.join(_HERE, "host")]
    if not verbose:
        cmd.insert(1, "-s")
    subprocess.check_call(cmd)
    return LIB_PATH


HOST_LIB_PATH = os.path.join(_LIB_DIR, "libcofusion.so")
HOST_SYMBOLS = [
    "cofusion_default_config", "cofusion_create", "cofusion_destroy", "cofusion_last_error", "cofusion_set_stream",
    "cofusion_process_frame", "cofusion_process_frame_device", "cofusion_process_frame_device_masked", "cofusion_group_process_frames_device_masked", "cofusion_num_models", "cofusion_tick", "cofusion_model_info",
    "cofusion_model_download", "cofusion_model_icp_stats", "cofusion_model_cull_box", "cofusion_model_level0_visited", "cofusion_model_tracking_inputs", "cofusion_mask_device", "cofusion_context", "cofusion_set_crf", "cofusion_set_seg_early",
    "cofusion_save_ply", "cofusion_export_poses", "cofusion_set_export_segmentation", "cofusion_klg_open", "cofusion_klg_next", "cofusion_klg_set_reference_compatible", "cofusion_klg_close",
    "cofusion_klg_create", "cofusion_klg_write", "cofusion_klg_finish", "cofusion_debug_phase_ms", "cofusion_set_allreduce", "cofusion_set_allreduce_device", "cofusion_group_create", "cofusion_group_destroy", "cofusion_group_size", "cofusion_group_sequence", "cofusion_group_set_stream", "cofusion_group_process_frames", "cofusion_group_process_frames_device", "cofusion_rccl_unique_id", "cofusion_init_rccl", "cofusion_broadcast", "cofusion_model_owned", "cofusion_is_lost",
    "cofusion_render", "cofusion_render_device", "cofusion_set_export_views", "cofusion_set_export_async", "cofusion_export_flush", "cofusion_export_stats", "cofusion_set_relocalisation", "cofusion_reloc_stats", "cofusion_deform_background", "cofusion_set_loop_closure", "cofusion_loop_stats", "cofusion_set_local_loop_closure", "cofusion_local_loop_stats",
    "cofusion_set_relative_constraints", "cofusion_add_relative_constraints", "cofusion_relative_constraints", "cofusion_relative_stats", "cofusion_local_closure_download",
    "cofusion_set_redetection", "cofusion_redetect_stats", "cofusion_redetect_last", "cofusion_num_inactive_models",
    "cofusion_set_redetection_search", "cofusion_redetect_search_last",
    "cofusion_klg_player_open", "cofusion_klg_player_next", "cofusion_klg_player_process", "cofusion_klg_player_rewind", "cofusion_klg_player_set_limits", "cofusion_klg_player_close",
    "cofusion_jpeg_front", "cofusion_jpeg_finish_host", "cofusion_klg_prefetch_open", "cofusion_klg_prefetch_next", "cofusion_klg_prefetch_rewind", "cofusion_klg_prefetch_close",
    "cofusion_image_reader_open", "cofusion_image_reader_next", "cofusion_image_reader_rewind", "cofusion_image_reader_close",
    "cofusion_image_player_open", "cofusion_image_player_next", "cofusion_image_player_process", "cofusion_image_player_rewind", "cofusion_image_player_set_limits",
    "cofusion_image_player_times", "cofusion_image_player_close",
    "cofusion_image_prefetch_open", "cofusion_image_prefetch_next", "cofusion_image_prefetch_rewind", "cofusion_image_prefetch_close",
    "cofusion_save_mesh", "cofusion_model_mesh", "cofusion_set_mesh_max_voxels", "cofusion_write_mesh_ply",
    "cofusion_png_decode", "cofusion_png_finish_host", "cofusion_exr_decode", "cofusion_exr_finish_host", "cofusion_ppm_decode",
]
_host = None


def load_host() -> C.CDLL:
    global _host
    if _host is None:
        load()
        if not os.path.exists(HOST_LIB_PATH):
            raise RuntimeError(f"{HOST_LIB_PATH} is missing: run __graft_entry__.build()")
        _host = C.CDLL(HOST_LIB_PATH)
        _host.cofusion_last_error.restype = C.c_char_p
        _host.cofusion_mask_device.restype = C.c_void_p
        _host.cofusion_context.restype = C.c_void_p
        _host.cofusion_group_sequence.restype = C.c_void_p
    return _host


_lib = None


def load() -> C.CDLL:
    global _lib
    if _lib is None:
        if not os.path.exists(LIB_PATH):
            raise RuntimeError(
                f"{LIB_PATH} is missing: build it with `python -c 'import __graft_entry__ as g; g.build()'` "
                "(there is no CPU fallback for the product path)")
        import torch
        _lib = C.CDLL(LIB_PATH)
        _lib.cf_last_error.restype = C.c_char_p
        _lib.cf_get_stream.restype = C.c_void_p
        pp = C.POINTER(C.c_void_p)
        _lib.cf_odom_init_models_batch_select.restype = C.c_int
        _lib.cf_odom_init_models_batch_select.argtypes = [C.c_void_p, pp, C.c_int, pp, pp, pp, pp, pp, pp, pp, C.c_float,
                                                          C.POINTER(C.POINTER(C.c_float)), pp]
        _lib.cf_models_frame_passes.restype = C.c_int
        _lib.cf_models_frame_passes.argtypes = [C.c_void_p, C.c_void_p, C.c_int, C.c_float, C.c_float, C.c_int]
        _lib.cf_models_preindex.restype = C.c_int
        _lib.cf_models_preindex.argtypes = [C.c_void_p, C.c_void_p, C.c_int, C.c_float, C.c_int]
    return _lib
```

### co_fusion_amd/model.py

```python
from __future__ import annotations

import ctypes as C

import numpy as np
import torch

from .api import Context, Odometry, _f, _p

SURFEL = 12
TIME_DELTA = 2 ** 31 // 2 - 1

class ModelPass(C.Structure):
    _fields_ = [("model", C.c_void_p), ("pose", C.POINTER(C.c_float)), ("rgba", C.c_void_p), ("mask", C.c_void_p), ("depth_raw", C.c_void_p),
                ("depth_filtered", C.c_void_p), ("do_fuse", C.c_int), ("time", C.c_int), ("fuse_max_depth", C.c_float), ("weighting", C.c_float),
                ("mask_id", C.c_int), ("conf_threshold", C.c_float), ("fill_in", C.c_int), ("passthrough_geom", C.c_int),
                ("passthrough_rgb", C.c_int)]


class ModelPreindex(C.Structure):
    _fields_ = [("model", C.c_void_p), ("odom", C.c_void_p), ("time", C.c_int)]


def frame_passes(ctx: Context, items, depth_cutoff, outlier_coeff, time_delta=None):
    n = len(items)
    arr = (ModelPass * n)()
    keep = []
    for a, it in zip(arr, items):
        pose = _f(np.asarray(it["pose"], np.float32).reshape(16))
        keep.append(pose)
        a.model = it["model"].h
        a.pose = C.cast(pose, C.POINTER(C.c_float))
        a.rgba, a.mask = _p(it["rgba"]), _p(it.get("mask"))
        a.depth_raw, a.depth_filtered = _p(it.get("depth_raw")), _p(it["depth_filt"])
        a.do_fuse = int(it.get("do_fuse", 1))
        a.time = int(it["time"])
        a.fuse_max_depth = float(it.get("fuse_max_depth", depth_cutoff))
        a.weighting = float(it.get("weighting", 1.0))
        a.mask_id = int(it.get("mask_id", 0))
        a.conf_threshold = float(it["conf_threshold"])
        a.fill_in, a.passthrough_geom, a.passthrough_rgb = int(it.get("fill_in", 0)), int(it.get("passthrough_geom", 0)), int(it.get("passthrough_rgb", 0))
    ctx._check(ctx.lib.cf_models_frame_passes(ctx.h, arr, n, C.c_float(depth_cutoff), C.c_float(outlier_coeff),
                                              int(TIME_DELTA if time_delta is None else time_delta)))


def preindex(ctx: Context, items, depth_cutoff, time_delta=None):
    n = len(items)
    arr = (ModelPreindex * n)()
    for a, (m, od, time) in zip(arr, items):
        a.model, a.odom, a.time = m.h, od.h, int(time)
    ctx._check(ctx.lib.cf_models_preindex(ctx.h, arr, n, C.c_float(depth_cutoff), int(TIME_DELTA if time_delta is None else time_delta)))


def set_extent_culling(ctx: Context, on=True):
    ctx._check(ctx.lib.cf_set_extent_culling(ctx.h, int(bool(on))))


_BUF = {0: (np.uint32, 1), 1: (np.float32, 4), 2: (np.float32, 4), 3: (np.float32, 4), 4: (np.uint8, 4), 5: (np.float32, 4),
        6: (np.float32, 4), 7: (np.uint16, 1), 8: (np.float32, 4), 9: (np.float32, 4), 10: (np.uint8, 4),
        15: (np.uint8, 4), 16: (np.float32, 4), 17: (np.float32, 4), 18: (np.uint16, 1)}


def bilateral(ctx: Context, depth, max_d):
    rows, cols = depth.shape
    out = ctx.empty((rows, cols))
    ctx._check(ctx.lib.cf_bilateral(ctx.h, _p(depth), cols, rows, C.c_float(max_d), _p(out)))
    return out


def fusion_weight(ctx: Context, pose, last_pose, mult):
    ctx.lib.cf_fusion_weight.restype = C.c_float
    return float(ctx.lib.cf_fusion_weight(_f(np.asarray(pose, np.float32).reshape(16)), _f(np.asarray(last_pose, np.float32).reshape(16)),
                                          C.c_float(mult)))


class Model:
    def __init__(self, ctx: Context, max_surfels=1 << 20):
        self.ctx = ctx
        self.h = C.c_void_p()
        ctx._check(ctx.lib.cf_model_create(ctx.h, int(max_surfels), C.byref(self.h)))

    def close(self):
        if getattr(self, "h", None) and self.ctx.h:
            self.ctx.lib.cf_model_destroy(self.h)
        self.h = None

    def __del__(self):
        try:
            self.close()
        except Exception:
            pass

    def _pose(self, pose):
        return _f(np.asarray(pose, np.float32).reshape(16))

    def initialise(self, rgba, depth_raw, depth_filt, time, max_depth):
        self.ctx._check(self.ctx.lib.cf_model_initialise(self.h, _p(rgba), _p(depth_raw), _p(depth_filt), time, C.c_float(max_depth)))

    def count(self):
        c = C.c_uint32()
        self.ctx._check(self.ctx.lib.cf_model_count(self.h, C.byref(c)))
        return c.value

    def predict_indices(self, pose, time, max_depth, time_delta=TIME_DELTA):
        self.ctx._check(self.ctx.lib.cf_model_predict_indices(self.h, self._pose(pose), time, C.c_float(max_depth), time_delta))

    def index_keys(self, pose, time, max_depth, surfel_begin, surfel_end, time_delta=TIME_DELTA):
        keys = torch.empty((self.ctx.height, self.ctx.width), dtype=torch.int64, device=self.ctx.device)
        self.ctx._check(self.ctx.lib.cf_model_index_keys(self.h, self._pose(pose), time, C.c_float(max_depth), time_delta,
                                                         int(surfel_begin), int(surfel_end), C.c_void_p(keys.data_ptr())))
        return keys

    def index_resolve(self, pose, keys):
        self.ctx._check(self.ctx.lib.cf_model_index_resolve(self.h, self._pose(pose), C.c_void_p(keys.data_ptr())))

    def combined_predict(self, pose, max_depth, conf_threshold, time, max_time, time_delta=TIME_DELTA):
        self.ctx._check(self.ctx.lib.cf_model_combined_predict(self.h, self._pose(pose), C.c_float(max_depth), C.c_float(conf_threshold),
                                                               time, max_time, time_delta))

    def predict_inactive(self, pose, max_depth, conf_threshold, max_time, time_delta):
        self.ctx._check(self.ctx.lib.cf_model_predict_inactive(self.h, self._pose(pose), C.c_float(max_depth), C.c_float(conf_threshold),
                                                               int(max_time), int(time_delta)))

    def inactive_covered(self):
        ptr, nbytes = self.tensor(19)
        host = np.empty(1, np.uint32)
        self.ctx._check(self.ctx.lib.cf_memcpy_d2h(self.ctx.h, host.ctypes.data_as(C.c_void_p), C.c_void_p(ptr), C.c_uint64(nbytes)))
        return int(host[0])

    def synthesize_depth(self, pose, max_depth, conf_threshold, time, max_time, time_delta, out):
        assert out.is_cuda and out.is_contiguous() and out.element_size() == 4 and out.numel() == self.ctx.width * self.ctx.height
        self.ctx._check(self.ctx.lib.cf_model_synthesize_depth(self.h, self._pose(pose), C.c_float(max_depth), C.c_float(conf_threshold),
                                                               int(time), int(max_time), int(time_delta), _p(out)))

    def perform_fill_in(self, rgba, depth_filt, pass_geom=False, pass_rgb=False):
        self.ctx._check(self.ctx.lib.cf_model_perform_fill_in(self.h, _p(rgba), _p(depth_filt), int(pass_geom), int(pass_rgb)))

    def prefetch_fill_ratio(self):
        self.ctx._check(self.ctx.lib.cf_model_prefetch_fill_ratio(self.h))

    def fill_counts_device(self):
        ptr = C.c_void_p()
        self.ctx._check(self.ctx.lib.cf_model_fill_ratio_device(self.h, C.byref(ptr)))
        if not ptr.value:
            return None
        host = np.empty(2, np.uint32)
        self.ctx._check(self.ctx.lib.cf_memcpy_d2h(self.ctx.h, host.ctypes.data_as(C.c_void_p), ptr, C.c_uint64(8)))
        return host

    def requires_fill_in(self, ratio=0.75):
        out = C.c_int()
        self.ctx._check(self.ctx.lib.cf_model_requires_fill_in(self.h, C.c_float(ratio), C.byref(out)))
        return bool(out.value)

    def fuse(self, pose, time, rgba, mask, depth_raw, depth_filt, max_depth, weighting, mask_id):
        self.ctx._check(self.ctx.lib.cf_model_fuse(self.h, self._pose(pose), time, _p(rgba), _p(mask), _p(depth_raw), _p(depth_filt),
                                                   C.c_float(max_depth), C.c_float(weighting), mask_id))

    def clean(self, pose, time, conf_threshold, outlier_coeff, depth_filt, mask, mask_id, time_delta=TIME_DELTA):
        c = C.c_uint32()
        self.ctx._check(self.ctx.lib.cf_model_clean(self.h, self._pose(pose), time, C.c_float(conf_threshold), C.c_float(outlier_coeff),
                                                    time_delta, _p(depth_filt), _p(mask), mask_id, C.byref(c)))
        return c.value

    def download_map(self):
        n = self.count()
        out = np.zeros((max(n, 1), SURFEL), np.float32)
        c = C.c_uint32()
        self.ctx._check(self.ctx.lib.cf_model_download_map(self.h, out.ctypes.data_as(C.c_void_p), n, C.byref(c)))
        return out[:n]

    def upload_map(self, surfels):
        s = np.ascontiguousarray(surfels, np.float32).reshape(-1, SURFEL)
        self.ctx._check(self.ctx.lib.cf_model_upload_map(self.h, s.ctypes.data_as(C.c_void_p), s.shape[0]))

    def extents_unknown(self):
        self.ctx._check(self.ctx.lib.cf_model_extents_unknown(self.h))

    def tensor(self, which):
        ptr = C.c_void_p(); nbytes = C.c_uint64()
        self.ctx._check(self.ctx.lib.cf_model_buffer(self.h, which, C.byref(ptr), C.byref(nbytes)))
        return ptr.value, nbytes.value

    def buffer(self, which):
        ptr, nbytes = self.tensor(which)
        host = np.empty(nbytes, np.uint8)
        if nbytes:
            self.ctx._check(self.ctx.lib.cf_memcpy_d2h(self.ctx.h, host.ctypes.data_as(C.c_void_p), C.c_void_p(ptr), C.c_uint64(nbytes)))
        h, w = self.ctx.height, self.ctx.width
        if which in (11, 12):
            return host.view(np.float32).reshape(-1, SURFEL)
        if which == 13:
            return host.view(np.float32).reshape(h, w, 8)
        if which == 14:
            return host.view(np.uint64).reshape(h, w)
        dt, ch = _BUF[which]
        a = host.view(dt)
        return a.reshape(h, w, ch) if ch > 1 else a.reshape(h, w)


class _DevView:

    def __init__(self, ptr):
        self._ptr = ptr
        self.is_cuda = True

    def is_contiguous(self):
        return True

    def data_ptr(self):
        return self._ptr
```

### include/cofusion_hip.h

```cpp
#ifndef COFUSION_HIP_H_
#define COFUSION_HIP_H_

#include <stdint.h>

#ifdef __cplusplus
extern "C" {
#endif

#define CF_OK 0
#define CF_EINVAL (-1)
#define CF_EHIP (-2)
#define CF_ENOMEM (-3)
#define CF_ESTATE (-4)

#define CF_NUM_PYRS 3
#define CF_SE3_WORDS 32
#define CF_SO3_WORDS 16
#define CF_FIX_ICP 32
#define CF_FIX_RGB_MAX 32
static inline int CF_FIX_RGB_BITS(float sigma)
{
    union { float f; uint32_t u; } v;
    int F;
    if (sigma == -1.0f || !(sigma >= 2.0f)) return 8;
    v.f = sigma;
    F = 8 + 2 * ((int)((v.u >> 23) & 255u) - 127);
    return F > CF_FIX_RGB_MAX ? CF_FIX_RGB_MAX : F;
}
#define CF_FIX_SO3 12

typedef struct cf_ctx cf_ctx;
typedef struct cf_odom cf_odom;
typedef struct cf_model cf_model;

typedef struct { float fx, fy, cx, cy; } cf_cam;

typedef struct {
    float x, y, z, conf;
    float colour24, unused, init_time, last_time;
    float nx, ny, nz, radius;
} cf_surfel;
#ifdef __cplusplus
static_assert(sizeof(cf_surfel) == 48, "surfel record is 3 x float4");
#else
_Static_assert(sizeof(cf_surfel) == 48, "surfel record is 3 x float4");
#endif

typedef struct {
    int16_t zero_x, zero_y;
    int16_t one_x, one_y;
    float diff;
    int32_t valid;
} cf_dataterm;

typedef struct {
    int width, height;
    float fx, fy, cx, cy;
    int device;
    int max_models;
    int max_surfels;
} cf_config;

int cf_create(const cf_config *cfg, cf_ctx **out);
void cf_destroy(cf_ctx *ctx);
const char *cf_last_error(const cf_ctx *ctx);
int cf_set_stream(cf_ctx *ctx, void *hip_stream);
int cf_use_own_stream(cf_ctx *ctx);
void *cf_get_stream(cf_ctx *ctx);
int cf_synchronize(cf_ctx *ctx);
int cf_fork(cf_ctx *ctx, int lane);
int cf_main(cf_ctx *ctx);
int cf_join(cf_ctx *ctx);
int cf_join_lane(cf_ctx *ctx, int lane);
int cf_thread_lane(cf_ctx *ctx, int lane);
int cf_mark(cf_ctx *ctx, int slot);
int cf_event_wait_host(cf_ctx *ctx, int slot);
int cf_fork_after(cf_ctx *ctx, int lane, int slot);
int cf_malloc(cf_ctx *ctx, uint64_t bytes, void **dptr);
int cf_free(cf_ctx *ctx, void *dptr);
int cf_memcpy_h2d(cf_ctx *ctx, void *dst, const void *src, uint64_t bytes);
int cf_memcpy_d2h(cf_ctx *ctx, void *dst, const void *src, uint64_t bytes);
int cf_malloc_host(cf_ctx *ctx, uint64_t bytes, void **hptr);
int cf_free_host(cf_ctx *ctx, void *hptr);
int cf_memcpy_h2d_async(cf_ctx *ctx, void *dst, const void *src_pinned, uint64_t bytes);
int cf_memcpy_d2h_async(cf_ctx *ctx, void *dst_pinned, const void *src, uint64_t bytes);
int cf_memcpy_d2d_async(cf_ctx *ctx, void *dst, const void *src, uint64_t bytes);
int cf_rgb_to_rgba(cf_ctx *ctx, const uint8_t *rgb_dev, int cols, int rows, uint8_t *rgba_dev);

int cf_create_vmap(cf_ctx *ctx, const float *depth, int cols, int rows, cf_cam intr, float depth_cutoff, float *vmap);
int cf_create_nmap(cf_ctx *ctx, const float *vmap, int cols, int rows, float *nmap);
int cf_copy_maps(cf_ctx *ctx, const float *vertex4, const float *normal4, int cols, int rows, float *vmap, float *nmap);
int cf_resize_map(cf_ctx *ctx, const float *in, int in_cols, int in_rows, float *out, int normalize);
int cf_transform_maps(cf_ctx *ctx, float *vmap, float *nmap, int cols, int rows, const float R[9], const float t[3]);
int cf_vertices_to_depth(cf_ctx *ctx, const float *vertex4, int cols, int rows, float cutoff, float *depth);
int cf_pyrdown_gauss_f32(cf_ctx *ctx, const float *src, int src_cols, int src_rows, float *dst);
int cf_pyrdown_gauss_u8(cf_ctx *ctx, const uint8_t *src, int src_cols, int src_rows, uint8_t *dst);
int cf_rgba_to_intensity(cf_ctx *ctx, const uint8_t *rgba, int cols, int rows, uint8_t *dst);
int cf_sobel(cf_ctx *ctx, const uint8_t *src, int cols, int rows, int16_t *dx, int16_t *dy);
int cf_project_cloud(cf_ctx *ctx, const float *depth, int cols, int rows, cf_cam intr_level, float *cloud3);

int cf_icp_step(cf_ctx *ctx, const float Rcurr[9], const float tcurr[3], const float *vmap_curr,
                const float *nmap_curr, const float Rprev_inv[9], const float tprev[3], cf_cam intr,
                const float *vmap_g_prev, const float *nmap_g_prev, float dist_thres, float angle_thres,
                int cols, int rows, float *A_host, float *b_host, float *residual_host, int64_t *sums_host,
                float *err_surface);
int cf_icp_step_band(cf_ctx *ctx, const float Rcurr[9], const float tcurr[3], const float *vmap_curr,
                     const float *nmap_curr, const float Rprev_inv[9], const float tprev[3], cf_cam intr,
                     const float *vmap_g_prev, const float *nmap_g_prev, float dist_thres, float angle_thres,
                     int cols, int rows, int row_begin, int row_end, float *A_host, float *b_host,
                     float *residual_host, int64_t *sums_host, float *err_surface);
int cf_rgb_residual(cf_ctx *ctx, float min_scale, const int16_t *dIdx, const int16_t *dIdy, const float *last_depth,
                    const float *next_depth, const uint8_t *last_image, const uint8_t *next_image,
                    cf_dataterm *corres, float max_depth_delta, const float kt[3], const float krkinv[9],
                    int cols, int rows, int *sigma_sum_host, int *count_host);
int cf_rgb_step(cf_ctx *ctx, const cf_dataterm *corres, float sigma, const float *cloud3, float fx, float fy,
                const int16_t *dIdx, const int16_t *dIdy, float sobel_scale, int cols, int rows, float *A_host,
                float *b_host, int64_t *sums_host);
int cf_so3_step(cf_ctx *ctx, const uint8_t *last_image, const uint8_t *next_image, const float image_basis[9],
                const float kinv[9], const float krlr[9], int cols, int rows, float *A_host, float *b_host,
                float *residual_host, int64_t *sums_host);

typedef struct {
    int rgb_only, pyramid, fast_odom, so3;
    float icp_weight;
} cf_track_opts;
typedef struct {
    float last_icp_error, last_icp_count, last_rgb_error, last_rgb_count, last_so3_error, last_so3_count;
    double lastA[36], lastb[6];
    int so3_iterations;
    int fault;
    int cull_box[4];
} cf_track_stats;

int cf_odom_create(cf_ctx *ctx, cf_odom **out);
void cf_odom_destroy(cf_odom *od);
int cf_odom_init_icp_model(cf_odom *od, const float *pred_vertex4, const float *pred_normal4, const float pose[16]);
int cf_odom_init_rgb_model(cf_odom *od, const uint8_t *pred_rgba);
int cf_odom_init_rgb(cf_odom *od, const uint8_t *rgba);
int cf_odom_init_first_rgb(cf_odom *od, const uint8_t *rgba);
int cf_odom_init_models_batch(cf_ctx *ctx, cf_odom *const *ods, int n, const float *const *pred_vertex4,
                              const float *const *pred_normal4, const uint8_t *const *pred_rgba, const float *const *poses ,
                              const uint8_t *frame_rgba);
int cf_odom_init_models_batch_frames(cf_ctx *ctx, cf_odom *const *ods, int n, const float *const *pred_vertex4,
                                     const float *const *pred_normal4, const uint8_t *const *pred_rgba, const float *const *poses ,
                                     const uint8_t *const *frame_rgba );
int cf_odom_init_models_batch_select(cf_ctx *ctx, cf_odom *const *ods, int n, const float *const *pred_vertex4,
                                     const float *const *pred_normal4, const uint8_t *const *pred_rgba,
                                     const float *const *alt_vertex4, const float *const *alt_normal4, const uint8_t *const *alt_rgba,
                                     const uint32_t *const *fill_counts, float ratio, const float *const *poses ,
                                     const uint8_t *const *frame_rgba );
int cf_odom_init_icp(cf_odom *od, const float *const depth_pyr[CF_NUM_PYRS], float depth_cutoff);
int cf_odom_get_incremental_transformation(cf_odom *od, float trans[3], float rot[9], const cf_track_opts *opts,
                                           float *icp_err_surface, cf_track_stats *stats);
int cf_odom_track_batch_async(cf_ctx *ctx, cf_odom *const *ods, int n, const float *const *poses_in ,
                              const cf_track_opts *opts, float *const *icp_err_surfaces );
int cf_odom_fetch_result(cf_odom *od, float trans[3], float rot[9], cf_track_stats *stats);
int cf_odom_get_covariance(const cf_track_stats *stats, double cov[36]);

typedef struct {
    cf_cam intr;
    int32_t width, height;
    int32_t icp, rgb, rgbOnly;
    float icpWeight;
    float Rprev[9], tprev[3], Rprev_inv[9], Rcurr[9], tcurr[3];
    double resultRt[16];
    float krkInv[9], kt[3];
    float lastRGBError;
    int32_t level_done, solves;
    float residual[2];
    float cull_z[2];
    float pose_inv[16];
    cf_track_stats stats;
} cf_gn_state;
typedef struct {
    int64_t icp_acc[64 * 32];
    int64_t rgb_acc[64 * 32];
    cf_gn_state state;
    cf_gn_state twin;
    uint32_t hot[48];
} cf_gn_system;
int cf_gn_solve_step(cf_ctx *ctx, int n, cf_gn_system *systems, int next_level, int last_of_level, int icp_fix);
typedef struct {
    const uint8_t *last_next_image;
    const uint8_t *next_image;
    cf_gn_state state_in;
    cf_gn_state state_out;
    uint32_t hot[48];
    uint64_t sync[418];
} cf_so3_system;
int cf_so3_prealign_step(cf_ctx *ctx, int n, cf_so3_system *systems, int do_so3, int first_level);
typedef struct {
    const uint8_t *cand;
    const float *next_depth, *last_depth;
    const uint8_t *last_image, *next_image;
    const float *cloud;
    const int16_t *dIdx, *dIdy;
    int32_t no_counts;
    int32_t ranged;
    uint32_t res_range[2];
    int32_t res_blocks;
    uint64_t *records;
    uint32_t *slot_counts;
    int64_t count_seed[64], sigma_seed[64];
    int64_t count_total, sigma_total;
    int64_t rgb_sums[32];
    cf_gn_state state;
    cf_gn_state twin;
    uint32_t hot[48];
} cf_rgb_system;
int cf_rgb_records_step(cf_ctx *ctx, int n, cf_rgb_system *systems, int cols, int rows, float max_depth_delta, float sobel_scale,
                        float fx, float fy, int next_level, int last_of_level);
int cf_odom_level0_visited(cf_odom *od, uint64_t *icp_pixels, uint64_t *residual_pixels);
int cf_odom_last_launch_shape(cf_odom *od, int icp_blocks[3], int residual_blocks[3], int *icp_blocks_err);
int cf_odom_set_culling(cf_odom *od, int on);
typedef int (*cf_collective_fn)(void *user, int op, void *dev_buf, uint64_t words, void *hip_stream);
int cf_set_collective(cf_ctx *ctx, cf_collective_fn fn, void *user);
int cf_odom_set_band(cf_odom *od, int row_begin, int row_end, int add_counts);
#define CF_RCCL_ID_BYTES 128
int cf_rccl_unique_id(void *id128);
int cf_rccl_init(cf_ctx *ctx, const void *id128, int rank, int world);
int cf_rccl_allreduce(cf_ctx *ctx, void *dev_buf, uint64_t words, int op, void *hip_stream);
int cf_rccl_broadcast(cf_ctx *ctx, void *dev_buf, uint64_t bytes, int root, void *hip_stream);
int cf_rccl_info(const cf_ctx *ctx, int *rank, int *world, int *rccl_version);
int cf_rccl_destroy(cf_ctx *ctx);
int cf_odom_bind_frame_maps(cf_odom *od, const float *const vmaps[CF_NUM_PYRS], const float *const nmaps[CF_NUM_PYRS]);
int cf_odom_share_frame_maps(cf_odom *od, cf_odom *owner);
int cf_odom_buffer(cf_odom *od, int which, int level, void **dptr, uint64_t *bytes);
int cf_odom_init_icp_maps(cf_odom *od, const float *vertex4, const float *normal4);
int cf_depth_pyramid(cf_ctx *ctx, const float *depth_filtered, int cols, int rows, float *l1, float *l2);

int cf_bilateral(cf_ctx *ctx, const float *depth, int cols, int rows, float maxD, float *out);

int cf_model_create(cf_ctx *ctx, int max_surfels, cf_model **out);
void cf_model_destroy(cf_model *m);
int cf_model_initialise(cf_model *m, const uint8_t *rgba, const float *depth_raw, const float *depth_filtered, int time,
                        float maxDepth);
int cf_model_count(cf_model *m, uint32_t *count);
int cf_model_predict_indices(cf_model *m, const float pose[16], int time, float maxDepth, int timeDelta);
int cf_model_index_keys(cf_model *m, const float pose[16], int time, float maxDepth, int timeDelta, uint32_t surfel_begin,
                        uint32_t surfel_end, uint64_t *keys_dev);
int cf_model_index_resolve(cf_model *m, const float pose[16], uint64_t *keys_dev);
int cf_model_predict_indices_sharded(cf_model *m, const float pose[16], int time, float maxDepth, int timeDelta, int shard, int nshards);
int cf_model_combined_predict(cf_model *m, const float pose[16], float maxDepth, float confThreshold, int time, int maxTime,
                              int timeDelta);
int cf_model_predict_inactive(cf_model *m, const float pose[16], float maxDepth, float confThreshold, int maxTime, int timeDelta);
int cf_model_synthesize_depth(cf_model *m, const float pose[16], float maxDepth, float confThreshold, int time, int maxTime, int timeDelta,
                              float *depth_out_dev);
int cf_model_prefetch_fill_ratio(cf_model *m);
int cf_model_perform_fill_in(cf_model *m, const uint8_t *rgba, const float *depth_filtered, int passthrough_geom,
                             int passthrough_rgb);
int cf_model_requires_fill_in(cf_model *m, float ratio, int *out);
int cf_model_fill_ratio_device(cf_model *m, const uint32_t **counts_dev);
int cf_model_fuse(cf_model *m, const float pose[16], int time, const uint8_t *rgba, const uint8_t *mask, const float *depth_raw,
                  const float *depth_filtered, float maxDepth, float weighting, int maskID);
int cf_model_clean(cf_model *m, const float pose[16], int time, float confThreshold, float outlierCoeff, int timeDelta,
                   const float *depth_filtered, const uint8_t *mask, int maskID, uint32_t *count_out);
typedef struct {
    cf_model *model;
    const float *pose;
    const uint8_t *rgba, *mask;
    const float *depth_raw, *depth_filtered;
    int do_fuse;
    int time;
    float fuse_max_depth;
    float weighting;
    int mask_id;
    float conf_threshold;
    int fill_in, passthrough_geom, passthrough_rgb;
} cf_model_pass;
int cf_models_frame_passes(cf_ctx *ctx, const cf_model_pass *items, int n, float depth_cutoff, float outlier_coeff, int time_delta);
typedef struct {
    cf_model *model;
    const cf_odom *odom;
    int time;
} cf_model_preindex;
int cf_models_preindex(cf_ctx *ctx, const cf_model_preindex *items, int n, float depth_cutoff, int time_delta);
int cf_model_download_map(cf_model *m, float *host_surfels, uint32_t capacity, uint32_t *count);
int cf_model_upload_map(cf_model *m, const float *host_surfels, uint32_t count);
int cf_model_buffer(cf_model *m, int which, void **dptr, uint64_t *bytes);
int cf_set_extent_culling(cf_ctx *ctx, int on);
int cf_model_extents_unknown(cf_model *m);
typedef struct { uint32_t projected, occluded, seen_through, agree, agree_on_label, covered; } cf_redetect_counts;
typedef struct {
    cf_model *model;
    float pose[16];
    float conf_threshold;
} cf_redetect_candidate;
typedef struct {
    const float *depth;
    const uint8_t *label;
    int cols, rows;
    cf_cam cam;
    int new_label;
    float depth_cutoff, depth_tol;
} cf_redetect_frame;
int cf_redetect_score(cf_ctx *ctx, const cf_redetect_candidate *candidates, int n, const cf_redetect_frame *frame, cf_redetect_counts *counts ,
                      uint32_t *label_pixels);
int cf_redetect_timing(cf_ctx *ctx, int on, float *last_ms);
int cf_relabel(cf_ctx *ctx, uint8_t *label_dev, uint64_t n, int from, int to);
#define CF_REDETECT_BINS 512
int cf_redetect_frame_moments(cf_ctx *ctx, const cf_redetect_frame *frame, const uint8_t *rgba_dev, int64_t moments[4], uint32_t hist[CF_REDETECT_BINS]);
int cf_redetect_model_moments(cf_ctx *ctx, const cf_redetect_candidate *candidates, int n, const float dhat[3], int64_t *moments ,
                              uint32_t *hist );
int cf_redetect_register_step(cf_ctx *ctx, cf_model *model, float conf_threshold, const float cam_from_model[16], const cf_redetect_frame *frame,
                              const float centre[3], int64_t sums[32]);
typedef struct {
    int ok, iterations;
    uint32_t first_inliers, last_inliers;
    float rms;
    float cam_from_model[16];
} cf_redetect_registration;
int cf_redetect_register(cf_ctx *ctx, cf_model *model, float conf_threshold, const float seed_cam_from_model[16], const cf_redetect_frame *frame,
                         const float centre[3], int max_iterations, cf_redetect_registration *out);
float cf_fusion_weight(const float pose[16], const float lastPose[16], float weightMultiplier);

typedef struct cf_segmenter cf_segmenter;
int cf_seg_create(cf_ctx *ctx, cf_segmenter **out);
void cf_seg_destroy(cf_segmenter *s);
int cf_seg_slic(cf_segmenter *s, const uint8_t *rgba);
int cf_seg_crf(cf_segmenter *s, const float *unary_host, int L, const float *feat_smooth_host, const float *feat_app_host,
               float w_smooth, float w_app, int iterations, float *Q_host);
typedef struct {
    float unaryWeightError, unaryKError, unaryThresholdNew;
    float weightAppearance, weightSmoothness;
    float scaleFeaturesRGB, scaleFeaturesDepth, scaleFeaturesPos;
    float minRelSizeNew, maxRelSizeNew;
    int crfIterations;
} cf_seg_params;
#define CF_SEG_MAX_ENTRIES 256
typedef struct {
    uint32_t id, superPixelCount;
    float avgConfidence, depthMean, depthStd;
    int32_t top, right, bottom, left;
} cf_seg_model;
typedef struct {
    int32_t has_new_label, n_models;
    float depth_range;
    cf_seg_model model[CF_SEG_MAX_ENTRIES];
} cf_seg_result;
int cf_seg_sums(cf_segmenter *s, const float *depth, int n_models, const float *const *icp_err, const float *const *vertconf4,
                int64_t **sums_dev, uint64_t *sums_words);
int cf_seg_infer(cf_segmenter *s, const cf_seg_params *params, const uint8_t *rgba, int n_models, const uint32_t *model_ids,
                 uint32_t next_model_id, int allow_new, uint8_t *full_dev);
int cf_seg_fetch(cf_segmenter *s, cf_seg_result *out, uint8_t *low_map_host);
int cf_seg_early(cf_segmenter *s, const float *depth, const uint8_t *rgba, int n_models, const float *const *vertconf4,
                 const cf_seg_params *params);
typedef struct cf_seg_job {
    cf_segmenter *seg;
    const float *depth;
    int32_t n_models;
    const float *const *icp_err;
    const float *const *vertconf4;
    const uint8_t *rgba;
    const uint32_t *model_ids;
    uint32_t next_model_id;
    int32_t allow_new;
    uint8_t *full_dev;
} cf_seg_job;
int cf_seg_run_batch(cf_ctx *ctx, const cf_seg_params *params, const cf_seg_job *jobs, int n_jobs);
int cf_seg_publish_poses(cf_segmenter *s, int n_models, cf_odom *const *trackers);
int cf_seg_fetch_poses(cf_segmenter *s, int n_models, int64_t *words_host);
int cf_seg_labels(cf_segmenter *s, void **dptr, uint64_t *bytes);
int cf_seg_buffer(cf_segmenter *s, int which, void **dptr, uint64_t *bytes);
typedef struct cf_seg_mask_job {
    cf_segmenter *seg;
    const uint8_t *mask_dev;
    const float *depth_dev;
    int32_t n_models;
    const uint32_t *model_ids;
    uint32_t next_model_id;
    int32_t allow_new;
    const uint8_t *mapping;
    uint8_t *full_dev;
} cf_seg_mask_job;
int cf_seg_create_masks(cf_ctx *ctx, cf_segmenter **out);
int cf_seg_masks(const cf_seg_mask_job *job);
int cf_seg_masks_batch(cf_ctx *ctx, const cf_seg_mask_job *jobs, int n_jobs);
int cf_seg_new_mask_value(cf_segmenter *s, int *value);

int cf_set_gn_mode(cf_ctx *ctx, int mode);
int cf_set_icp_launch(cf_ctx *ctx, int threads, int pixels_per_thread);
#define CF_ICP_ARITH_PRODUCT 0
#define CF_ICP_ARITH_GRAM 1
#define CF_ICP_ARITH_REFERENCE 2
int cf_set_icp_arith(cf_ctx *ctx, int mode);
int cf_get_icp_arith(cf_ctx *ctx);

typedef struct cf_renderer cf_renderer;
#define CF_RENDER_MAX_ITEMS 256
#define CF_RENDER_MAX_COLOUR 8
#define CF_RENDER_UNSTABLE 1
#define CF_RENDER_WINDOW 2
#define CF_RENDER_PHONG 4
#define CF_RENDER_GREY 0
#define CF_RENDER_NORMALS 1
#define CF_RENDER_COLOUR 2
#define CF_RENDER_TIMES 3
#define CF_RENDER_LABEL 4
#define CF_RENDER_ITEM_MODE (-1)
#define CF_RENDER_RGBA 0
#define CF_RENDER_DEPTH 1
#define CF_RENDER_LABELS 2
typedef struct {
    float pose[16];
    float fx, fy, cx, cy;
    int width, height;
    float near_z, far_z;
    int flags;
    int tick, time_delta;
} cf_render_view;
typedef struct {
    const float *surfels;
    uint32_t count;
    float pose[16];
    float conf_threshold;
    int model_id;
    int colour_mode;
} cf_render_item;
typedef struct {
    void *dst;
    int kind;
    int mode;
} cf_render_output;
int cf_render_create(cf_ctx *ctx, int max_w, int max_h, cf_renderer **out);
void cf_render_destroy(cf_renderer *r);
int cf_render(cf_renderer *r, const cf_render_view *view, const cf_render_item *items, int n_items, const cf_render_output *outputs,
              int n_outputs);
int cf_render_palette(uint8_t *rgb768);

#define CF_FERNS_MAX 2048
typedef struct cf_ferns cf_ferns;
typedef struct {
    int32_t x, y;
    int32_t r, g, b;
    int32_t d;
} cf_fern;
typedef struct {
    int n_ferns;
    int capacity;
    int max_depth_mm;
    float photo_threshold;
} cf_ferns_config;
typedef struct {
    int accepted;
    int keyframe;
    float dissimilarity;
    float overlap;
    float pose[16];
    float icp_error, icp_count;
    int icp_ran;
    int photo_count;
    double photo_error;
} cf_ferns_result;
int cf_ferns_table(uint64_t seed, int n_ferns, int reduced_width, int reduced_height, int max_depth_mm, cf_fern *out);
int cf_ferns_create(cf_ctx *ctx, const cf_ferns_config *cfg, const cf_fern *table, uint64_t seed, cf_ferns **out);
void cf_ferns_destroy(cf_ferns *f);
int cf_ferns_get_table(const cf_ferns *f, cf_fern *out );
int cf_ferns_encode(cf_ferns *f, const float *vertex4, const float *normal4, const uint8_t *rgba);
int cf_ferns_search(cf_ferns *f, int time, int min_age);
int cf_ferns_append(cf_ferns *f, const float pose[16], int src_time, float threshold);
int cf_ferns_add_async(cf_ferns *f, const float *vertex4, const float *normal4, const uint8_t *rgba, const float pose[16], int src_time,
                       float threshold);
int cf_ferns_relocalise(cf_ferns *f, const float curr_pose[16], int time, int min_age, int lost, cf_ferns_result *result);
int cf_ferns_count(cf_ferns *f, int *count, int *full);
int cf_ferns_download(cf_ferns *f, int id, uint8_t *codes, int *good, float pose[16], int *time, float *vmap, float *nmap, uint8_t *rgb);
int cf_ferns_last_search(cf_ferns *f, int32_t *co_host, int co_capacity, int *searched, float *min_all, float *min_match, int *match_id,
                         int *appended);
#include "cofusion_loop.h"

typedef struct { int32_t h, v, bw, bh, first; } cf_jpeg_comp;
typedef struct {
    int32_t width, height, ncomp , hmax, vmax, total_blocks;
    cf_jpeg_comp comp[3];
    uint8_t qt[3][64];
} cf_jpeg_header;
#define CF_JPEG_MAX_BLOCKS(w, h) (48ull * (uint64_t)(((w) + 31) / 32) * (uint64_t)(((h) + 31) / 32))
#define CF_FRAME_COLOR_NONE 0
#define CF_FRAME_COLOR_JPEG 1
#define CF_FRAME_COLOR_RAW 2
#define CF_FRAME_COLOR_DECODED 3
typedef struct {
    int32_t width, height;
    int32_t color_kind;
    int32_t flip_colors;
} cf_frame_desc;
typedef struct {
    cf_jpeg_header *header;
    int16_t *coef;
    uint64_t coef_blocks;
    uint16_t *depth;
    uint8_t *rgb;
} cf_frame_slot;
typedef struct cf_frame_decoder cf_frame_decoder;
int cf_frame_decoder_create(cf_ctx *ctx, int max_w, int max_h, int slots, cf_frame_decoder **out);
void cf_frame_decoder_destroy(cf_frame_decoder *dec);
int cf_frame_decoder_slot(cf_frame_decoder *dec, int slot, cf_frame_slot *out);
int cf_frame_decoder_submit(cf_frame_decoder *dec, int slot, const cf_frame_desc *desc);
int cf_frame_decoder_acquire(cf_frame_decoder *dec, int slot, int complete, const float **depth_dev, const uint8_t **rgba_dev);
int cf_frame_decoder_timing(cf_frame_decoder *dec, int on, double *idct_ms, double *finish_ms, uint64_t *frames);

#define CF_IMAGE_NONE 0
#define CF_IMAGE_PNG 1
#define CF_IMAGE_EXR 2
#define CF_IMAGE_JPEG 3
#define CF_IMAGE_RAW 4
typedef struct { uint32_t offset, bytes, stored_raw, first_line; } cf_exr_block;
typedef struct {
    int32_t width, height;
    int32_t color_kind, depth_kind, mask_kind;
    int32_t flip_colors;
    int32_t png_color_type;
    int32_t png_palette_entries;
    float depth_scale;
    int32_t exr_blocks;
    int32_t exr_lines_per_block;
    int32_t exr_line_bytes;
    int32_t exr_chan_offset;
    int32_t exr_chan_half;
} cf_image_desc;
typedef struct {
    uint8_t *color;  uint64_t color_bytes;
    uint8_t *depth;  uint64_t depth_bytes;
    uint8_t *mask;   uint64_t mask_bytes;
    uint8_t *palette;
    cf_exr_block *blocks;  uint32_t max_blocks;
} cf_image_slot;
int cf_frame_decoder_enable_images(cf_frame_decoder *dec);
int cf_frame_decoder_image_slot(cf_frame_decoder *dec, int slot, cf_image_slot *out);
int cf_frame_decoder_submit_images(cf_frame_decoder *dec, int slot, const cf_image_desc *desc);
int cf_frame_decoder_acquire_mask(cf_frame_decoder *dec, int slot, int complete, const uint8_t **mask_dev);
int cf_frame_decoder_image_timing(cf_frame_decoder *dec, double *exr_ms, uint64_t *exr_frames, double *finish_ms, uint64_t *finish_frames);

#define CF_PNG_LABELS 1
typedef struct {
    uint32_t offset;
    uint32_t bytes;
    uint32_t adler;
    uint32_t stream_bytes;
} cf_png_band;
typedef struct {
    int32_t width, height, channels, rows_per_band, bands;
    const cf_png_band *table;
    const uint8_t *data;
    uint64_t data_bytes;
} cf_png_stream;
typedef struct cf_png_encoder cf_png_encoder;
int cf_png_encoder_create(cf_ctx *ctx, int max_w, int max_h, int slots, int rows_per_band, cf_png_encoder **out);
void cf_png_encoder_destroy(cf_png_encoder *enc);
int cf_png_encoder_submit(cf_png_encoder *enc, int slot, const void *src_dev, int width, int height, int channels, int flags);
int cf_png_encoder_acquire(cf_png_encoder *enc, int slot, cf_png_stream *out);
int cf_png_encoder_timing(cf_png_encoder *enc, int on, double *kernel_ms, uint64_t *images);

int cf_odom_bench_icp(cf_odom *od, int level, int iters, float *avg_us);

typedef struct {
    double icp_ms_total;
    uint64_t icp_launches;
    uint64_t icp_bytes;
    double surfel_ms_total;
    uint64_t surfel_calls;
    uint64_t surfel_bytes;
} cf_profile;
int cf_profile_enable(cf_ctx *ctx, int on);
int cf_profile_read(cf_ctx *ctx, cf_profile *out, int reset);

#define CF_DEFORM_MAX_NODES 1024
#define CF_DEFORM_MAX_CONSTRAINTS 128
#define CF_DEFORM_MAX_CONSTRAINTS_SIZED 1536
#define CF_DEFORM_BAND 240
typedef struct cf_deform cf_deform;
typedef struct {
    float min_cons_error; int max_iterations; float min_delta, min_error, min_change, max_first_error, accept_cons_error, accept_error;
} cf_deform_thresholds;
typedef struct { float error; double delta_norm; int failed; float mean_cons_error; } cf_deform_step;
typedef struct {
    int optimised, accepted, failed, iterations;
    float error_before, mean_cons_error_before, error, mean_cons_error;
} cf_deform_result;
typedef struct {
    float pose[16];
    cf_cam cam; int cols, rows;
    float max_depth;
    const float *depth;
// ... 66 lines not shown
```

Before: 946.8.

## Fold kept-surfel compaction into the prediction splat raster and resolve launches

After cleaning, the kept-surfel compaction (block sums and scatter) is no longer launched separately. It is merged into the model prediction's raster and resolve kernels, which now read the staged surfels through live flags and a bound. Each fused kernel splits its grid so the two independent pieces of work share a launch. This removes launches and lets compaction run alongside prediction, at the cost of larger kernel arguments, a batch size capped by the 4 KB argument segment, and a raster pass that reads uncompacted staged buffers with per-id flag checks.

```diff
diff --git a/co_fusion_amd/csrc/cabi.hip b/co_fusion_amd/csrc/cabi.hip
--- a/co_fusion_amd/csrc/cabi.hip
+++ b/co_fusion_amd/csrc/cabi.hip
@@ -61,6 +61,9 @@
             ctx->set_error("CF_ICP_ARITH: product | gram | reference"); return CF_EINVAL;
         }
     }
+    if (const char* e = getenv("CF_SURFEL_FOLDS")) {
+        if (cf_set_surfel_folds(ctx, (e[0] >= '0' && e[0] <= '3' && !e[1]) ? e[0] - '0' : -1) != CF_OK) { ctx->set_error("CF_SURFEL_FOLDS: 0 | 1 | 2 | 3"); return CF_EINVAL; }
+    }
     if (int r = dmalloc(ctx, &ctx->d_cand_scratch, (size_t)cfg->width * cfg->height)) return r;
     HIPCHK(ctx, hipHostMalloc(reinterpret_cast<void**>(&ctx->h_scratch_state), sizeof(OdomDev)));
     HIPCHK(ctx, hipHostMalloc(reinterpret_cast<void**>(&ctx->h_out), sizeof(unsigned long long) * 64));
diff --git a/co_fusion_amd/csrc/cabi_model.hip b/co_fusion_amd/csrc/cabi_model.hip
--- a/co_fusion_amd/csrc/cabi_model.hip
+++ b/co_fusion_amd/csrc/cabi_model.hip
@@ -566,6 +566,8 @@
         ctx->surf_calls++;
     }
     static const bool clean_rec_on = getenv("CF_NO_CLEAN_REC") == nullptr;
+    static const bool side_by_side = getenv("CF_NO_SIDE_BY_SIDE") == nullptr;
+    const int folds = side_by_side && !ctx->collective && !ctx->rccl ? ctx->surfel_folds : 0;
     auto index_args_of = [&](const std::vector<int>& which, bool feeds_clean, std::vector<IndexPassArgs>& a) -> int {
         a.assign(which.size(), IndexPassArgs{});
         for (size_t q = 0; q < which.size(); q++) {
@@ -577,6 +579,8 @@
         }
         return CF_OK;
     };
+    std::vector<ScanPassArgs> kept(n);
+    std::vector<unsigned> staged_bound(n, 0u);
     if (!fusing.empty()) {
         const int nf = (int)fusing.size();
         {
@@ -608,7 +612,6 @@
         {
             std::vector<IndexPassArgs> ia;
             if (int r = index_args_of(fusing, true, ia)) return r;
-            static const bool side_by_side = getenv("CF_NO_SIDE_BY_SIDE") == nullptr;
             if (!(side_by_side && launch_update_compaction_index_keys(s, ua.data(), sa.data(), ia.data(), nf, cam, W, H))) {
                 launch_scan_scatter_batch(s, sa.data(), nf);
                 launch_update_batch(s, ua.data(), nf);
@@ -626,7 +629,8 @@
             sa[q] = kept_compaction_args(m, bound);
         }
         launch_clean_batch(s, ca.data(), nf);
-        launch_scan_scatter_batch(s, sa.data(), nf);
+        for (int q = 0; q < nf; q++) { kept[fusing[q]] = sa[q]; staged_bound[fusing[q]] = ca[q].total_bound; }
+        if (!(folds & 2)) launch_scan_scatter_batch(s, sa.data(), nf);
         if (!ctx->batch_event) HIPCHK(ctx, hipEventCreateWithFlags(&ctx->batch_event, hipEventDisableTiming));
         for (int q = 0; q < nf; q++) {
             cf_model* m = items[fusing[q]].model;
@@ -647,7 +651,24 @@
                                    m->fill_vertex, m->fill_normal, m->fill_image, reinterpret_cast<unsigned long long*>(m->d_tmp2 + 4),
                                    m->d_tmp2 + 2, m->h_counts + 2, m->ratio_blocks};
     }
-    launch_combined_predict_batch(s, pa.data(), n, cam, W, H);
+    if ((folds & 2) && !fusing.empty()) {
+        std::vector<SplatPassArgs> fp; std::vector<ScanPassArgs> fs;
+        for (int at = 0; at < n; at += kSurfFoldBatch) {
+            const int cnt = n - at < kSurfFoldBatch ? n - at : kSurfFoldBatch;
+            fp.assign(pa.begin() + at, pa.begin() + at + cnt); fs.clear();
+            for (int k = at; k < at + cnt; k++)
+                if (items[k].do_fuse) {
+                    SplatPassArgs& p = fp[k - at]; cf_model* m = items[k].model;
+                    p.surfels = m->staged; p.live = m->flags; p.count = nullptr; p.count_bound = staged_bound[k];
+                    fs.push_back(kept[k]);
+                }
+            if (fs.empty() || !launch_predict_kept_compaction(s, fp.data(), cnt, fs.data(), (int)fs.size(), cam, W, H)) {
+                if (!fs.empty()) launch_scan_scatter_batch(s, fs.data(), (int)fs.size());
+                launch_combined_predict_batch(s, pa.data() + at, cnt, cam, W, H);
+            }
+        }
+    } else
+        launch_combined_predict_batch(s, pa.data(), n, cam, W, H);
     LAUNCHCHK(ctx);
     for (int k = 0; k < n; k++)
         if (items[k].fill_in) {
@@ -737,6 +758,12 @@
     ctx->extent_cull = on != 0;
     return CF_OK;
 }
+int cf_set_surfel_folds(cf_ctx* ctx, int mask)
+{
+    if (!ctx || mask < 0 || mask > 3) return CF_EINVAL;
+    ctx->surfel_folds = mask;
+    return CF_OK;
+}
 int cf_model_extents_unknown(cf_model* m)
 {
     if (!m) return CF_EINVAL;
diff --git a/co_fusion_amd/csrc/cf_host.h b/co_fusion_amd/csrc/cf_host.h
--- a/co_fusion_amd/csrc/cf_host.h
+++ b/co_fusion_amd/csrc/cf_host.h
@@ -39,6 +39,7 @@
     bool slot_used[kStateSlots]{};
     hipEvent_t batch_event = nullptr;
     bool extent_cull = true;
+    int surfel_folds = 3;
     static constexpr int kLanes = 8;
     hipStream_t lanes[kLanes]{};
     hipEvent_t lane_done[kLanes]{};
diff --git a/co_fusion_amd/csrc/cf_kernels.h b/co_fusion_amd/csrc/cf_kernels.h
--- a/co_fusion_amd/csrc/cf_kernels.h
+++ b/co_fusion_amd/csrc/cf_kernels.h
@@ -327,6 +327,7 @@
     const float* surfels; const unsigned* count; unsigned count_bound; float t_inv[16]; float maxDepth, confThreshold; int time, maxTime, timeDelta;
     const float* rays; unsigned long long* keys; uint8_t* image; float* vertexConf; float* normalRad; uint16_t* time16;
     SplatFillArgs fill;
+    const unsigned* live = nullptr;
 };
 struct UpdatePassArgs { const float* in; const unsigned* count; unsigned count_bound; unsigned* owner; const float* records; int time; float* out; };
 struct SurfelFuseArgs {
@@ -353,6 +354,8 @@
 bool launch_update_compaction_index_keys(hipStream_t s, const UpdatePassArgs* up, const ScanPassArgs* sc, const IndexPassArgs* ix, int n, cf_cam cam, int cols,
                                          int rows);
 void launch_index_resolve_batch(hipStream_t s, const IndexPassArgs* items, int n, cf_cam cam, int cols, int rows);
+constexpr int kSurfFoldBatch = 12;
+bool launch_predict_kept_compaction(hipStream_t s, const SplatPassArgs* sp, int n, const ScanPassArgs* sc, int n_sc, cf_cam cam, int cols, int rows);
 enum { kSplatFull = 0, kSplatCount = 1, kSplatDepth = 2 };
 void launch_combined_predict_batch(hipStream_t s, const SplatPassArgs* items, int n, cf_cam cam, int cols, int rows, int mode = kSplatFull);
 void launch_associate_batch(hipStream_t s, const SurfelFuseArgs* items, int n);
diff --git a/co_fusion_amd/csrc/surf_batch_dev.h b/co_fusion_amd/csrc/surf_batch_dev.h
--- a/co_fusion_amd/csrc/surf_batch_dev.h
+++ b/co_fusion_amd/csrc/surf_batch_dev.h
@@ -13,24 +13,27 @@
 #else
 static constexpr int xcd_env(const char*, int dflt) { return dflt; }
 #endif
-struct BatchHdr { int n; int blk_end[kSurfBatch]; };
-template <class A> struct Batch { BatchHdr h; A m[kSurfBatch]; };
+template <int N> struct BatchHdrN { int n; int blk_end[N]; };
+using BatchHdr = BatchHdrN<kSurfBatch>;
+template <class A, int N = kSurfBatch> struct Batch { BatchHdrN<N> h; A m[N]; };
 struct VBlock { int model, bid, nblk; };
-__device__ __forceinline__ VBlock batch_decode_at(const BatchHdr& h, int b)
+template <int N>
+__device__ __forceinline__ VBlock batch_decode_at(const BatchHdrN<N>& h, int b)
 {
     int slot = 0;
 #pragma unroll
-    for (int k = 0; k < kSurfBatch - 1; k++) slot += (b >= h.blk_end[k]) ? 1 : 0;
+    for (int k = 0; k < N - 1; k++) slot += (b >= h.blk_end[k]) ? 1 : 0;
     const int start = slot ? h.blk_end[slot - 1] : 0;
     return VBlock{slot, b - start, h.blk_end[slot] - start};
 }
-__device__ __forceinline__ VBlock batch_decode(const BatchHdr& h) { return batch_decode_at(h, (int)blockIdx.x); }
-template <class A>
-static int batch_layout(Batch<A>& B, const int* blocks, int n)
+template <int N>
+__device__ __forceinline__ VBlock batch_decode(const BatchHdrN<N>& h) { return batch_decode_at(h, (int)blockIdx.x); }
+template <class A, int N>
+static int batch_layout(Batch<A, N>& B, const int* blocks, int n)
 {
     int total = 0;
     B.h.n = n;
-    for (int k = 0; k < kSurfBatch; k++) {
+    for (int k = 0; k < N; k++) {
         if (k < n) total += (blocks[k] + 7) / 8 * 8;
         B.h.blk_end[k] = k < n ? total : 0x7fffffff;
     }
diff --git a/co_fusion_amd/csrc/surf_scan_dev.h b/co_fusion_amd/csrc/surf_scan_dev.h
--- a/co_fusion_amd/csrc/surf_scan_dev.h
+++ b/co_fusion_amd/csrc/surf_scan_dev.h
@@ -21,7 +21,8 @@
         for (int e = 0; e < 8; e++) f[e] = (i0 + e < n) ? t[e] : 0u;
     }
 }
-__device__ __forceinline__ void scan_block_sums_body(const Batch<ScanArgs>& B, int blk)
+template <int N>
+__device__ __forceinline__ void scan_block_sums_body(const Batch<ScanArgs, N>& B, int blk)
 {
     const VBlock vb = batch_decode_at(B.h, blk);
     const ScanArgs& a = B.m[vb.model];
@@ -39,7 +40,8 @@
     if (threadIdx.x == 0) block_sums[vb.bid] = w[0] + w[1] + w[2] + w[3];
 }
 __global__ void __launch_bounds__(256) scan_block_sums_kernel(const Batch<ScanArgs> B) { scan_block_sums_body(B, (int)blockIdx.x); }
-__device__ __forceinline__ void scan_scatter_body(const Batch<ScanArgs>& B, int blk)
+template <int N>
+__device__ __forceinline__ void scan_scatter_body(const Batch<ScanArgs, N>& B, int blk)
 {
     const VBlock vb = batch_decode_at(B.h, blk);
     const ScanArgs& a = B.m[vb.model];
diff --git a/co_fusion_amd/csrc/surf_splat_dev.h b/co_fusion_amd/csrc/surf_splat_dev.h
--- a/co_fusion_amd/csrc/surf_splat_dev.h
+++ b/co_fusion_amd/csrc/surf_splat_dev.h
@@ -59,20 +59,22 @@
 
 struct SplatArgs {
     const float4* surfels; const unsigned* count; Mat4 t_inv; float maxDepth, confThreshold; int time, maxTime, timeDelta;
+    unsigned bound;
     const float4* rays; unsigned long long* keys; uchar4* image; float4* vertexConf; float4* normalRad; unsigned short* time16;
     SplatFillArgs fill;
 };
 
-__global__ void __launch_bounds__(kB) splat_raster_kernel(const Batch<SplatArgs> B, const FrameGeom g)
-{
-    const VBlock vb = batch_decode(B.h);
+template <int N>
+__device__ __forceinline__ void splat_raster_body(const Batch<SplatArgs, N>& B, const FrameGeom& g, int blk)
+{
+    const VBlock vb = batch_decode_at(B.h, blk);
     const SplatArgs& a = B.m[vb.model];
     const float4* __restrict__ surfels = a.surfels; const float4* __restrict__ rays = a.rays; unsigned long long* __restrict__ keys = a.keys;
     const int cols = g.cols, rows = g.rows;
     const unsigned gt = vb.bid * kB + threadIdx.x;
     const unsigned id = gt >> 2;
     const int sub = (int)(gt & 3u);
-    if (id >= *a.count) return;
+    if (a.bound ? (id >= a.bound || a.count[id] == 0) : id >= *a.count) return;
     SplatSetup s;
     if (!splat_setup(surfels[id * 3], surfels[id * 3 + 1], surfels[id * 3 + 2], a.t_inv, g.cam, cols, rows, a.maxDepth, a.confThreshold, a.time,
                      a.maxTime, a.timeDelta, s))
@@ -91,6 +93,7 @@
         while (fx >= w) { fx -= w; fy++; }
     }
 }
+__global__ void __launch_bounds__(kB) splat_raster_kernel(const Batch<SplatArgs> B, const FrameGeom g) { splat_raster_body(B, g, (int)blockIdx.x); }
 
 __device__ __forceinline__ void fill_in_px(float4 v, float4 n, uchar4 e, const float* __restrict__ depth, const uchar4* __restrict__ rgba, int cols,
                                            int rows, int x, int y, int q, float cx, float cy, float inv_fx, float inv_fy, int pass_geom, int pass_rgb,
@@ -140,10 +143,10 @@
     return blocks;
 }
 
-template <int kMode>
-__global__ void __launch_bounds__(kB) splat_resolve_kernel(const Batch<SplatArgs> B, const FrameGeom g)
-{
-    const VBlock vb = batch_decode(B.h);
+template <int kMode, int N>
+__device__ __forceinline__ void splat_resolve_body(const Batch<SplatArgs, N>& B, const FrameGeom& g, int blk)
+{
+    const VBlock vb = batch_decode_at(B.h, blk);
     const SplatArgs& a = B.m[vb.model];
     const float4* __restrict__ surfels = a.surfels; const float4* __restrict__ rays = a.rays; unsigned long long* __restrict__ keys = a.keys;
     uchar4* __restrict__ image = a.image; float4* __restrict__ vertexConf = a.vertexConf; float4* __restrict__ normalRad = a.normalRad;
@@ -210,6 +213,8 @@
     a.fill.out2[0] = total; a.fill.out2[1] = samples;
     if (a.fill.out2_host) { a.fill.out2_host[0] = total; a.fill.out2_host[1] = samples; }
 }
+template <int kMode>
+__global__ void __launch_bounds__(kB) splat_resolve_kernel(const Batch<SplatArgs> B, const FrameGeom g) { splat_resolve_body<kMode>(B, g, (int)blockIdx.x); }
 
 __global__ void __launch_bounds__(1024) fill_ratio_kernel(const uchar4* __restrict__ pimg, int cols, int rows, unsigned* __restrict__ out2,
                                                           unsigned* __restrict__ out2_host)
@@ -234,16 +239,17 @@
     }
 }
 
+static SplatArgs splat_args(const SplatPassArgs& h)
+{
+    return SplatArgs{reinterpret_cast<const float4*>(h.surfels), h.live ? h.live : h.count, mat4_from(h.t_inv), h.maxDepth, h.confThreshold, h.time, h.maxTime,
+                     h.timeDelta, h.live ? h.count_bound : 0u, reinterpret_cast<const float4*>(h.rays), h.keys, reinterpret_cast<uchar4*>(h.image),
+                     reinterpret_cast<float4*>(h.vertexConf), reinterpret_cast<float4*>(h.normalRad), h.time16, h.fill};
+}
+static int splat_raster_blocks(const SplatPassArgs& h) { return gridFor(4ll * h.count_bound); }
 void launch_combined_predict_batch(hipStream_t s, const SplatPassArgs* items, int n_items, cf_cam cam, int cols, int rows, int mode)
 {
     const FrameGeom g{cam, cols, rows};
-    for_each_batch<SplatArgs>(items, n_items,
-        [](const SplatPassArgs& h, SplatArgs& a) {
-            a = SplatArgs{reinterpret_cast<const float4*>(h.surfels), h.count, mat4_from(h.t_inv), h.maxDepth, h.confThreshold, h.time, h.maxTime,
-                          h.timeDelta, reinterpret_cast<const float4*>(h.rays), h.keys, reinterpret_cast<uchar4*>(h.image),
-                          reinterpret_cast<float4*>(h.vertexConf), reinterpret_cast<float4*>(h.normalRad), h.time16, h.fill};
-            return gridFor(4ll * h.count_bound);
-        },
+    for_each_batch<SplatArgs>(items, n_items, [](const SplatPassArgs& h, SplatArgs& a) { a = splat_args(h); return splat_raster_blocks(h); },
         [&](Batch<SplatArgs>& B, int* blocks, int nb, const SplatPassArgs*) {
             if (const int grid = batch_layout(B, blocks, nb)) splat_raster_kernel<<<grid, kB, 0, s>>>(B, g);
             for (int k = 0; k < nb; k++) blocks[k] = gridFor((long long)cols * rows);
diff --git a/co_fusion_amd/csrc/surfel.hip b/co_fusion_amd/csrc/surfel.hip
--- a/co_fusion_amd/csrc/surfel.hip
+++ b/co_fusion_amd/csrc/surfel.hip
@@ -45,4 +45,43 @@
     return true;
 }
 
+template <class A> using Fold = Batch<A, kSurfFoldBatch>;
+static_assert(sizeof(Fold<SplatArgs>) + sizeof(FrameGeom) + sizeof(Fold<ScanArgs>) + 16 <= 4096,
+              "the folded launches carry the prediction's and the compaction's arguments in one 4 KB kernel-argument segment: lower kSurfFoldBatch");
+__global__ void __launch_bounds__(kB) splatraster_blocksums_kernel(const Fold<SplatArgs> P, const FrameGeom g, const Fold<ScanArgs> S, int p_blocks)
+{
+    const int b = (int)blockIdx.x;
+    if (b < p_blocks) splat_raster_body(P, g, b);
+    else scan_block_sums_body(S, b - p_blocks);
 }
+__global__ void __launch_bounds__(kB) splatresolve_scatter_kernel(const Fold<SplatArgs> P, const FrameGeom g, const Fold<ScanArgs> S, int s_blocks)
+{
+    const int b = (int)blockIdx.x;
+    if (b < s_blocks) scan_scatter_body(S, b);
+    else splat_resolve_body<kSplatFull>(P, g, b - s_blocks);
+}
+bool launch_predict_kept_compaction(hipStream_t s, const SplatPassArgs* sp, int n, const ScanPassArgs* sc, int n_sc, cf_cam cam, int cols, int rows)
+{
+    if (n <= 0 || n > kSurfFoldBatch || n_sc <= 0 || n_sc > n) return false;
+    Fold<SplatArgs> P; Fold<ScanArgs> S;
+    int pb[kSurfFoldBatch], sb[kSurfFoldBatch];
+    for (int k = 0; k < n_sc; k++) {
+        if (sc[k].zero_flags) return false;
+        S.m[k] = scan_args(sc[k]); sb[k] = scan_blocks(sc[k]);
+        if (sb[k] == 0) return false;
+    }
+    for (int k = 0; k < n; k++) {
+        if (sp[k].live && sp[k].count_bound == 0) return false;
+        P.m[k] = splat_args(sp[k]); pb[k] = splat_raster_blocks(sp[k]);
+    }
+    const int sg = batch_layout(S, sb, n_sc);
+    const FrameGeom g{cam, cols, rows};
+    const int pg = batch_layout(P, pb, n);
+    splatraster_blocksums_kernel<<<pg + sg, kB, 0, s>>>(P, g, S, pg);
+    for (int k = 0; k < n; k++) pb[k] = gridFor((long long)cols * rows);
+    const int rg = batch_layout(P, pb, n);
+    splatresolve_scatter_kernel<<<sg + rg, kB, 0, s>>>(P, g, S, sg);
+    return true;
+}
+
+}
diff --git a/co_fusion_amd/facade.py b/co_fusion_amd/facade.py
--- a/co_fusion_amd/facade.py
+++ b/co_fusion_amd/facade.py
@@ -518,6 +518,9 @@
     def set_extent_culling(self, on=True):
         assert self.abi.cf_set_extent_culling(self._ctx(), int(bool(on))) == 0
 
+    def set_surfel_folds(self, mask=3):
+        assert self.abi.cf_set_surfel_folds(self._ctx(), int(mask)) == 0
+
     def model_download(self, index):
         n = self.model_info(index)["count"]
         out = np.zeros((max(n, 1), 12), np.float32)
diff --git a/co_fusion_amd/lib.py b/co_fusion_amd/lib.py
--- a/co_fusion_amd/lib.py
+++ b/co_fusion_amd/lib.py
@@ -19,7 +19,7 @@
     "cf_bilateral", "cf_model_create", "cf_model_destroy", "cf_model_initialise", "cf_model_count",
     "cf_model_predict_indices", "cf_model_index_keys", "cf_model_index_resolve", "cf_model_combined_predict", "cf_model_predict_inactive", "cf_model_synthesize_depth", "cf_model_prefetch_fill_ratio", "cf_model_perform_fill_in", "cf_model_requires_fill_in",
     "cf_model_fuse", "cf_model_clean", "cf_models_frame_passes", "cf_models_preindex", "cf_model_download_map", "cf_model_upload_map", "cf_model_buffer",
-    "cf_set_extent_culling", "cf_model_extents_unknown",
+    "cf_set_extent_culling", "cf_set_surfel_folds", "cf_model_extents_unknown",
     "cf_redetect_score", "cf_redetect_timing", "cf_relabel",
     "cf_redetect_frame_moments", "cf_redetect_model_moments", "cf_redetect_register_step", "cf_redetect_register",
     "cf_fusion_weight", "cf_seg_create", "cf_seg_destroy", "cf_seg_slic", "cf_seg_crf", "cf_seg_sums", "cf_seg_infer", "cf_seg_early", "cf_seg_run_batch", "cf_seg_fetch", "cf_seg_publish_poses", "cf_seg_fetch_poses",
diff --git a/co_fusion_amd/model.py b/co_fusion_amd/model.py
--- a/co_fusion_amd/model.py
+++ b/co_fusion_amd/model.py
@@ -55,6 +55,10 @@
     ctx._check(ctx.lib.cf_set_extent_culling(ctx.h, int(bool(on))))
 
 
+def set_surfel_folds(ctx: Context, mask=3):
+    ctx._check(ctx.lib.cf_set_surfel_folds(ctx.h, int(mask)))
+
+
 _BUF = {0: (np.uint32, 1), 1: (np.float32, 4), 2: (np.float32, 4), 3: (np.float32, 4), 4: (np.uint8, 4), 5: (np.float32, 4),
         6: (np.float32, 4), 7: (np.uint16, 1), 8: (np.float32, 4), 9: (np.float32, 4), 10: (np.uint8, 4),
         15: (np.uint8, 4), 16: (np.float32, 4), 17: (np.float32, 4), 18: (np.uint16, 1)}
diff --git a/include/cofusion_hip.h b/include/cofusion_hip.h
--- a/include/cofusion_hip.h
+++ b/include/cofusion_hip.h
@@ -279,6 +279,7 @@
 int cf_model_upload_map(cf_model *m, const float *host_surfels, uint32_t count);
 int cf_model_buffer(cf_model *m, int which, void **dptr, uint64_t *bytes);
 int cf_set_extent_culling(cf_ctx *ctx, int on);
+int cf_set_surfel_folds(cf_ctx *ctx, int mask);
 int cf_model_extents_unknown(cf_model *m);
 typedef struct { uint32_t projected, occluded, seen_through, agree, agree_on_label, covered; } cf_redetect_counts;
 typedef struct {
```

Result: no change. 955.5 (median of 6 runs) (+0.9%).
